# uw-x/AcousticSwarms-Speech

Hardware: AMD Instinct MI355X
Metric: TDoA candidates/sec (shift+normalise+spot forward+energies) (higher is better)
Workload: dtype f32 via f16x3 split-operand MFMA (fp32 accumulate); 1 GPU; configs[2] scene: 5-speaker reverberant mixture (image sources), 7 mics, T=48000 samples (BASELINE's '3 s @ 16 kHz' sample count; the reference pipeline and this scene generator run at 48 kHz, where it is a 1 s clip -- the reference-native 3 s is extras.T144000), fine-stage (Strict=1) candidate batch of one mixture, FULL spot net 47.27 M params, seeded random weights; internal_batch=256, parallelism=candidate-shard x1

## Files before the change

acousticswarms-speech_amd/csrc/asw_common.cpp:

```cpp
#include "asw_common.h"

#include <cmath>
#include <cstdlib>

namespace asw {
char* err_buf() {
  static thread_local char buf[512] = {0};
  return buf;
}
int set_error(int code, const char* fmt, ...) {
  va_list ap;
  va_start(ap, fmt);
  vsnprintf(err_buf(), 512, fmt, ap);
  va_end(ap);
  return code;
}
int SmemAttr::ensure(const void* kern, size_t want) {
  int dev = 0;
  ASW_HIP(hipGetDevice(&dev));
  if (dev < 0 || dev >= kMaxDev) return set_error(ASW_ERR_ARG, "device ordinal %d out of range", dev);
  if (bytes[dev] >= want) return ASW_OK;
  ASW_HIP(hipFuncSetAttribute(kern, hipFuncAttributeMaxDynamicSharedMemorySize, (int)want));
  bytes[dev] = want;
  return ASW_OK;
}
}

extern "C" const char* asw_last_error(void) { return asw::err_buf(); }
extern "C" int asw_abi_version(void) { return 3; }

extern "C" int asw_split_weights_f16(const float* w, size_t n, uint16_t* hi, uint16_t* lo, int32_t* w_shift) {
  ASW_CHECK_ARG(w && hi && lo && w_shift, "split_weights: null pointer");
  float mx = 0.f;
  for (size_t i = 0; i < n; ++i) { const float a = w[i] < 0 ? -w[i] : w[i]; if (a > mx || a != a) mx = a; }
  ASW_CHECK_ARG(mx == mx && mx < 3.0e38f, "split_weights: non-finite weight");
  int shift = 0;
  if (mx > 0.f) {
    int e;
    (void)frexpf(mx, &e);
    shift = 11 - e;
    if (shift > 24) shift = 24;
    if (shift < -24) shift = -24;
  }
  const float sc = ldexpf(1.0f, shift);
  for (size_t i = 0; i < n; ++i) {
    float c = w[i] * sc;
    if (c > 65504.f) c = 65504.f;
    if (c < -65504.f) c = -65504.f;
    const _Float16 h = (_Float16)c;
    const _Float16 l = (_Float16)(c - (float)h);
    memcpy(hi + i, &h, 2);
    memcpy(lo + i, &l, 2);
  }
  *w_shift = shift;
  return ASW_OK;
}

extern "C" int asw_pack_fragments_f16(const float* Wt, int N, int K, uint16_t* hi, uint16_t* lo, int32_t* w_shift) {
  ASW_CHECK_ARG(Wt && hi && lo && w_shift, "pack_fragments: null pointer");
  ASW_CHECK_ARG(N > 0 && K > 0 && N % 32 == 0 && K % 16 == 0, "pack_fragments: N %% 32, K %% 16 required (N=%d K=%d)", N, K);
  const size_t n = (size_t)N * K;
  uint16_t* th = new uint16_t[2 * n];
  uint16_t* tl = th + n;
  int rc = asw_split_weights_f16(Wt, n, th, tl, w_shift);
  if (rc == ASW_OK) {
    const int NT = N / 32;
    for (int ks = 0; ks < K / 16; ++ks)
      for (int nt = 0; nt < NT; ++nt)
        for (int l = 0; l < 64; ++l) {
          const size_t src = (size_t)(nt * 32 + (l & 31)) * K + ks * 16 + 8 * (l >> 5);
          const size_t dst = (((size_t)ks * NT + nt) * 64 + l) * 8;
          memcpy(hi + dst, th + src, 16);
          memcpy(lo + dst, tl + src, 16);
        }
  }
  delete[] th;
  return rc;
}

extern "C" int asw_up_feed_kperm(int k) { return (k & ~12) | ((k & 4) << 1) | ((k & 8) >> 1); }

extern "C" int asw_pack_up_feed_f16(const float* Wt, int N, int K, uint16_t* hi, uint16_t* lo, int32_t* w_shift) {
  ASW_CHECK_ARG(Wt && N > 0 && K > 0 && K % 16 == 0, "pack_up_feed: K %% 16 required (N=%d K=%d)", N, K);
  float* wp = new float[(size_t)N * K];
  for (int n = 0; n < N; ++n)
    for (int k = 0; k < K; ++k) wp[(size_t)n * K + k] = Wt[(size_t)n * K + (k & ~15) + asw_up_feed_kperm(k & 15)];
  const int rc = asw_pack_fragments_f16(wp, N, K, hi, lo, w_shift);
  delete[] wp;
  return rc;
}

namespace asw {
bool residue_feed_on() {
  static const bool off = getenv("ASW_NO_RESIDUE_FEED") != nullptr;
  return !off;
}
}

extern "C" int asw_residue_schedule(int taps, int stride, int dil, int pad, int Cin, int BK, int BM, int m0, int has_skip,
                                    asw_residue_stage* out, int cap, int* n_stages, int* max_shift) {
  ASW_CHECK_ARG(n_stages != nullptr && cap >= 0 && (out != nullptr || cap == 0), "residue_schedule: null pointer");
  ASW_CHECK_ARG(taps > 0 && stride > 0 && dil > 0 && Cin > 0 && BK > 0 && BM > 0, "residue_schedule: bad dims");
  *n_stages = 0;
  if (max_shift) *max_shift = 0;
  if (!asw::residue_feed_applies(taps, stride, dil, Cin, BK, has_skip != 0)) return ASW_OK;
  const asw::ResidueFeed rf{taps, stride, Cin / BK};
  ASW_CHECK_ARG(rf.ntaps(0) <= ASW_RESIDUE_MAX_TAPS, "residue_schedule: %d taps on one image, at most %d", rf.ntaps(0),
                ASW_RESIDUE_MAX_TAPS);
  *n_stages = rf.stages();
  if (max_shift) *max_shift = rf.shifts(0);
  for (int s = 0; s < rf.stages() && s < cap; ++s) {
    asw_residue_stage& d = out[s];
    memset(&d, 0, sizeof d);
    d.residue = s / rf.cpb;
    d.chunk = s - d.residue * rf.cpb;
    d.rows = BM + rf.shifts(d.residue);
    d.first_row = m0 * stride - pad + d.residue;
    d.ntaps = rf.ntaps(d.residue);
    for (int q = 0; q < d.ntaps; ++q) {
      d.tap[q] = rf.tap(d.residue, q);
      d.shift[q] = q;
      d.kstep[q] = rf.kstep(d.tap[q], d.chunk, BK / 16);
    }
  }
  return ASW_OK;
}

#include <map>
#include <mutex>
#include <vector>
namespace asw {
namespace {
struct Rec { std::string name; double work, bytes; hipEvent_t e0, e1; };
std::mutex g_mu;
bool g_on = false;
bool g_detail = false;
std::vector<Rec> g_recs;
std::vector<hipEvent_t> g_pool;
hipEvent_t take_event() {
  if (!g_pool.empty()) { hipEvent_t e = g_pool.back(); g_pool.pop_back(); return e; }
  hipEvent_t e = nullptr;
  (void)hipEventCreate(&e);
  return e;
}
}

std::string prof_name(const char* base, int bm, int bn, int bk, bool ln, bool stats) {
  char b[96];
  snprintf(b, sizeof b, "%s<%d,%d,%d,%s>", base, bm, bn, bk, ln ? "ln" : stats ? "stats" : "plain");
  return b;
}
bool prof_detail() { return g_detail; }
ProfScope::ProfScope(hipStream_t s, const std::string& name, double work, double bytes) : slot(-1), stream(s) {
  if (!g_on) return;
  std::lock_guard<std::mutex> lk(g_mu);
  Rec r{name, work, bytes, take_event(), take_event()};
  (void)hipEventRecord(r.e0, s);
  g_recs.push_back(r);
  slot = (int)g_recs.size() - 1;
}
ProfScope::~ProfScope() {
  if (slot < 0) return;
  std::lock_guard<std::mutex> lk(g_mu);
  if (slot < (int)g_recs.size()) (void)hipEventRecord(g_recs[slot].e1, stream);
}
}

extern "C" int asw_profile_enable(int on) {
  std::lock_guard<std::mutex> lk(asw::g_mu);
  for (auto& r : asw::g_recs) { asw::g_pool.push_back(r.e0); asw::g_pool.push_back(r.e1); }
  asw::g_recs.clear();
  asw::g_on = on != 0;
  asw::g_detail = on == 2;
  return ASW_OK;
}

extern "C" int asw_profile_report(char* buf, size_t cap) {
  if (!buf || cap < 64) return asw::set_error(ASW_ERR_ARG, "profile_report: buffer too small");
  std::lock_guard<std::mutex> lk(asw::g_mu);
  struct Agg { long n = 0; double ms = 0, work = 0, bytes = 0; };
  std::map<std::string, Agg> agg;
  for (auto& r : asw::g_recs) {
    if (hipEventSynchronize(r.e1) != hipSuccess) continue;
    float ms = 0.f;
    if (hipEventElapsedTime(&ms, r.e0, r.e1) != hipSuccess) continue;
    Agg& a = agg[r.name];
    a.n += 1; a.ms += ms; a.work += r.work; a.bytes += r.bytes;
  }
  size_t off = 0;
  off += snprintf(buf + off, cap - off, "{");
  bool first = true;
  for (auto& kv : agg) {
    if (off + 256 >= cap) break;
    off += snprintf(buf + off, cap - off, "%s\"%s\":{\"launches\":%ld,\"ms\":%.6f,\"work\":%.6e,\"bytes\":%.6e}", first ? "" : ",",
                    kv.first.c_str(), kv.second.n, kv.second.ms, kv.second.work, kv.second.bytes);
    first = false;
  }
  snprintf(buf + off, cap - off, "}");
  return ASW_OK;
}
```

acousticswarms-speech_amd/csrc/model_common.h:

```cpp
#pragma once
#include <cstdlib>
#include <iterator>
#include <map>
#include <memory>
#include <string>
#include <vector>

#include "asw_common.h"

namespace asw_model {

struct DevBuf {
  float* p = nullptr;
  size_t n = 0;
  DevBuf() = default;
  DevBuf(const DevBuf&) = delete;
  DevBuf& operator=(const DevBuf&) = delete;
  DevBuf(DevBuf&& o) noexcept : p(o.p), n(o.n) { o.p = nullptr; o.n = 0; }
  ~DevBuf() { if (p) (void)hipFree(p); }
  int upload(const std::vector<float>& h) {
    if (p) { (void)hipFree(p); p = nullptr; }
    n = h.size();
    if (hipMalloc(&p, n * sizeof(float)) != hipSuccess) return asw::set_error(ASW_ERR_NOMEM, "hipMalloc(%zu floats)", n);
    ASW_HIP(hipMemcpy(p, h.data(), n * sizeof(float), hipMemcpyHostToDevice));
// ... 86 lines not shown
inline int pack_res_layers(const std::map<std::string, std::vector<float>>& raw, const std::string& p, int ch, int K,
                           int n_layers, int dil_factor, std::vector<ResLayer>& out) {
  out.clear();
  out.resize(n_layers);
  int dil = 1;
  for (int j = 0; j < n_layers; ++j) {
    const std::string q = p + ".res.seq." + std::to_string(j);
    int rc;
    {
      const std::vector<float> packed = pack_conv(raw.at(q + ".conv.weight"), ch, ch, K, nullptr);
      if ((rc = out[j].wt.upload(packed))) return rc;
      if (ch % 32 == 0 && (ch * K) % 16 == 0 && (rc = out[j].wt.upload_frags(packed, ch, ch * K))) return rc;
    }
    if ((rc = out[j].bias.upload(raw.at(q + ".conv.bias")))) return rc;
    if ((rc = out[j].g.upload(raw.at(q + ".norm.weight")))) return rc;
    if ((rc = out[j].b.upload(raw.at(q + ".norm.bias")))) return rc;
    out[j].dil = dil;
    dil *= dil_factor;
  }
  return ASW_OK;
}

struct Arena {
  char* base;
  size_t off = 0, cap;
  bool dry;
  Arena(char* b, size_t c, bool d) : base(b), cap(c), dry(d) {}
  template <typename T>
  T* take(size_t n) {
    off = (off + 255) & ~(size_t)255;
    T* p = reinterpret_cast<T*>(base + off);
    off += n * sizeof(T);
    return p;
  }
};


struct GluSrc { const float* raw; const float* mr; const float* gamma; const float* beta; float* side_out = nullptr; };

inline bool glu_on_load_ok(const std::vector<ResLayer>& res, int prec, int ch) {
  static const int max_c = getenv("ASW_GLU_ON_LOAD_MAX_C") ? atoi(getenv("ASW_GLU_ON_LOAD_MAX_C")) : 512;
  return prec >= 1 && (ch == 64 || ch == 128 || ch == 256 || ch == 512) && ch <= max_c && !res.empty() &&
         res[0].dil == 1 && res[0].wt.fhi && res[0].wt.flo;
}

inline bool resstack_ok(const std::vector<ResLayer>& res, int prec, int ch, int K) {
  static const bool off = getenv("ASW_NO_RESSTACK") != nullptr;
  if (off || prec < 1 || ch != 64 || K % 2 == 0 || K < 3 || K > 15) return false;
  for (const ResLayer& r : res)
    if (!r.wt.fhi || !r.wt.flo) return false;
  return true;
}

inline size_t resstack_fuse_count(const std::vector<ResLayer>& res, size_t j, int K) {
  static const bool nofuse = getenv("ASW_RESSTACK_NOFUSE") != nullptr;
  size_t n = 1;
  int halo = 0;
  while (!nofuse && j + n < res.size() && n < 3) {
    const int pad = res[j + n].dil * (K - 1) / 2;
    if (halo + pad > 64) break;
    halo += pad;
    ++n;
  }
  return n;
}

struct SrcFeed { const void* hi; const void* lo; const WBuf* comp; const WBuf* pre; };

struct UpFeed { const WBuf* w; const float* bias; const float* skip; float* out; float* stats; int tiles; };

inline void resstack_last_launch(const std::vector<ResLayer>& res, int K, size_t& j0, size_t& n) {
  j0 = 0;
  n = resstack_fuse_count(res, 0, K);
  while (j0 + n < res.size()) { j0 += n; n = resstack_fuse_count(res, j0, K); }
}
inline int up_feed_tiles(const std::vector<ResLayer>& res, int K, int T, bool glu) {
  size_t j0, n;
  resstack_last_launch(res, K, j0, n);
  int32_t dil[3] = {1, 1, 1};
  for (size_t i = 0; i < n; ++i) dil[i] = res[j0 + i].dil;
  return asw_resstack_tiles(T, K, (int)n, dil, glu && j0 == 0);
}

inline int run_res(const std::vector<ResLayer>& res, int prec, int B, int T, int ch, int K, float* x, float* p, float* q,
            float** final_out, hipStream_t s, const GluSrc* glu = nullptr, const SrcFeed* feed = nullptr, UpFeed* up = nullptr) {
  const float* in = glu ? glu->raw : x;
  float* outb = p;
  if (feed && !(resstack_ok(res, prec, ch, K) && prec == 1 && resstack_fuse_count(res, 0, K) == 2))
    return asw::set_error(ASW_ERR_STATE, "run_res: the source-fed form needs the fused f16x3 pair");
  if (up && !(resstack_ok(res, prec, ch, K) && prec == 1))
    return asw::set_error(ASW_ERR_STATE, "run_res: UpFeed needs the f16x3 stack kernel");
  if (resstack_ok(res, prec, ch, K)) {
    size_t j = 0;
    while (j < res.size()) {
      const size_t n = resstack_fuse_count(res, j, K);
      asw_resstack_args a = {};
      a.x = ((glu || feed) && j == 0) ? nullptr : in;
      a.out = outb;
      a.B = B; a.T = T; a.C = ch; a.taps = K; a.n_layers = (int)n; a.precision = prec; a.ln_eps = 1e-5f;
      for (size_t i = 0; i < n; ++i) {
        const ResLayer& r = res[j + i];
        a.layer[i].Wf_hi = r.wt.fhi; a.layer[i].Wf_lo = r.wt.flo; a.layer[i].w_shift = r.wt.shift;
        a.layer[i].bias = r.bias.p; a.layer[i].ln_gamma = r.g.p; a.layer[i].ln_beta = r.b.p; a.layer[i].dil = r.dil;
      }
      if (glu && j == 0) {
        a.glu_raw = glu->raw; a.glu_mr = glu->mr; a.glu_gamma = glu->gamma; a.glu_beta = glu->beta; a.glu_out = glu->side_out;
      }
      if (feed && j == 0) {
        a.src_hi = feed->hi; a.src_lo = feed->lo;
        a.layer[0].Wf_hi = feed->comp->fhi; a.layer[0].Wf_lo = feed->comp->flo; a.layer[0].w_shift = feed->comp->shift;
        a.pre_hi = feed->pre->fhi; a.pre_lo = feed->pre->flo; a.pre_shift = feed->pre->shift;
      }
      if (up && j + n == res.size()) {
        a.out = nullptr;
        a.up_hi = up->w->fhi; a.up_lo = up->w->flo; a.up_shift = up->w->shift; a.up_bias = up->bias; a.up_skip = up->skip;
        a.up_out = up->out; a.up_stats = up->stats;
        up->tiles = up_feed_tiles(res, K, T, glu != nullptr);
        if (up->tiles < 0) return up->tiles;
        outb = nullptr;
      }
      int rc = asw_resstack64_f16x3(&a, s);
      if (rc) return rc;
      in = outb;
      outb = (outb == p) ? q : p;
      j += n;
    }
    *final_out = const_cast<float*>(in);
    return ASW_OK;
  }
  for (size_t j = 0; j < res.size(); ++j) {
    asw_convgemm_args a = {};
    a.A = in; res[j].wt.bind(a, prec); a.bias = res[j].bias.p; a.resid = in;
    if (glu && j == 0) {
      a.glu_raw = glu->raw; a.glu_mr = glu->mr; a.glu_gamma = glu->gamma; a.glu_beta = glu->beta; a.glu_out = glu->side_out;
    }
    a.ln_gamma = res[j].g.p; a.ln_beta = res[j].b.p; a.out = outb;
    a.B = B; a.M_out = T; a.N = ch; a.Cin = ch; a.taps = K; a.stride = 1; a.dil = res[j].dil;
    a.pad = (res[j].dil * (K - 1) + 1) / 2;
    a.a_row_stride = ch; a.a_batch_stride = (int64_t)T * ch; a.a_len = (int64_t)T * ch;
    a.relu = 1; a.ln_eps = 1e-5f;
    int rc = asw_convgemm_f32(&a, s);
    if (rc) return rc;
    in = outb;
    outb = (outb == p) ? q : p;
  }
  *final_out = const_cast<float*>(in);
  return ASW_OK;
}

inline int linear(const float* A, const WBuf& W, int prec, const float* bias, int rows, int N, int K, int relu, const float* resid,
           const float* g, const float* b, float* out, hipStream_t s) {
  asw_convgemm_args a = {};
  a.A = A; W.bind(a, prec); a.bias = bias; a.resid = resid; a.ln_gamma = g; a.ln_beta = b; a.out = out;
  a.B = 1; a.M_out = rows; a.N = N; a.Cin = K; a.taps = 1; a.stride = 1; a.dil = 1; a.pad = 0;
  a.a_row_stride = K; a.a_batch_stride = (int64_t)rows * K; a.a_len = (int64_t)rows * K;
  a.relu = relu; a.ln_eps = 1e-5f;
  if (g && N >= 1024 && N % 256 == 0 && N <= 2048) {
    a.resid = nullptr; a.ln_gamma = nullptr; a.ln_beta = nullptr;
    int rc = asw_convgemm_f32(&a, s);
    if (rc) return rc;
    return asw_add_layernorm(out, resid, g, b, rows, N, 1e-5f, out, s);
  }
  return asw_convgemm_f32(&a, s);
}

inline void pack_conv_transpose(const std::vector<float>& w, const std::vector<float>& b, int Cin, int N, int S,
                                const float* out_gate, std::vector<float>& wt, std::vector<float>& bb) {
  wt.assign((size_t)S * N * Cin, 0.f);
  bb.assign((size_t)S * N, 0.f);
  for (int r = 0; r < S; ++r)
    for (int n = 0; n < N; ++n) {
      bb[(size_t)r * N + n] = out_gate ? b[n] * out_gate[n] : b[n];
      for (int c = 0; c < Cin; ++c) {
        const float v = w[((size_t)c * N + n) * S + r];
        wt[((size_t)r * N + n) * Cin + c] = out_gate ? v * out_gate[n] : v;
      }
    }
}


#define UP(buf, vec) if ((rc = (buf).upload(vec))) return rc

struct TrunkCfg {
  int n_mics, kernel_size, depth, stride_list[8], channels, growth, encoder_channels, encoder_kernel_size,
      encoder_stride, residual_layers, residual_dilation_factor, ffw_dim;
  template <class Cfg>
  static TrunkCfg of(const Cfg& c) {
    TrunkCfg t = {c.n_mics, c.kernel_size, c.depth, {}, c.channels, c.growth, c.encoder_channels,
                  c.encoder_kernel_size, c.encoder_stride, c.residual_layers, c.residual_dilation_factor, c.ffw_dim};
    for (int i = 0; i < 8; ++i) t.stride_list[i] = c.stride_list[i];
    return t;
  }
};

inline int check_trunk_config(const TrunkCfg& c, const char* who, const char* odd) {
  ASW_CHECK_ARG(c.depth >= 1 && c.depth <= 8, "%s: depth %d", who, c.depth);
  ASW_CHECK_ARG(c.n_mics >= 1 && c.n_mics <= 32, "%s: n_mics %d", who, c.n_mics);
  ASW_CHECK_ARG(c.channels % 64 == 0, "%s: channels=%d must be a multiple of 64 for the MFMA tiles", who, c.channels);
  ASW_CHECK_ARG(c.growth >= 1 && c.residual_layers >= 1, "%s: bad config", who);
  ASW_CHECK_ARG(c.kernel_size % 2 == 1, "%s: %s", who, odd);
  ASW_CHECK_ARG(c.encoder_channels % 128 == 0, "%s: encoder_channels must be a multiple of 128", who);
  ASW_CHECK_ARG(c.encoder_stride % 4 == 0 && c.encoder_kernel_size / 2 == c.encoder_stride && c.encoder_kernel_size <= 64,
                "%s: encoder kernel/stride %d/%d unsupported (the reference's trim [9:-8] assumes 33/16)", who,
                c.encoder_kernel_size, c.encoder_stride);
  ASW_CHECK_ARG(c.ffw_dim % 128 == 0, "%s: ffw_dim must be a multiple of 128", who);
  return ASW_OK;
}

struct EncBlock { std::vector<ResLayer> res; DevBuf bias, gn_g, gn_b; };
struct DecBlock { std::vector<ResLayer> res; DevBuf gn_g, gn_b; };
struct GatedConvs { std::vector<WBuf> down_wt, up_wt, up_feed; std::vector<DevBuf> up_bias; };
struct Tap { const float* p; size_t numel; };
using ParamList = std::vector<std::pair<std::string, size_t>>;

struct TrunkPlan {
  int B, T, Tp, F, RL;
  std::vector<int> Tl;
  float *mean, *stdv, *refn;
  uint16_t *src_hi = nullptr, *src_lo = nullptr;
  std::vector<float*> X, Pb, Qb, raw_dn, raw_up, st_dn, st_up, mr_dn, mr_up;
  float *Y, *D, *ywave;
};

struct Trunk {
  TrunkCfg tc;
  std::map<std::string, std::vector<float>> raw;
  std::map<std::string, Tap> taps;
  bool finalized = false;
  int device = 0;
  int precision = 0;
  bool exact_raw = false;
  bool fuse_mask = true;
  bool want_src = false;
  bool src_stack = true;
  bool want_up = false;
  bool up_fusion = true;

  std::vector<int> enc_cin, enc_cout;
  std::vector<int> dec_cin, dec_cout, dec_stride;
  int stride_product = 1;

  DevBuf pre_w, pre_b;
  WBuf src_wt, src_pre;
  std::vector<EncBlock> enc;
  std::vector<DecBlock> dec;
  WBuf byp_wt, mask_wt, dec_wt;
  WBuf byp_wt48;
  DevBuf byp_b, mask_b;
  float out_bias = 0.f;
  int byp_k = 0;

  const std::vector<float>& P(const std::string& k) const { return raw.at(k); }

  enum class Src { Normed, Raw };
  int site(Src a) const { return !exact_raw ? precision : a == Src::Raw ? 0 : 3; }

  int init_shape(const TrunkCfg& c, const char* who) {
    tc = c;
    ASW_HIP(hipGetDevice(&device));
    int cin = c.channels, ch = c.channels;
    for (int i = 0; i < c.depth; ++i) {
      ASW_CHECK_ARG(c.stride_list[i] >= 1, "%s: stride", who);
      enc_cin.push_back(cin);
      enc_cout.push_back(ch);
      stride_product *= c.stride_list[i];
      cin = ch;
      ch *= c.growth;
    }
    dec_cin.assign(enc_cout.rbegin(), enc_cout.rend());
    dec_cout.assign(enc_cin.rbegin(), enc_cin.rend());
    dec_stride.assign(std::make_reverse_iterator(c.stride_list + c.depth), std::make_reverse_iterator(c.stride_list));
    return ASW_OK;
  }
  int check_level_widths(const char* who) const {
    for (int w : enc_cin) ASW_CHECK_ARG(w <= 512 && (w & (w - 1)) == 0, "%s: level width %d must be a power of two <= 512", who, w);
    return ASW_OK;
  }

  ParamList trunk_params() const {
    ParamList v;
    const size_t K = tc.kernel_size;
    v.push_back({"preproc.weight", (size_t)tc.channels * tc.n_mics});
    v.push_back({"preproc.bias", (size_t)tc.channels});
    auto res = [&](const std::string& p, size_t ch) {
      for (int j = 0; j < tc.residual_layers; ++j) {
        const std::string q = p + ".res.seq." + std::to_string(j);
        v.push_back({q + ".conv.weight", ch * ch * K});
        v.push_back({q + ".conv.bias", ch});
        v.push_back({q + ".norm.weight", ch});
        v.push_back({q + ".norm.bias", ch});
      }
    };
    for (int i = 0; i < tc.depth; ++i) {
      const std::string p = "encoder.module_list." + std::to_string(i);
      const size_t ci = enc_cin[i], co = enc_cout[i];
      res(p, ci);
      v.push_back({p + ".conv1.weight", 2 * co * ci * K});
      v.push_back({p + ".conv1.bias", 2 * co});
      v.push_back({p + ".norm1.weight", 2 * co});
      v.push_back({p + ".norm1.bias", 2 * co});
    }
    for (int i = 0; i < tc.depth; ++i) {
      const std::string p = "decoder.module_list." + std::to_string(i);
      const size_t ci = dec_cin[i], co = dec_cout[i], s = dec_stride[i];
      v.push_back({p + ".upsample.conv.weight", ci * 2 * co * s});
      v.push_back({p + ".upsample.conv.bias", 2 * co});
      v.push_back({p + ".norm1.weight", 2 * co});
      v.push_back({p + ".norm1.bias", 2 * co});
      res(p, co);
    }
    const size_t E = tc.encoder_channels, EK = tc.encoder_kernel_size;
    v.push_back({"reference_bypass.weight", E * EK});
    v.push_back({"reference_bypass.bias", E});
    v.push_back({"mask_encoder.weight", E * tc.channels * EK});
    v.push_back({"mask_encoder.bias", E});
    v.push_back({"output_decoder.weight", E * EK});
    v.push_back({"output_decoder.bias", 1});
    return v;
  }
// ... 97 lines not shown
    }
    return ASW_OK;
  }

  bool fused_mask_path() const {
    return fuse_mask && precision >= 1 && tc.encoder_channels % 256 == 0 && tc.channels % 32 == 0 &&
           tc.encoder_kernel_size <= 48 && tc.encoder_stride % 4 == 0 && byp_wt48.fhi && dec_wt.fhi && mask_wt.fhi;
  }
  bool src_path() const {
    return want_src && src_stack && precision == 1 && src_wt.fhi && src_pre.fhi && !enc.empty() &&
           resstack_ok(enc[0].res, precision, enc_cin[0], tc.kernel_size) &&
           resstack_fuse_count(enc[0].res, 0, tc.kernel_size) == 2;
  }
  bool up_feed_shape(int j) const {
    return j >= 1 && dec_cin[j] == 64 && dec_cout[j] == 64 && dec_stride[j] == 2 && dec_cout[j - 1] == 64;
  }
  bool up_path(const GatedConvs& g, int j) const {
    static const bool off = getenv("ASW_NO_UP_FUSION") != nullptr;
    return !off && want_up && up_fusion && precision == 1 && up_feed_shape(j) && g.up_feed[j].fhi &&
           resstack_ok(dec[j - 1].res, precision, 64, tc.kernel_size);
  }
  void layout_levels(int B, int T, Arena& a, TrunkPlan& pl) const {
    const int depth = tc.depth, EK = tc.encoder_kernel_size, ES = tc.encoder_stride;
    pl.B = B; pl.T = T;
    pl.Tp = ((T - 1) / stride_product + 1) * stride_product;
    pl.F = (pl.Tp + 2 * (EK / 2) - EK) / ES + 1;
    pl.RL = ((EK / 2 + pl.Tp + byp_k + 64) + 3) & ~3;
    pl.Tl.assign(depth + 1, pl.Tp);
    for (int i = 0; i < depth; ++i) pl.Tl[i + 1] = pl.Tl[i] / tc.stride_list[i];
    pl.mean = a.take<float>(B);
    pl.stdv = a.take<float>(B);
    pl.refn = a.take<float>((size_t)B * pl.RL);
    if (want_src) {
      pl.src_hi = a.take<uint16_t>((size_t)B * pl.Tp * 8);
      pl.src_lo = a.take<uint16_t>((size_t)B * pl.Tp * 8);
    }
    pl.X.resize(depth + 1); pl.Pb.resize(depth); pl.Qb.resize(depth);
    pl.raw_dn.resize(depth); pl.raw_up.resize(depth); pl.st_dn.resize(depth); pl.st_up.resize(depth);
    pl.mr_up.resize(depth); pl.mr_dn.resize(depth);
    for (int i = 0; i <= depth; ++i) {
      const int ch = i == 0 ? tc.channels : enc_cout[i - 1];
      pl.X[i] = a.take<float>((size_t)B * pl.Tl[i] * ch);
    }
    for (int i = 0; i < depth; ++i) {
      const size_t n = (size_t)B * pl.Tl[i] * enc_cin[i];
      pl.Pb[i] = a.take<float>(n);
      pl.Qb[i] = a.take<float>(n);
      pl.raw_dn[i] = a.take<float>((size_t)B * pl.Tl[i + 1] * 2 * enc_cout[i]);
      pl.st_dn[i] = a.take<float>((size_t)B * 4 * asw_convgemm_stats_tiles(pl.Tl[i + 1], 2 * enc_cout[i]));
      pl.mr_dn[i] = a.take<float>((size_t)B * 4);
    }
    for (int j = 0; j < depth; ++j) {
      const int lvl = depth - j;
      const int s = dec_stride[j], co2 = 2 * dec_cout[j];
      pl.raw_up[j] = a.take<float>((size_t)B * pl.Tl[lvl] * s * co2);
      int tiles = asw_convgemm_stats_tiles(pl.Tl[lvl], s * co2);
      if (want_up && up_feed_shape(j))
        for (int glu = 0; glu < 2; ++glu) {
          const int t = up_feed_tiles(dec[j - 1].res, tc.kernel_size, pl.Tl[lvl], glu != 0);
          tiles = t > tiles ? t : tiles;
        }
      pl.st_up[j] = a.take<float>((size_t)B * 4 * tiles);
      pl.mr_up[j] = a.take<float>((size_t)B * 4);
    }
  }
  void layout_mask(Arena& a, TrunkPlan& pl) const {
    const int E = tc.encoder_channels;
    const bool fused = fused_mask_path();
    pl.Y = fused ? nullptr : a.take<float>((size_t)pl.B * pl.F * E);
    pl.D = a.take<float>((size_t)(fused ? E / 256 : 1) * pl.B * pl.F * 64);
    pl.ywave = a.take<float>((size_t)pl.B * pl.T);
  }

  int encode(TrunkPlan& pl, const GatedConvs& g, hipStream_t s, bool src0 = false) {
    const int B = pl.B, K = tc.kernel_size;
    taps.clear();
    if (!src0) taps["preproc"] = {pl.X[0], (size_t)B * pl.Tl[0] * tc.channels};
    int rc;
    GluSrc src = {};
    const SrcFeed feed = {pl.src_hi, pl.src_lo, &src_wt, &src_pre};
    bool glu = false;
    for (int i = 0; i < tc.depth; ++i) {
      float* r = nullptr;
      if ((rc = run_res(enc[i].res, precision, B, pl.Tl[i], enc_cin[i], K, pl.X[i], pl.Pb[i], pl.Qb[i], &r, s,
                        glu ? &src : nullptr, (src0 && i == 0) ? &feed : nullptr)))
        return rc;
      asw_convgemm_args a = {};
      a.A = r; g.down_wt[i].bind(a, precision); a.bias = enc[i].bias.p; a.out = pl.raw_dn[i]; a.stats = pl.st_dn[i];
      a.B = B; a.M_out = pl.Tl[i + 1]; a.N = 2 * enc_cout[i]; a.Cin = enc_cin[i]; a.taps = K;
      a.stride = tc.stride_list[i]; a.dil = 1; a.pad = K / 2;
      a.a_row_stride = a.Cin; a.a_batch_stride = (int64_t)pl.Tl[i] * a.Cin; a.a_len = a.a_batch_stride;
      a.chan_mod = a.N;
      if ((rc = asw_convgemm_f32(&a, s))) return rc;
      glu = fuse_mask && i + 1 < tc.depth && glu_on_load_ok(enc[i + 1].res, precision, enc_cout[i]);
      const int tiles = asw_convgemm_stats_tiles(a.M_out, a.N);
      if (glu) {
        if ((rc = asw_gn_finalize(pl.st_dn[i], tiles, B, pl.Tl[i + 1], enc_cout[i], 1e-5f, pl.mr_dn[i], s))) return rc;
        src = {pl.raw_dn[i], pl.mr_dn[i], enc[i].gn_g.p, enc[i].gn_b.p, pl.X[i + 1]};
      } else if ((rc = asw_gn_glu(pl.raw_dn[i], pl.st_dn[i], tiles, enc[i].gn_g.p, enc[i].gn_b.p, B, pl.Tl[i + 1],
                                  enc_cout[i], 1e-5f, pl.X[i + 1], s))) {
        return rc;
      }
      taps["enc" + std::to_string(i)] = {pl.X[i + 1], (size_t)B * pl.Tl[i + 1] * enc_cout[i]};
    }
    return ASW_OK;
  }

  int decode(TrunkPlan& pl, const GatedConvs& g, const float*& x, hipStream_t s, bool up = false) {
    const int B = pl.B, K = tc.kernel_size;
    int rc;
    int fed_tiles = 0;
    for (int j = 0; j < tc.depth; ++j) {
      const int lvl = tc.depth - j, ci = dec_cin[j], co = dec_cout[j], st = dec_stride[j];
      int tiles = fed_tiles;
      if (!fed_tiles) {
        asw_convgemm_args a = {};
        a.A = x; a.A2 = pl.X[lvl]; g.up_wt[j].bind(a, precision); a.bias = g.up_bias[j].p; a.out = pl.raw_up[j];
        a.stats = pl.st_up[j];
        a.B = B; a.M_out = pl.Tl[lvl]; a.N = st * 2 * co; a.Cin = ci; a.taps = 1; a.stride = 1; a.dil = 1; a.pad = 0;
        a.a_row_stride = ci; a.a_batch_stride = (int64_t)pl.Tl[lvl] * ci; a.a_len = a.a_batch_stride;
        a.chan_mod = 2 * co;
        if ((rc = asw_convgemm_f32(&a, s))) return rc;
        tiles = asw_convgemm_stats_tiles(a.M_out, a.N);
      }
      const int To = pl.Tl[lvl] * st;
      float* gb = pl.Qb[lvl - 1];
      float* r = nullptr;
      const bool feed_next = up && j + 1 < tc.depth && up_path(g, j + 1);
      UpFeed uf = {};
      if (feed_next) uf = {&g.up_feed[j + 1], g.up_bias[j + 1].p, pl.X[lvl - 1], pl.raw_up[j + 1], pl.st_up[j + 1], 0};
      UpFeed* ufp = feed_next ? &uf : nullptr;
      if (fuse_mask && glu_on_load_ok(dec[j].res, precision, co)) {
        if ((rc = asw_gn_finalize(pl.st_up[j], tiles, B, To, co, 1e-5f, pl.mr_up[j], s))) return rc;
        const GluSrc src = {pl.raw_up[j], pl.mr_up[j], dec[j].gn_g.p, dec[j].gn_b.p, co > 64 ? gb : nullptr};
        if ((rc = run_res(dec[j].res, precision, B, To, co, K, gb, pl.Pb[lvl - 1], gb, &r, s, &src, nullptr, ufp))) return rc;
      } else {
        if ((rc = asw_gn_glu(pl.raw_up[j], pl.st_up[j], tiles, dec[j].gn_g.p, dec[j].gn_b.p, B, To, co, 1e-5f, gb, s)))
          return rc;
        if ((rc = run_res(dec[j].res, precision, B, To, co, K, gb, pl.Pb[lvl - 1], gb, &r, s, nullptr, nullptr, ufp))) return rc;
      }
      x = r;
      fed_tiles = feed_next ? uf.tiles : 0;
      if (!feed_next) taps["dec" + std::to_string(j)] = {x, (size_t)B * To * co};
    }
    return ASW_OK;
  }

  int mask_path(TrunkPlan& pl, const float* x, const float* mean, const float* stdv, float* out_wave, hipStream_t s) {
    const int B = pl.B, C = tc.channels, E = tc.encoder_channels, EK = tc.encoder_kernel_size, ES = tc.encoder_stride;
    int rc;
    asw_convgemm_args me = {};
    me.A = x; mask_wt.bind(me, site(Src::Normed)); me.bias = mask_b.p;
    me.B = B; me.M_out = pl.F; me.N = E; me.Cin = C; me.taps = EK; me.stride = ES; me.dil = 1; me.pad = EK / 2;
    me.a_row_stride = C; me.a_batch_stride = (int64_t)pl.Tp * C; me.a_len = me.a_batch_stride;
    if (fused_mask_path()) {
      asw_maskpath_args f = {};
      f.enc = me;
      f.ref = pl.refn; f.ref_batch_stride = pl.RL; f.ref_len = pl.RL; f.ref_hop = ES;
      f.byp_k = 48; f.byp_taps = EK; f.byp_shift = byp_wt48.shift; f.byp_hi = byp_wt48.fhi; f.byp_lo = byp_wt48.flo;
      f.byp_bias = byp_b.p;
      f.dec_hi = dec_wt.fhi; f.dec_lo = dec_wt.flo; f.dec_shift = dec_wt.shift; f.dec_taps = EK;
      f.taps = pl.D;
      f.enc.precision = precision;
      if ((rc = exact_raw ? asw_mask_path_f16x3_scaled(&f, s) : asw_mask_path_f16x3(&f, s))) return rc;
      return asw_overlap_add_parts(pl.D, E / 256, B, pl.F, 64, EK, EK / 2, pl.T, 9, 8, out_bias, mean, stdv, out_wave, s);
    }
    {
      asw_convgemm_args a = {};
      a.A = pl.refn; byp_wt.bind(a, site(Src::Normed)); a.bias = byp_b.p; a.out = pl.Y;
      a.B = B; a.M_out = pl.F; a.N = E; a.Cin = byp_k; a.taps = 1; a.stride = 1; a.dil = 1; a.pad = 0;
      a.a_row_stride = ES; a.a_batch_stride = pl.RL; a.a_len = pl.RL; a.relu = 1;
      if ((rc = asw_convgemm_f32(&a, s))) return rc;
    }
    me.mul = pl.Y; me.out = pl.Y; me.relu = 1;
    if ((rc = asw_convgemm_f32(&me, s))) return rc;
    taps["latent"] = {pl.Y, (size_t)B * pl.F * E};
    {
      asw_convgemm_args a = {};
      a.A = pl.Y; dec_wt.bind(a, site(Src::Raw)); a.out = pl.D;
      a.B = B; a.M_out = pl.F; a.N = 64; a.Cin = E; a.taps = 1; a.stride = 1; a.dil = 1; a.pad = 0;
      a.a_row_stride = E; a.a_batch_stride = (int64_t)pl.F * E; a.a_len = a.a_batch_stride;
      if ((rc = asw_convgemm_f32(&a, s))) return rc;
    }
    return asw_overlap_add_unnorm(pl.D, B, pl.F, 64, EK, EK / 2, pl.T, 9, 8, out_bias, mean, stdv, out_wave, s);
  }
};

struct PostNormLayer { WBuf w_in, w_out, w1, w2; DevBuf b_in, b_out, b1, b2, n1g, n1b, n2g, n2b; };
struct PostNormBufs { float *qkv, *ctx, *x1, *ff; };

template <class Attention>
int run_post_norm(const Trunk& m, const PostNormLayer& t, const PostNormBufs& b, const float* x, float* out, int rows, int d,
                  int ffw, Attention&& attention, hipStream_t s) {
  const int normed = m.site(Trunk::Src::Normed), rawp = m.site(Trunk::Src::Raw);
  int rc;
  if ((rc = linear(x, t.w_in, normed, t.b_in.p, rows, 3 * d, d, 0, nullptr, nullptr, nullptr, b.qkv, s))) return rc;
  if ((rc = attention(b.qkv, b.ctx))) return rc;
  if ((rc = linear(b.ctx, t.w_out, rawp, t.b_out.p, rows, d, d, 0, x, t.n1g.p, t.n1b.p, b.x1, s))) return rc;
  if ((rc = linear(b.x1, t.w1, normed, t.b1.p, rows, ffw, d, 1, nullptr, nullptr, nullptr, b.ff, s))) return rc;
  return linear(b.ff, t.w2, rawp, t.b2.p, rows, d, ffw, 0, b.x1, t.n2g.p, t.n2b.p, out, s);
}

inline int check_ready(const Trunk* m, const char* fin) {
  if (!m) return asw::set_error(ASW_ERR_ARG, "null model handle");
  if (!m->finalized) return asw::set_error(ASW_ERR_STATE, "%s() has not been called", fin);
  int dev = -1;
  ASW_HIP(hipGetDevice(&dev));
  if (dev != m->device)
    return asw::set_error(ASW_ERR_STATE, "model lives on HIP device %d but the current device is %d", m->device, dev);
  return ASW_OK;
}

inline int set_precision(Trunk* m, const char* who, int precision) {
  ASW_CHECK_ARG(m && (precision >= 0 && precision <= 3), "%s: 0 (f32), 1 (f16x3), 2 (single-pass f16) or 3 (f16x3_safe)", who);
  m->exact_raw = precision == 3;
  m->precision = m->exact_raw ? 1 : precision;
  return ASW_OK;
}

inline int set_param(Trunk* m, const char* who, const char* key, const float* host_data, size_t numel) {
  ASW_CHECK_ARG(m && key && host_data, "%s: null pointer", who);
  m->raw[key].assign(host_data, host_data + numel);
// ... 20 lines not shown
```

acousticswarms-speech_amd/csrc/resconv.hip:

```cpp
#include "gemm_epilogue.h"

namespace {
using namespace asw_mfma;

#ifdef ASW_PHASE_TIMING
__device__ unsigned long long g_phase_cycles[4] = {0, 0, 0, 0};
#endif

template <int BM, int PH, bool POLY>
struct ResRows {
  static constexpr int BMJ = BM / PH;
  int m0, jb, pb, dil, T;
  __device__ __forceinline__ int operator()(int trow) const {
    if (!POLY) { const int t = m0 + trow; return t < T ? t : -1; }
    const int ph = pb * PH + trow / BMJ;
    const int t = dil * (jb * BMJ + trow % BMJ) + ph;
    return (ph < dil && t < T) ? t : -1;
  }
};

template <int BM, int C, int WM, int WN, int PH, int QD = 4, bool POLY = (PH > 1), bool GLU = false, int NTERM = 3>
__global__ __launch_bounds__(64 * WM * WN)
__attribute__((amdgpu_waves_per_eu(C == 64 ? 4 : WM * WN == 8 ? 2 : (QD == 2 ? (C >= 512 || (C == 256 && BM == 128) ? 2 : 3) : (C == 64 && WM * WN == 4 ? 4 : 1)))))
void resconv16_kernel(const asw_convgemm_args p) {
  static_assert(QD == 2 || QD == 4, "B prefetch depth in k-steps");
  static_assert(!GLU || (PH == 1 && !POLY), "GroupNorm + GLU on load: contiguous tiles only");
  static_assert(WM * WN == 2 || WM * WN == 4 || WM * WN == 8, "2, 4 or 8 waves per workgroup");
  constexpr int NTHR = 64 * WM * WN;
  constexpr int TM = BM / WM / 32, TN = C / WN / 32;
  constexpr int NT = C / 32;
  constexpr int BMJ = BM / PH;
  constexpr int SU = (GLU && C > 64) ? 4 : 8;
  static_assert(BMJ % 32 == 0, "an MFMA row tile must stay inside one phase");

  extern __shared__ __align__(16) float smem[];
  char* img = reinterpret_cast<char*>(smem);

  const int tid = threadIdx.x, lane = tid & 63, wid = tid >> 6;
  const int wm = wid / WN, wn = wid % WN;
  const int b = blockIdx.z;
  const int taps = p.taps, dil = p.dil, pad = p.pad;
  const int T = p.M_out;
  const int n_pb = (dil + PH - 1) / PH;
  const int jb = !POLY ? 0 : blockIdx.x / n_pb, pb = !POLY ? 0 : blockIdx.x % n_pb;
  const int m0 = blockIdx.x * BM;
  const int RJ = BMJ + (!POLY ? (taps - 1) * dil : taps - 1);
  const int R = PH * RJ;
  const int tapstep = !POLY ? dil : 1;
  const __amdgpu_buffer_rsrc_t rX = GLU ? act_rsrc(p.glu_raw + (long)b * T * 2 * C, (long)T * 2 * C)
                                        : act_rsrc(p.A + (long)b * p.a_batch_stride, (long)T * C);
  const half8* __restrict__ Wh = reinterpret_cast<const half8*>(p.Wf_hi);
  const half8* __restrict__ Wl = reinterpret_cast<const half8*>(p.Wf_lo);

  floatx16 acc[TM][TN];
#pragma unroll
  for (int i = 0; i < TM; ++i)
#pragma unroll
    for (int j = 0; j < TN; ++j)
#pragma unroll
      for (int r = 0; r < 16; ++r) acc[i][j][r] = 0.f;

  const int sc4 = tid & 15;
  int a_base[TM];
#pragma unroll
  for (int i = 0; i < TM; ++i) {
    const int trow = wm * (BM / WM) + i * 32;
    a_base[i] = ((trow / BMJ) * RJ + trow % BMJ + (lane & 31)) * RS + (lane >> 5) * 16;
  }
  const int nt0 = wn * TN;

  GluCoef gc;
  if (GLU) gc.stats(p.glu_mr, b);
  ASW_PHASE_MARK(t_begin);
#ifdef ASW_PHASE_TIMING
  unsigned long long t_stage = 0, t_loop = 0;
#endif
#pragma unroll(C == 128 && (NTERM == 3 || GLU) ? 2 : 1)
  for (int cc = 0; cc < C / 64; ++cc) {
    ASW_PHASE_MARK(t_s0);
    if (GLU) gc.affine(p.glu_gamma, p.glu_beta, C, cc * 64 + sc4 * 4);
    __syncthreads();
    stage_image<NTHR, C, SU, GLU, NTERM, C == 64>(
        img, R, rX, cc * 64, gc,
        [&](int row) __attribute__((always_inline)) {
          int g;
          bool ok = row < R;
          if (!POLY) {
            g = m0 - pad + row;
          } else {
            const int ph = pb * PH + row / RJ;
            g = dil * (jb * BMJ + row % RJ - (taps - 1) / 2) + ph;
            ok = ok && ph < dil && (jb * BMJ + row % RJ - (taps - 1) / 2) >= 0;
          }
          return ImgSrc{g, ok && g >= 0 && g < T};
        },
        [&](int g, bool ok, const float4& o) __attribute__((always_inline)) {
          if (p.glu_out && ok && g >= m0 && g < m0 + BM)
            *reinterpret_cast<float4*>(p.glu_out + ((long)b * T + g) * C + cc * 64 + sc4 * 4) = o;
        });
    __syncthreads();
    auto bload = [&](int tap, int ks, half8 (&bh)[TN], half8 (&bl)[TN]) {
      const long kg = (long)tap * (C / 16) + cc * 4 + ks;
#pragma unroll
      for (int j = 0; j < TN; ++j) frag_load<NTERM>(Wh, Wl, kg * NT + nt0 + j, lane, bh[j], bl[j]);
    };
    auto aload = [&](int tap, int ks, half8 (&ah)[TM], half8 (&al)[TM]) {
#pragma unroll
      for (int i = 0; i < TM; ++i) {
        const char* q = img + a_base[i] + tap * tapstep * RS + ks * 32;
        ah[i] = *reinterpret_cast<const half8*>(q + IMG_HI);
        if (NTERM == 3) al[i] = *reinterpret_cast<const half8*>(q + IMG_LO);
      }
    };
    auto mma = [&](const half8 (&ah)[TM], const half8 (&al)[TM], const half8 (&bh)[TN], const half8 (&bl)[TN]) {
#pragma unroll
      for (int i = 0; i < TM; ++i)
#pragma unroll
        for (int j = 0; j < TN; ++j) mma3<NTERM>(acc[i][j], ah[i], al[i], bh[j], bl[j]);
    };
    constexpr bool ADB = C != 128;
    half8 qh[QD][TN], ql[QD][TN];
    half8 ah[ADB ? 2 : 1][TM], al[ADB ? 2 : 1][TM];
    ASW_PHASE_MARK(t_s1);
#pragma unroll
    for (int ks = 0; ks < QD; ++ks) bload(0, ks, qh[ks], ql[ks]);
    if (ADB) aload(0, 0, ah[0], al[0]);
    for (int tap = 0; tap < taps; ++tap) {
#pragma unroll
      for (int ks = 0; ks < 4; ++ks) {
        if (ADB) {
          const int nks = (ks + 1) & 3, ntp = tap + (ks == 3 ? 1 : 0);
          if (ntp < taps) aload(ntp, nks, ah[(ks + 1) & 1], al[(ks + 1) & 1]);
        } else {
          aload(tap, ks, ah[0], al[0]);
        }
        mma(ah[ADB ? (ks & 1) : 0], al[ADB ? (ks & 1) : 0], qh[ks % QD], ql[ks % QD]);
        const int nk = ks + QD, ntap = tap + nk / 4;
        if (ntap < taps) bload(ntap, nk % 4, qh[ks % QD], ql[ks % QD]);
      }
    }
#ifdef ASW_PHASE_TIMING
    {
      float sink = acc[0][0][0];
      asm volatile("" ::"v"(sink));
      const unsigned long long t_s2 = __builtin_readcyclecounter();
      t_stage += t_s1 - t_s0;
      t_loop += t_s2 - t_s1;
    }
#endif
  }
  ASW_PHASE_MARK(t_epi0);
  if constexpr (C == 64) {
    using G = EpiGeom<C, WM, WN>;
    float4 rpre[TM * G::NSTEP * G::VPL];
    const int sub = lane / G::LPR, lc = lane % G::LPR;
#pragma unroll
    for (int tm = 0; tm < TM; ++tm)
#pragma unroll
      for (int st = 0; st < G::NSTEP; ++st) {
        const int sr = (st * G::NW + wid) * G::RPI + sub;
        const int trow = (sr >> 5) * (BM / WM) + tm * 32 + (sr & 31);
        const int irow = POLY ? (trow / BMJ) * RJ + trow % BMJ + (taps - 1) / 2 : trow + pad;
#pragma unroll
        for (int q = 0; q < G::VPL; ++q) {
          const int col = (lc + q * G::LPR) * 4;
          const half4 hi = *reinterpret_cast<const half4*>(img + irow * RS + IMG_HI + col * 2);
          const half4 lo = *reinterpret_cast<const half4*>(img + irow * RS + IMG_LO + col * 2);
          rpre[(tm * G::NSTEP + st) * G::VPL + q] = make_float4((float)hi[0] + (float)lo[0], (float)hi[1] + (float)lo[1],
                                                                (float)hi[2] + (float)lo[2], (float)hi[3] + (float)lo[3]);
        }
      }
    epilogue<BM, C, WM, WN, true, false, true, false, ResRows<BM, PH, POLY>, true>(
        acc, p, smem, __builtin_ldexpf(1.0f, -p.w_shift), ResRows<BM, PH, POLY>{m0, jb, pb, dil, T}, blockIdx, gridDim.y, rpre);
  } else {
    epilogue<BM, C, WM, WN, true, false, true, false>(acc, p, smem, __builtin_ldexpf(1.0f, -p.w_shift),
                                                      ResRows<BM, PH, POLY>{m0, jb, pb, dil, T}, blockIdx, gridDim.y);
  }
#ifdef ASW_PHASE_TIMING
  {
    const unsigned long long t_end = __builtin_readcyclecounter();
    if (threadIdx.x == 0) {
      atomicAdd(&g_phase_cycles[0], t_stage);
      atomicAdd(&g_phase_cycles[1], t_loop);
      atomicAdd(&g_phase_cycles[2], t_end - t_epi0);
      atomicAdd(&g_phase_cycles[3], 1ull);
    }
    (void)t_begin;
  }
#endif
}

template <int BM, int C, int WM, int WN, int PH, int QD = 4, bool POLY = (PH > 1), bool GLU = false>
int launch_res(const asw_convgemm_args& a, hipStream_t s) {
  constexpr int BMJ = BM / PH;
  const int RJ = BMJ + (!POLY ? (a.taps - 1) * a.dil : a.taps - 1);
  const size_t img = (size_t)PH * RJ * RS;
  const size_t slab = (size_t)(WM * 32) * (C + 4) * sizeof(float);
  const size_t smem = img > slab ? img : slab;
  if (smem > 160 * 1024) return 1;
  const int gx = !POLY ? asw::cdiv(a.M_out, BM)
                       : asw::cdiv(asw::cdiv(a.M_out, a.dil), BMJ) * asw::cdiv(a.dil, PH);
  char nm[96];
  snprintf(nm, sizeof nm, "resconv16<%d,%d,%s%d%s%s>", BM, C, POLY ? "poly" : "ph", PH, QD == 2 ? ",q2" : "", GLU ? ",glu" : "");
  asw_convgemm_args k = a;
  if (GLU && C > 64) k.resid = a.glu_out;
  return asw::launch_pair<resconv16_kernel<BM, C, WM, WN, PH, QD, POLY, GLU, 1>, resconv16_kernel<BM, C, WM, WN, PH, QD, POLY, GLU, 3>>(
      a.precision, dim3(gx, 1, a.B), dim3(64 * WM * WN), smem, 160 * 1024, nm, asw::ShapeTag(a, 'd', a.dil).s,
      2.0 * a.B * (double)a.M_out * a.N * (double)a.taps * a.Cin, 0.0, s, k);
}

}

#ifdef ASW_PHASE_TIMING
extern "C" int asw_debug_phase_cycles(unsigned long long* out4, int reset) {
  ASW_HIP(hipMemcpyFromSymbol(out4, HIP_SYMBOL(g_phase_cycles), 4 * sizeof(unsigned long long)));
  if (reset) {
    const unsigned long long z[4] = {0, 0, 0, 0};
    ASW_HIP(hipMemcpyToSymbol(HIP_SYMBOL(g_phase_cycles), z, sizeof z));
  }
  return ASW_OK;
}
#endif

namespace asw {
int try_resconv(const asw_convgemm_args& a, hipStream_t s) {
  const bool shape = a.precision >= 1 && a.Wf_hi && a.Wf_lo && a.ln_gamma && a.stride == 1 && a.taps > 1 &&
                     a.taps % 2 == 1 && a.Cin == a.N && a.a_row_stride == a.Cin && a.resid == a.A && !a.A2 &&
                     !a.mul && !a.stats && a.pad * 2 == (a.taps - 1) * a.dil &&
                     a.a_len == (int64_t)a.M_out * a.Cin && a.a_batch_stride == a.a_len;
  if (!shape) return 1;
  if (a.glu_raw) {
    ASW_CHECK_ARG(a.dil == 1 && a.glu_mr && a.glu_gamma && a.glu_beta,
                  "convgemm: GroupNorm + GLU on load needs dilation 1 and the statistics / affine arrays");
    ASW_CHECK_ARG(a.N == 64 || a.glu_out, "convgemm: GroupNorm + GLU on load at %d channels takes the residual from glu_out", a.N);
  }
  const int rows_per_phase = a.M_out / a.dil;
  const bool poly = a.dil >= 16 && rows_per_phase >= 32;
  switch (a.N) {
    case 64:
      if (a.glu_raw) return launch_res<128, 64, 2, 2, 1, 4, false, true>(a, s);
      if (a.dil >= 7 && a.dil < 16 && rows_per_phase >= 96) return launch_res<128, 64, 2, 2, 1, 4, true>(a, s);
      if (!poly) return launch_res<128, 64, 2, 2, 1>(a, s);
      if (rows_per_phase >= 96) return launch_res<128, 64, 2, 2, 1, 4, true>(a, s);
      return rows_per_phase >= 48 ? launch_res<128, 64, 2, 2, 2>(a, s) : launch_res<128, 64, 2, 2, 4>(a, s);
    case 128:
      if (a.glu_raw) return launch_res<128, 128, 2, 2, 1, 2, false, true>(a, s);
      if (!poly) return launch_res<128, 128, 2, 2, 1, 2>(a, s);
      return rows_per_phase >= 48 ? launch_res<128, 128, 2, 2, 2, 2>(a, s) : launch_res<128, 128, 2, 2, 4, 2>(a, s);
    case 256: {
      if (a.glu_raw)
        return (long)asw::cdiv(a.M_out, 128) * a.B >= 512 ? launch_res<128, 256, 1, 4, 1, 2, false, true>(a, s)
                                                          : launch_res<64, 256, 1, 4, 1, 2, false, true>(a, s);
      if (!poly && (long)asw::cdiv(a.M_out, 128) * a.B >= 512) return launch_res<128, 256, 1, 4, 1, 2>(a, s);
      if (poly && rows_per_phase >= 48 && (long)asw::cdiv(a.M_out, 128) * a.B >= 512) return launch_res<128, 256, 1, 4, 2, 2>(a, s);
      return poly ? launch_res<64, 256, 1, 4, 2, 2>(a, s) : launch_res<64, 256, 1, 4, 1, 2>(a, s);
    }
    case 512:
      if (a.glu_raw) return launch_res<64, 512, 1, 4, 1, 2, false, true>(a, s);
      if (poly && a.M_out / a.dil >= 64) return launch_res<64, 512, 1, 4, 2>(a, s);
      return a.dil >= 16 ? launch_res<64, 512, 1, 4, 1>(a, s) : launch_res<64, 512, 1, 4, 1, 2>(a, s);
    default: return 1;
  }
}
}
```

acousticswarms-speech_amd/csrc/resstack.hip:

```cpp
#include <type_traits>

#include "asw_common.h"
#include "f16x3_tile.h"

namespace {
using namespace asw_mfma;

constexpr int C = 64;
constexpr int MAXL = 3;

struct LayerDev {
  const half8* Wh;
  const half8* Wl;
  const float* bias;
  const float* gamma;
  const float* beta;
  int dil, pad;
  int halo;
  int nfrag;
  float scale;
};

#ifdef ASW_PHASE_TIMING
__device__ unsigned long long g_rs_cycles[6] = {0, 0, 0, 0, 0, 0};
#define RS_MARK(var) const unsigned long long var = __builtin_readcyclecounter()
#else
#define RS_MARK(var)
#endif

struct KArgs {
  const float* x;
  float* out;
  const float* glu_raw;
  const float* glu_mr;
  const float* glu_gamma;
  const float* glu_beta;
  float* glu_out;
  const half8* src_h;
  const half8* src_l;
  const half8* Pre_h;
  const half8* Pre_l;
  float pre_up, pre_down;
  int B, T, taps, ntile, BM, img_rows;
  float eps;
  LayerDev L[MAXL];
};

constexpr int UPN = 256;
struct UpArgs {
  const half8* Wh;
  const half8* Wl;
  const float* bias;
  const float* skip;
  float* out;
  float* stats;
  float scale;
};
struct KArgsUp : KArgs { UpArgs u; };

__device__ __forceinline__ __amdgpu_buffer_rsrc_t src_rsrc(const half8* base, long rows) {
  return __builtin_amdgcn_make_buffer_rsrc(const_cast<half8*>(base), 0, (int)(rows * 16), 0x00020000);
}
__device__ __forceinline__ half8 src_load(__amdgpu_buffer_rsrc_t r, int row) {
  return __builtin_bit_cast(half8, __builtin_amdgcn_raw_buffer_load_b128(r, row >= 0 ? row * 16 : (int)0x80000000, 0, 0));
}

template <int NL, int NW, int TM, int PH, bool POLY, bool GLU, int NTERM, int QD, bool SRC = false, bool UP = false>
__global__ __launch_bounds__(64 * NW) __attribute__((amdgpu_waves_per_eu(TM >= 4 ? 1 : 2)))
void resstack64_kernel(const std::conditional_t<UP, KArgsUp, KArgs> p) {
  static_assert(!UP || (!SRC && NTERM == 3), "UpFeed: f16x3, never source-fed");
  static_assert(!POLY || NL == 1, "polyphase row sets: single layers only");
  static_assert(!SRC || (!POLY && !GLU && NTERM == 3), "source-fed layer 0: contiguous tiles, f16x3");
  static_assert(QD == 2 || QD == 4, "weight prefetch depth in k-steps");
  constexpr int NTHR = 64 * NW, SROWS = NTHR / 16;
  constexpr int R0 = 32 * NW * TM;
  constexpr int BMJ = R0 / PH;
  static_assert(BMJ % 32 == 0, "a row fragment must stay inside one phase");

  extern __shared__ __align__(16) char smem[];
  char* img = smem;
  float* tab = reinterpret_cast<float*>(smem + (size_t)p.img_rows * RS);

  const int tid = threadIdx.x, lane = tid & 63, wid = tid >> 6;
  int idx;
  if (!xcd_tile_run(p.B * p.ntile, idx)) return;
  const int b = idx / p.ntile, tile = idx - b * p.ntile;
  const int T = p.T, taps = p.taps;
  const int dil0 = p.L[0].dil, pad0 = p.L[0].pad;
  const int n_pb = POLY ? (dil0 + PH - 1) / PH : 1;
  const int jb = POLY ? tile / n_pb : 0, pb = POLY ? tile - jb * n_pb : 0;
  const int m0 = tile * p.BM;
  const int RJ = BMJ + taps - 1;
  const int R_img = POLY ? PH * RJ : R0 + 2 * pad0;

  RS_MARK(t_start);
  if constexpr (!SRC) {
    for (int i = tid; i < NL * 3 * 16; i += NTHR) {
      const int li = i / 48, w = (i - li * 48) / 16, c4 = i & 15;
      const float* src = w == 0 ? p.L[li].bias : w == 1 ? p.L[li].gamma : p.L[li].beta;
      reinterpret_cast<float4*>(tab)[i] = *reinterpret_cast<const float4*>(src + c4 * 4);
    }
  }
  if constexpr (!SRC) {
    const __amdgpu_buffer_rsrc_t rX = GLU ? act_rsrc(p.glu_raw + (long)b * T * 2 * C, (long)T * 2 * C)
                                          : act_rsrc(p.x + (long)b * T * C, (long)T * C);
    const int srow = tid >> 4, sc4 = tid & 15;
    GluCoef gc;
    if (GLU) {
      gc.stats(p.glu_mr, b);
      gc.affine(p.glu_gamma, p.glu_beta, C, sc4 * 4);
    }
    constexpr int SU = GLU ? 9 : 18;
    for (int r0 = 0; r0 < R_img; r0 += SROWS * SU) {
      float4 buf[SU];
      float4 gate[GLU ? SU : 1];
      bool okr[GLU ? SU : 1];
#pragma unroll
      for (int u = 0; u < SU; ++u) {
        const int row = r0 + u * SROWS + srow;
        int g;
        bool ok = row < R_img;
        if (!POLY) {
          g = m0 - p.L[0].halo - pad0 + row;
        } else {
          const int ph = pb * PH + row / RJ;
          const int jj = jb * BMJ + row % RJ - (taps - 1) / 2;
          g = dil0 * jj + ph;
          ok = ok && ph < dil0 && jj >= 0;
        }
        ok = ok && g >= 0 && g < T;
        if (GLU) {
          buf[u] = act_load4(rX, (long)g * 2 * C + sc4 * 4, ok);
          gate[u] = act_load4(rX, (long)g * 2 * C + C + sc4 * 4, ok);
          okr[u] = ok;
        } else {
          buf[u] = act_load4(rX, (long)g * C + sc4 * 4, ok);
        }
      }
      if (GLU) {
#pragma unroll
        for (int u = 0; u < SU; ++u) {
          const float4 o = gn_glu4(buf[u], gate[u], gc, okr[u]);
          buf[u] = o;
          if (p.glu_out && okr[u]) {
            const int g = m0 - p.L[0].halo - pad0 + r0 + u * SROWS + srow;
            if (g >= m0 && g < m0 + p.BM)
              *reinterpret_cast<float4*>(p.glu_out + ((long)b * T + g) * C + sc4 * 4) = o;
          }
        }
      }
#pragma unroll
      for (int u = 0; u < SU; ++u) {
        const int row = r0 + u * SROWS + srow;
        if (row < R_img) {
          half4 hi, lo;
          split4t<NTERM>(buf[u], hi, lo);
          *reinterpret_cast<half4*>(img + row * RS + IMG_HI + sc4 * 8) = hi;
          *reinterpret_cast<half4*>(img + row * RS + IMG_LO + sc4 * 8) = lo;
        }
      }
    }
  }
  if constexpr (!SRC) __syncthreads();
  RS_MARK(t_staged);
#ifdef ASW_PHASE_TIMING
  unsigned long long t_marks[2 * MAXL + 1];
  t_marks[0] = t_staged;
#endif

  const int h = lane >> 5;
  floatx16 acc[TM][2];
  auto layer = [&](auto lic) {
    constexpr int li = decltype(lic)::value;
    constexpr bool last = li == NL - 1;
    const LayerDev& Ld = p.L[li];
    const int tapstep = (POLY ? 1 : Ld.dil) * RS;
    const int nf = Ld.nfrag - wid * TM;
#pragma unroll
    for (int i = 0; i < TM; ++i)
#pragma unroll
      for (int cb = 0; cb < 2; ++cb)
#pragma unroll
        for (int r = 0; r < 16; ++r) acc[i][cb][r] = 0.f;
    auto img_row = [&](int trow) { return POLY ? (trow / BMJ) * RJ + trow % BMJ : trow; };
    auto run = [&](auto nfc) {
      constexpr int NF = decltype(nfc)::value;
      int xb[NF];
      floatx16 a[NF][2];
#pragma unroll
      for (int i = 0; i < NF; ++i) {
        xb[i] = (img_row((wid * TM + i) * 32) + (lane & 31)) * RS + h * 16;
        a[i][0] = acc[i][0];
        a[i][1] = acc[i][1];
      }
      kloop<NF, 2, QD, NTERM>(
          a, taps, [&](int tap, int i) __attribute__((always_inline)) { return img + xb[i] + tap * tapstep; }, Ld.Wh, Ld.Wl,
          [](int kg, int cb) __attribute__((always_inline)) { return (long)kg * 2 + cb; }, lane);
#pragma unroll
      for (int i = 0; i < NF; ++i) { acc[i][0] = a[i][0]; acc[i][1] = a[i][1]; }
    };
    if constexpr (SRC && li == 0) {
      const __amdgpu_buffer_rsrc_t rH = src_rsrc(p.src_h + (long)b * T, T), rL = src_rsrc(p.src_l + (long)b * T, T);
      const int g0 = m0 - Ld.halo - Ld.pad + wid * TM * 32 + (lane & 31);
      half8 xh[4][TM], xl[4][TM], rh[TM], rl[TM];
#pragma unroll
      for (int ks = 0; ks < 4; ++ks)
#pragma unroll
        for (int i = 0; i < TM; ++i) {
          xh[ks][i] = src_load(rH, g0 + i * 32 + 2 * ks + h);
          xl[ks][i] = src_load(rL, g0 + i * 32 + 2 * ks + h);
        }
#pragma unroll
      for (int i = 0; i < TM; ++i) {
        rh[i] = src_load(rH, g0 + i * 32 + Ld.pad);
        rl[i] = src_load(rL, g0 + i * 32 + Ld.pad);
      }
      half8 wh[2][2], wl[2][2];
      auto wload = [&](auto kgc, int slot) {
        constexpr int kg = decltype(kgc)::value;
#pragma unroll
        for (int cb = 0; cb < 2; ++cb) {
          if constexpr (kg < 4) frag_load<3>(Ld.Wh, Ld.Wl, (long)kg * 2 + cb, lane, wh[slot][cb], wl[slot][cb]);
          else frag_load<3>(p.Pre_h, p.Pre_l, (long)cb, lane, wh[slot][cb], wl[slot][cb]);
        }
      };
      wload(std::integral_constant<int, 0>{}, 0);
      wload(std::integral_constant<int, 1>{}, 1);
      for (int i = tid; i < NL * 3 * 16; i += NTHR) {
        const int lj = i / 48, w = (i - lj * 48) / 16, c4 = i & 15;
        const float* src = w == 0 ? p.L[lj].bias : w == 1 ? p.L[lj].gamma : p.L[lj].beta;
        reinterpret_cast<float4*>(tab)[i] = *reinterpret_cast<const float4*>(src + c4 * 4);
      }
      __syncthreads();
      auto kstep = [&](auto ksc) {
        constexpr int ks = decltype(ksc)::value;
#pragma unroll
        for (int i = 0; i < TM; ++i)
#pragma unroll
          for (int cb = 0; cb < 2; ++cb) mma3<3, true>(acc[i][cb], xh[ks][i], xl[ks][i], wh[ks & 1][cb], wl[ks & 1][cb]);
        if constexpr (ks + 2 <= 4) wload(std::integral_constant<int, ks + 2>{}, ks & 1);
        __builtin_amdgcn_sched_barrier(0);
      };
      kstep(std::integral_constant<int, 0>{});
      kstep(std::integral_constant<int, 1>{});
      kstep(std::integral_constant<int, 2>{});
      kstep(std::integral_constant<int, 3>{});
      const float* tb0 = tab;
#pragma unroll
      for (int i = 0; i < TM; ++i) {
#pragma unroll
        for (int cb = 0; cb < 2; ++cb)
#pragma unroll
          for (int q = 0; q < 4; ++q) {
            const float4 bi = *reinterpret_cast<const float4*>(tb0 + cb * 32 + q * 8 + h * 4);
            const float bv[4] = {bi.x, bi.y, bi.z, bi.w};
#pragma unroll
            for (int j = 0; j < 4; ++j)
              acc[i][cb][q * 4 + j] = fmaxf(acc[i][cb][q * 4 + j] * Ld.scale + bv[j], 0.f) * p.pre_up;
          }
#pragma unroll
        for (int cb = 0; cb < 2; ++cb) mma3<3, true>(acc[i][cb], rh[i], rl[i], wh[0][cb], wl[0][cb]);
      }
    } else {
    if (nf >= TM) run(std::integral_constant<int, TM>{});
    else if constexpr (TM > 1) {
      if (nf == 1) run(std::integral_constant<int, 1>{});
      if constexpr (TM > 2) {
        if (nf == 2) run(std::integral_constant<int, 2>{});
        if (nf == 3) run(std::integral_constant<int, 3>{});
      }
    }
    }
#ifdef ASW_PHASE_TIMING
    {
      float sink = acc[0][0][0];
      asm volatile("" ::"v"(sink));
      t_marks[2 * li + 1] = __builtin_readcyclecounter();
    }
#endif
    const float* tb = tab + li * 192;
    const int cpad = POLY ? (taps - 1) / 2 : Ld.pad;
#pragma unroll
    for (int i = 0; i < TM; ++i) {
      if (i < nf) {
        const int trow = (wid * TM + i) * 32 + (lane & 31);
        const char* rrow = img + (img_row(trow) + cpad) * RS;
        float s = 0.f;
#pragma unroll
        for (int cb = 0; cb < 2; ++cb)
#pragma unroll
          for (int q = 0; q < 4; ++q) {
            const int c0 = cb * 32 + q * 8 + h * 4;
            const float4 bi = *reinterpret_cast<const float4*>(tb + c0);
            const half4 rh = *reinterpret_cast<const half4*>(rrow + IMG_HI + c0 * 2);
            const half4 rl = *reinterpret_cast<const half4*>(rrow + IMG_LO + c0 * 2);
            const float bv[4] = {bi.x, bi.y, bi.z, bi.w};
#pragma unroll
            for (int j = 0; j < 4; ++j) {
              float v;
              if constexpr (SRC && li == 0) {
                v = acc[i][cb][q * 4 + j] * p.pre_down;
              } else {
                v = fmaxf(acc[i][cb][q * 4 + j] * Ld.scale + bv[j], 0.f);
                v += (float)rh[j] + (float)rl[j];
              }
              acc[i][cb][q * 4 + j] = v;
              s += v;
            }
          }
        s += __shfl_xor(s, 32, 64);
        const float mean = s * (1.0f / C);
        float d = 0.f;
#pragma unroll
        for (int cb = 0; cb < 2; ++cb)
#pragma unroll
          for (int r = 0; r < 16; ++r) { const float cx = acc[i][cb][r] - mean; d += cx * cx; }
        d += __shfl_xor(d, 32, 64);
        const float rstd = 1.0f / sqrtf(d * (1.0f / C) + p.eps);
#pragma unroll
        for (int cb = 0; cb < 2; ++cb)
#pragma unroll
          for (int q = 0; q < 4; ++q) {
            const int c0 = cb * 32 + q * 8 + h * 4;
            const float4 g4 = *reinterpret_cast<const float4*>(tb + 64 + c0);
            const float4 b4 = *reinterpret_cast<const float4*>(tb + 128 + c0);
            const float gv[4] = {g4.x, g4.y, g4.z, g4.w}, be[4] = {b4.x, b4.y, b4.z, b4.w};
#pragma unroll
            for (int j = 0; j < 4; ++j) acc[i][cb][q * 4 + j] = (acc[i][cb][q * 4 + j] - mean) * rstd * gv[j] + be[j];
          }
      }
    }
    if constexpr (!last) {
      if constexpr (!(SRC && li == 0)) __syncthreads();
#pragma unroll
      for (int i = 0; i < TM; ++i) {
        if (i < nf) {
          const int trow = (wid * TM + i) * 32 + (lane & 31);
          const int t = m0 - Ld.halo + trow;
          const bool inside = t >= 0 && t < T;
          char* wrow = img + trow * RS;
#pragma unroll
          for (int cb = 0; cb < 2; ++cb)
#pragma unroll
            for (int q = 0; q < 4; ++q) {
              const int c0 = cb * 32 + q * 8 + h * 4;
              float4 v = make_float4(acc[i][cb][q * 4 + 0], acc[i][cb][q * 4 + 1], acc[i][cb][q * 4 + 2], acc[i][cb][q * 4 + 3]);
              if (!inside) v = make_float4(0.f, 0.f, 0.f, 0.f);
              half4 hi, lo;
              split4t<NTERM>(v, hi, lo);
              *reinterpret_cast<half4*>(wrow + IMG_HI + c0 * 2) = hi;
              *reinterpret_cast<half4*>(wrow + IMG_LO + c0 * 2) = lo;
            }
        }
      }
      __syncthreads();
    } else if constexpr (UP) {
      const UpArgs& u = p.u;
      const __amdgpu_buffer_rsrc_t rS = act_rsrc(u.skip + (long)b * T * C, (long)T * C);
      const int tstep = POLY ? dil0 : 1;
      const int widu = __builtin_amdgcn_readfirstlane(wid);
      half8 xh[TM][4], xl[TM][4];
      int t0[TM], nv[TM];
#pragma unroll
      for (int i = 0; i < TM; ++i) {
        const int f0 = (widu * TM + i) * 32;
        int lim;
        if (!POLY) {
          t0[i] = m0 + f0;
          lim = min(p.BM, T - m0) - f0;
// ... 14 lines not shown
          for (int q = 0; q < 4; ++q) {
            const float4 s4 = sk[cb * 4 + q];
            const float4 v = make_float4(acc[i][cb][q * 4 + 0] + s4.x, acc[i][cb][q * 4 + 1] + s4.y,
                                         acc[i][cb][q * 4 + 2] + s4.z, acc[i][cb][q * 4 + 3] + s4.w);
            half4 hi, lo;
            split4t<NTERM>(v, hi, lo);
#pragma unroll
            for (int j = 0; j < 4; ++j) {
              xh[i][cb * 2 + (q >> 1)][(q & 1) * 4 + j] = hi[j];
              xl[i][cb * 2 + (q >> 1)][(q & 1) * 4 + j] = lo[j];
            }
          }
      }
      float st0 = 0.f, sq0 = 0.f, st1 = 0.f, sq1 = 0.f;
      __amdgpu_buffer_rsrc_t rO[TM];
#pragma unroll
      for (int i = 0; i < TM; ++i)
        rO[i] = __builtin_amdgcn_make_buffer_rsrc(u.out + ((long)b * T + t0[i]) * UPN, 0,
                                                  nv[i] > 0 ? ((nv[i] - 1) * tstep + 1) * UPN * 4 : 0, 0x00020000);
      const int voff = (4 * h * tstep * UPN + (lane & 31)) * 4;
      const int rstep = tstep * UPN * 4;
      half8 wh[2][2], wl[2][2];
      auto wload = [&](int ks, int nb2, int slot) __attribute__((always_inline)) {
#pragma unroll
        for (int e = 0; e < 2; ++e) frag_load<NTERM>(u.Wh, u.Wl, (long)ks * (UPN / 32) + nb2 * 2 + e, lane, wh[slot][e], wl[slot][e]);
      };
      wload(0, 0, 0);
#pragma unroll 1
      for (int nb2 = 0; nb2 < UPN / 64; ++nb2) {
        floatx16 y[TM][2];
#pragma unroll
        for (int i = 0; i < TM; ++i)
#pragma unroll
          for (int e = 0; e < 2; ++e)
#pragma unroll
            for (int r = 0; r < 16; ++r) y[i][e][r] = 0.f;
        const float bv[2] = {u.bias[nb2 * 64 + (lane & 31)], u.bias[nb2 * 64 + 32 + (lane & 31)]};
#pragma unroll
        for (int ks = 0; ks < 4; ++ks) {
          if (ks < 3) wload(ks + 1, nb2, (ks + 1) & 1);
          else wload(0, nb2 + 1 < UPN / 64 ? nb2 + 1 : nb2, 0);
#pragma unroll
          for (int i = 0; i < TM; ++i)
#pragma unroll
            for (int e = 0; e < 2; ++e) mma3<NTERM, false>(y[i][e], xh[i][ks], xl[i][ks], wh[ks & 1][e], wl[ks & 1][e]);
        }
        float s1 = 0.f, s2 = 0.f;
#pragma unroll
        for (int i = 0; i < TM; ++i) {
          const bool whole = nv[i] == 32;
#pragma unroll
          for (int e = 0; e < 2; ++e)
#pragma unroll
            for (int r = 0; r < 16; ++r) {
              const float v = y[i][e][r] * u.scale + bv[e];
              __builtin_amdgcn_raw_buffer_store_b32(__builtin_bit_cast(int, v), rO[i],
                                                    voff + ((r & 3) + 8 * (r >> 2)) * rstep + (nb2 * 64 + e * 32) * 4, 0, 0);
              const float m = (whole || acc_row(r, h) < nv[i]) ? v : 0.f;
              s1 += m;
              s2 += m * m;
            }
        }
        if (nb2 & 1) { st1 += s1; sq1 += s2; } else { st0 += s1; sq0 += s2; }
      }
      st0 = wave_sum(st0); sq0 = wave_sum(sq0); st1 = wave_sum(st1); sq1 = wave_sum(sq1);
      __syncthreads();
      float* red = reinterpret_cast<float*>(smem);
      if (lane == 0) { red[wid * 4 + 0] = st0; red[wid * 4 + 1] = sq0; red[wid * 4 + 2] = st1; red[wid * 4 + 3] = sq1; }
      __syncthreads();
      if (tid < 4) {
        float s = 0.f;
#pragma unroll
        for (int w = 0; w < NW; ++w) s += red[w * 4 + tid];
        u.stats[((long)b * p.ntile + tile) * 4 + tid] = s;
      }
    } else {
      float* __restrict__ ob = p.out + (long)b * T * C;
#pragma unroll
      for (int i = 0; i < TM; ++i) {
        if (i < nf) {
          const int trow = (wid * TM + i) * 32 + (lane & 31);
          int t;
          bool ok;
          if (!POLY) {
            t = m0 + trow;
            ok = trow < p.BM && t < T;
          } else {
            const int ph = pb * PH + trow / BMJ;
            t = dil0 * (jb * BMJ + trow % BMJ) + ph;
            ok = ph < dil0 && t < T;
          }
          if (ok) {
            float* orow = ob + (long)t * C;
#pragma unroll
            for (int cb = 0; cb < 2; ++cb)
#pragma unroll
              for (int q = 0; q < 4; ++q) {
                const int c0 = cb * 32 + q * 8 + h * 4;
                *reinterpret_cast<float4*>(orow + c0) =
                    make_float4(acc[i][cb][q * 4 + 0], acc[i][cb][q * 4 + 1], acc[i][cb][q * 4 + 2], acc[i][cb][q * 4 + 3]);
              }
          }
        }
      }
    }
  };
  layer(std::integral_constant<int, 0>{});
#ifdef ASW_PHASE_TIMING
  t_marks[2] = __builtin_readcyclecounter();
#endif
  if constexpr (NL > 1) layer(std::integral_constant<int, 1>{});
  if constexpr (NL > 2) layer(std::integral_constant<int, 2>{});
#ifdef ASW_PHASE_TIMING
  if (threadIdx.x == 0 && NL <= 2) {
    const unsigned long long t_end = __builtin_readcyclecounter();
    atomicAdd(&g_rs_cycles[0], t_staged - t_start);
    atomicAdd(&g_rs_cycles[1], t_marks[1] - t_marks[0]);
    if (NL == 1) {
      atomicAdd(&g_rs_cycles[4], t_end - t_marks[1]);
    } else {
      atomicAdd(&g_rs_cycles[2], t_marks[2] - t_marks[1]);
      atomicAdd(&g_rs_cycles[3], t_marks[3] - t_marks[2]);
      atomicAdd(&g_rs_cycles[4], t_end - t_marks[3]);
    }
    atomicAdd(&g_rs_cycles[5], 1ull);
  }
#endif
}

template <int NL, int NW, int TM, int PH, bool POLY, bool GLU, int QD, bool SRC = false>
int launch_stack(const KArgs& k, const UpArgs* up, int precision, size_t smem, double flops, const char* tag, hipStream_t s) {
  char nm[128], detail[48] = "";
  snprintf(nm, sizeof nm, "resstack64<%s,%dx%d%s%s%s%s>", tag, NW, TM, POLY ? (PH == 1 ? ",poly1" : PH == 2 ? ",poly2" : ",poly4") : "",
           GLU ? ",glu" : "", SRC ? ",src" : "", up ? ",up" : "");
  if (asw::prof_detail()) snprintf(detail, sizeof detail, "[B%d M%d d%d]", k.B, k.T, k.L[0].dil);
  if constexpr (!SRC) {
    if (up) {
      KArgsUp ku;
      static_cast<KArgs&>(ku) = k;
      ku.u = *up;
      return asw::launch_pair<resstack64_kernel<NL, NW, TM, PH, POLY, GLU, 3, QD, false, true>, resstack64_kernel<NL, NW, TM, PH, POLY, GLU, 3, QD, false, true>>(
          1, dim3(xcd_grid_run(k.B * k.ntile)), dim3(64 * NW), smem, 160 * 1024, nm, detail,
          flops + 2.0 * k.B * (double)k.T * C * UPN, (double)k.B * k.T * 4 * ((GLU ? 3 : 2) * C + UPN), s, ku);
    }
  }
  if constexpr (SRC) {
    return asw::launch_pair<resstack64_kernel<NL, NW, TM, PH, POLY, GLU, 3, QD, true>, resstack64_kernel<NL, NW, TM, PH, POLY, GLU, 3, QD, true>>(
        1, dim3(xcd_grid_run(k.B * k.ntile)), dim3(64 * NW), smem, 160 * 1024, nm, detail, flops,
        (double)k.B * k.T * (32 + C * 4), s, k);
  } else {
  return asw::launch_pair<resstack64_kernel<NL, NW, TM, PH, POLY, GLU, 1, QD>, resstack64_kernel<NL, NW, TM, PH, POLY, GLU, 3, QD>>(
      precision, dim3(xcd_grid_run(k.B * k.ntile)), dim3(64 * NW), smem, 160 * 1024, nm, detail, flops,
      (double)k.B * k.T * C * 4 * (GLU ? 3 : 2), s, k);
  }
}

struct TilePlan { bool poly; int PH, BM, ntile; };
TilePlan plan_tiles(int T, int n_layers, int dil0, int halo0, bool glu, int R0) {
  const int rpp = T / dil0;
  if (n_layers == 1 && dil0 >= 7 && rpp >= 48 && !glu) {
    const int PH = rpp >= R0 - 32 ? 1 : rpp >= R0 / 2 - 32 ? 2 : 4;
    return {true, PH, R0, asw::cdiv(asw::cdiv(T, dil0), R0 / PH) * asw::cdiv(dil0, PH)};
  }
  const int BM = R0 - 2 * halo0;
  return {false, 1, BM, BM > 0 ? asw::cdiv(T, BM) : 0};
}

template <int NW, int TM>
int dispatch(const asw_resstack_args& a, KArgs& k, const UpArgs* up, bool glu, double flops, hipStream_t s) {
  constexpr int R0 = 32 * NW * TM;
  const int dil0 = k.L[0].dil;
  const TilePlan tp = plan_tiles(a.T, a.n_layers, dil0, k.L[0].halo, glu, R0);
  k.BM = tp.BM;
  k.ntile = tp.ntile;
  if (tp.poly) {
    const int PH = tp.PH;
    const int BMJ = R0 / PH;
    k.L[0].nfrag = NW * TM;
    k.img_rows = PH * (BMJ + a.taps - 1);
    const size_t smem = (size_t)k.img_rows * RS + 3 * 64 * sizeof(float);
    switch (PH) {
      case 1: return launch_stack<1, NW, TM, 1, true, false, 4>(k, up, a.precision, smem, flops, "1", s);
      case 2: return launch_stack<1, NW, TM, 2, true, false, 4>(k, up, a.precision, smem, flops, "1", s);
      default: return launch_stack<1, NW, TM, 4, true, false, 4>(k, up, a.precision, smem, flops, "1", s);
    }
  }
  ASW_CHECK_ARG(k.BM >= R0 / 2, "resstack: the later layers' halo (%d rows per side) leaves %d of %d rows; fuse fewer layers",
                k.L[0].halo, k.BM, R0);
  int rows = 0;
  for (int i = 0; i < a.n_layers; ++i) {
    k.L[i].nfrag = asw::cdiv(k.BM + 2 * k.L[i].halo, 32);
    const int r = 32 * k.L[i].nfrag + 2 * k.L[i].pad;
    rows = r > rows ? r : rows;
  }
  k.img_rows = rows;
  const size_t smem = (size_t)rows * RS + (size_t)a.n_layers * 3 * 64 * sizeof(float);
  ASW_CHECK_ARG(smem <= 160 * 1024, "resstack: image of %d rows exceeds LDS (dilation %d x %d taps too wide for a contiguous tile)",
                rows, dil0, a.taps);
  if (k.src_h) {
    ASW_CHECK_ARG(k.L[0].nfrag == NW * TM, "resstack: source-fed layer 0 computes %d of %d fragments", k.L[0].nfrag, NW * TM);
    return launch_stack<2, NW, TM, 1, false, false, 4, true>(k, nullptr, a.precision, smem, flops, "2", s);
  }
  switch (a.n_layers) {
    case 1: return glu ? launch_stack<1, NW, TM, 1, false, true, 4>(k, up, a.precision, smem, flops, "1", s)
                       : launch_stack<1, NW, TM, 1, false, false, 4>(k, up, a.precision, smem, flops, "1", s);
    case 2: return glu ? launch_stack<2, NW, TM, 1, false, true, 4>(k, up, a.precision, smem, flops, "2", s)
                       : launch_stack<2, NW, TM, 1, false, false, 4>(k, up, a.precision, smem, flops, "2", s);
    default: return glu ? launch_stack<3, NW, TM, 1, false, true, 4>(k, up, a.precision, smem, flops, "3", s)
                        : launch_stack<3, NW, TM, 1, false, false, 4>(k, up, a.precision, smem, flops, "3", s);
  }
}

}

#ifdef ASW_PHASE_TIMING
extern "C" int asw_debug_resstack_cycles(unsigned long long* out6, int reset) {
  ASW_HIP(hipMemcpyFromSymbol(out6, HIP_SYMBOL(g_rs_cycles), 6 * sizeof(unsigned long long)));
  if (reset) {
    const unsigned long long z[6] = {0, 0, 0, 0, 0, 0};
    ASW_HIP(hipMemcpyToSymbol(HIP_SYMBOL(g_rs_cycles), z, sizeof z));
  }
  return ASW_OK;
}
#endif

extern "C" int asw_compose_source_weights(const float* wc, const float* wpre, const float* bpre, int M, int taps, float* comp,
                                          float* pre16) {
  ASW_CHECK_ARG(wc && wpre && bpre && comp && pre16, "compose_source_weights: null pointer");
  ASW_CHECK_ARG(M >= 1 && M <= 7 && taps >= 1 && taps <= 7, "compose_source_weights: M=%d taps=%d (at most 7 each)", M, taps);
  for (int i = 0; i < C * 16; ++i) pre16[i] = 0.f;
  for (int i = 0; i < C * 64; ++i) comp[i] = 0.f;
  for (int c = 0; c < C; ++c) {
    for (int m = 0; m < M; ++m) pre16[c * 16 + m] = wpre[c * M + m];
    pre16[c * 16 + 7] = bpre[c];
  }
  for (int n = 0; n < C; ++n)
    for (int k = 0; k < taps; ++k)
      for (int j = 0; j < 8; ++j) {
        double acc = 0.0;
        for (int c = 0; c < C; ++c) acc += (double)wc[((size_t)n * C + c) * taps + k] * (double)pre16[c * 16 + j];
        comp[n * 64 + k * 8 + j] = (float)acc;
      }
  return ASW_OK;
}

extern "C" int asw_resstack_tiles(int T, int taps, int n_layers, const int32_t* dil, int glu) {
  ASW_CHECK_ARG(T > 0 && taps >= 3 && taps % 2 == 1 && n_layers >= 1 && n_layers <= MAXL && dil, "resstack_tiles: bad argument");
  int halo0 = 0;
  for (int i = 1; i < n_layers; ++i) halo0 += dil[i] * (taps - 1) / 2;
  const TilePlan t = plan_tiles(T, n_layers, dil[0], halo0, glu != 0, 256);
  ASW_CHECK_ARG(t.BM >= 128, "resstack_tiles: the later layers' halo (%d rows per side) is too wide", halo0);
  return t.ntile;
}

// ... 48 lines not shown
```

acousticswarms-speech_amd/csrc/sep_model.hip:

```cpp
#include <cmath>
#include <map>
#include <memory>
#include <string>
#include <vector>

#include "model_common.h"

using namespace asw_model;

extern "C" int asw_joint_shift_stats_scratch_doubles(void);
namespace asw {
int inter_attention_launch(const char* who, const float* qkv, const int32_t* bounds, int G, int S_uniform, int L, int d,
                           int nhead, float* ctx, hipStream_t st);
}

namespace {

struct Ffn { DevBuf lng, lnb, b1, b2; WBuf w1, w2; };
struct ConfLayer {
  Ffn f1, f2;
  DevBuf n1g, n1b, n2g, n2b, fng, fnb;
  WBuf w_in, w_pos, w_out;
  DevBuf b_out, bu, bv;
  DevBuf cm_lng, cm_lnb, cm_pwb, dw_wT, dw_b, ac_lng, ac_lnb, ac_b;
// ... 157 lines not shown
  const int rows = pl.B * pl.L, d = pl.d, ffw = cfg.ffw_dim;
  const int prec = m->site(Trunk::Src::Normed), rawp = m->site(Trunk::Src::Raw);
  int rc;
  if ((rc = asw_add_layernorm2(x, nullptr, 0.f, c.f1.lng.p, c.f1.lnb.p, rows, d, 1e-5f, 0, nullptr, pl.h, s))) return rc;
  if ((rc = ffn_first(c.f1, prec, pl.h, rows, d, ffw, pl.f, s))) return rc;
  if ((rc = linear(pl.f, c.f1.w2, rawp, c.f1.b2.p, rows, d, ffw, 0, nullptr, nullptr, nullptr, pl.g, s))) return rc;
  if ((rc = asw_add_layernorm2(x, pl.g, 1.f, c.n1g.p, c.n1b.p, rows, d, 1e-5f, 0, pl.x1, pl.h, s))) return rc;
  if ((rc = linear(pl.h, c.w_in, prec, nullptr, rows, 3 * d, d, 0, nullptr, nullptr, nullptr, pl.qkv, s))) return rc;
  if ((rc = linear(m->pe.p, c.w_pos, prec, nullptr, 2 * pl.L - 1, d, d, 0, nullptr, nullptr, nullptr, pl.pos, s))) return rc;
  if ((rc = asw_relpos_attention(pl.qkv, pl.pos, c.bu.p, c.bv.p, pl.B, pl.L, d, cfg.num_head, 1.0f / sqrtf((float)d), pl.ctx, s)))
    return rc;
  if ((rc = linear(pl.ctx, c.w_out, rawp, c.b_out.p, rows, d, d, 0, nullptr, nullptr, nullptr, pl.g, s))) return rc;
  if ((rc = asw_add_layernorm2(pl.x1, pl.g, 1.f, c.cm_lng.p, c.cm_lnb.p, rows, d, 1e-5f, 0, pl.x2, pl.h, s))) return rc;
  if ((rc = linear(pl.h, c.cm_pw, prec, c.cm_pwb.p, rows, 2 * d, d, 0, nullptr, nullptr, nullptr, pl.raw2, s))) return rc;
  if ((rc = asw_glu_rows(pl.raw2, rows, d, pl.u, s))) return rc;
  if ((rc = asw_dwconv_ln_swish(pl.u, c.dw_wT.p, c.dw_b.p, c.ac_lng.p, c.ac_lnb.p, pl.B, pl.L, d, cfg.bottleneck_ksize, 1e-5f,
                                pl.v2, s)))
    return rc;
  if ((rc = linear(pl.v2, c.ac_w, prec, c.ac_b.p, rows, d, d, 0, nullptr, nullptr, nullptr, pl.g, s))) return rc;
  if ((rc = asw_add_layernorm2(pl.x2, pl.g, 1.f, c.f2.lng.p, c.f2.lnb.p, rows, d, 1e-5f, 0, pl.x3, pl.h, s))) return rc;
  if ((rc = ffn_first(c.f2, prec, pl.h, rows, d, ffw, pl.f, s))) return rc;
  if ((rc = linear(pl.f, c.f2.w2, rawp, c.f2.b2.p, rows, d, ffw, 0, pl.x3, c.n2g.p, c.n2b.p, pl.y, s))) return rc;
  return asw_add_layernorm2(pl.y, nullptr, 0.f, c.fng.p, c.fnb.p, rows, d, 1e-6f, 0, nullptr, out, s);
}

int run_inter(asw_sep* m, Plan& pl, PostNormLayer& t, const float* x, float* out, hipStream_t s) {
  auto attention = [&](const float* qkv, float* ctx) {
    return asw::inter_attention_launch("inter_attention", qkv, pl.bounds, pl.G, pl.S, pl.L, pl.d, m->cfg.num_head, ctx, s);
  };
  return run_post_norm(*m, t, {pl.qkv, pl.ctx, pl.x1, pl.f}, x, out, pl.B * pl.L, pl.d, m->cfg.ffw_dim, attention, s);
}

int run_network(asw_sep* m, Plan& pl, const float* mean, const float* stdv, float* out_wave, hipStream_t s) {
  const asw_sep_config& c = m->cfg;
  const int B = pl.B;
  int rc;
  if ((rc = m->encode(pl, m->convs, s))) return rc;
  if ((rc = ensure_pos_table(m, pl.L))) return rc;
  const float* x = pl.X[c.depth];
  for (int l = 0; l < c.bottleneck_layers; ++l) {
    if ((rc = run_conformer(m, pl, m->conf[l], x, pl.intra_out[l], s))) return rc;
    m->taps["intra" + std::to_string(l)] = {pl.intra_out[l], (size_t)B * pl.L * pl.d};
    if (pl.counts) {
      for (int n = 0; n < pl.G; ++n)
        if (pl.counts[n] < pl.S)
          ASW_HIP(hipMemsetAsync(pl.intra_out[l] + ((size_t)n * pl.S + pl.counts[n]) * pl.L * pl.d, 0,
                                 (size_t)(pl.S - pl.counts[n]) * pl.L * pl.d * sizeof(float), s));
    }
    if ((rc = run_inter(m, pl, m->inter[l], pl.intra_out[l], pl.inter_out[l], s))) return rc;
    m->taps["inter" + std::to_string(l)] = {pl.inter_out[l], (size_t)B * pl.L * pl.d};
    x = pl.inter_out[l];
  }
  m->taps["bottleneck"] = {x, (size_t)B * pl.L * pl.d};
  if ((rc = m->decode(pl, m->convs, x, s))) return rc;
  return m->mask_path(pl, x, mean, stdv, out_wave, s);
}

}

extern "C" int asw_sep_create(const asw_sep_config* cfg, asw_sep** out) {
  ASW_CHECK_ARG(cfg && out, "sep_create: null pointer");
  const asw_sep_config& c = *cfg;
  const TrunkCfg tc = TrunkCfg::of(c);
  int rc = check_trunk_config(tc, "sep_create", "kernel sizes must be odd");
  if (rc) return rc;
  ASW_CHECK_ARG(c.max_speakers >= 1 && c.max_speakers <= 64, "sep_create: max_speakers %d", c.max_speakers);
  ASW_CHECK_ARG(c.bottleneck_layers >= 0, "sep_create: bad config");
  ASW_CHECK_ARG(c.bottleneck_ksize % 2 == 1, "sep_create: kernel sizes must be odd");
  std::unique_ptr<asw_sep> m(new asw_sep());
  m->cfg = c;
  if ((rc = m->init_shape(tc, "sep_create"))) return rc;
  const int d = m->enc_cout.back();
  ASW_CHECK_ARG(d <= 1024 && (d & (d - 1)) == 0 && d >= 128, "sep_create: bottleneck width %d must be a power of two in 128..1024", d);
  const int hd = c.num_head > 0 && d % c.num_head == 0 ? d / c.num_head : 0;
  ASW_CHECK_ARG(hd == 16 || hd == 32 || hd == 64, "sep_create: head_dim %d unsupported (16, 32, 64)", hd);
  if ((rc = m->check_level_widths("sep_create"))) return rc;
  *out = m.release();
  return ASW_OK;
}

extern "C" void asw_sep_destroy(asw_sep* m) { delete m; }

extern "C" int asw_sep_set_precision(asw_sep* m, int precision) { return set_precision(m, "sep_set_precision", precision); }

extern "C" int asw_sep_set_param(asw_sep* m, const char* key, const float* host_data, size_t numel) {
  return set_param(m, "sep_set_param", key, host_data, numel);
}

extern "C" int asw_sep_finalize(asw_sep* m) {
  ASW_CHECK_ARG(m, "sep_finalize: null handle");
  const asw_sep_config& c = m->cfg;
  int rc = m->finalize_trunk("sep_finalize", expected_params(m));
  if (rc) return rc;
  if ((rc = m->pack_gated(m->convs, [](const std::string&) { return std::vector<float>(); }))) return rc;
  const int d = m->enc_cout.back(), H = c.num_head, hd = d / H, BK = c.bottleneck_ksize;
  m->inv_freq = m->P("bottleneck.pe_single.inv_freq");
  m->pe_L = 0;
  m->conf.clear(); m->conf.resize(c.bottleneck_layers);
  m->inter.clear(); m->inter.resize(c.bottleneck_layers);
  for (int l = 0; l < c.bottleneck_layers; ++l) {
    const std::string cl = "bottleneck.module_list." + std::to_string(l) + ".intra.layers.0";
    ConfLayer& q = m->conf[l];
    auto ffn = [&](Ffn& f, const std::string& p) -> int {
      UP(f.lng, m->P(p + ".0.weight")); UP(f.lnb, m->P(p + ".0.bias"));
      UP(f.w1, m->P(p + ".1.ffn.0.weight")); UP(f.b1, m->P(p + ".1.ffn.0.bias"));
      UP(f.w2, scaled(m->P(p + ".1.ffn.3.weight"), 0.5f)); UP(f.b2, scaled(m->P(p + ".1.ffn.3.bias"), 0.5f));
      return ASW_OK;
    };
    if ((rc = ffn(q.f1, cl + ".ffn_module1"))) return rc;
    if ((rc = ffn(q.f2, cl + ".ffn_module2"))) return rc;
    UP(q.n1g, m->P(cl + ".norm1.norm.weight")); UP(q.n1b, m->P(cl + ".norm1.norm.bias"));
    UP(q.n2g, m->P(cl + ".norm2.norm.weight")); UP(q.n2b, m->P(cl + ".norm2.norm.bias"));
    const std::string ce = "bottleneck.module_list." + std::to_string(l) + ".intra.norm.norm";
    UP(q.fng, m->P(ce + ".weight")); UP(q.fnb, m->P(ce + ".bias"));
    {
      const std::vector<float>& w = m->P(cl + ".mha_layer.in_proj_weight");
      std::vector<float> o(w.size());
      for (int h = 0; h < H; ++h)
        for (int part = 0; part < 3; ++part)
          for (int cc = 0; cc < hd; ++cc)
            memcpy(&o[((size_t)part * d + h * hd + cc) * d], &w[((size_t)h * 3 * hd + part * hd + cc) * d], sizeof(float) * d);
      UP(q.w_in, o);
    }
    UP(q.w_pos, m->P(cl + ".mha_layer.linear_pos.weight"));
    UP(q.w_out, m->P(cl + ".mha_layer.out_proj.weight")); UP(q.b_out, m->P(cl + ".mha_layer.out_proj.bias"));
    UP(q.bu, m->P(cl + ".mha_layer.pos_bias_u")); UP(q.bv, m->P(cl + ".mha_layer.pos_bias_v"));
    UP(q.cm_lng, m->P(cl + ".convolution_module.layer_norm.weight"));
    UP(q.cm_lnb, m->P(cl + ".convolution_module.layer_norm.bias"));
    UP(q.cm_pw, m->P(cl + ".convolution_module.bottleneck.0.weight"));
    UP(q.cm_pwb, m->P(cl + ".convolution_module.bottleneck.0.bias"));
    {
      const std::vector<float>& w = m->P(cl + ".convolution_module.conv.weight");
      std::vector<float> o((size_t)BK * d);
      for (int cc = 0; cc < d; ++cc)
        for (int k = 0; k < BK; ++k) o[(size_t)k * d + cc] = w[(size_t)cc * BK + k];
      UP(q.dw_wT, o);
    }
    UP(q.dw_b, m->P(cl + ".convolution_module.conv.bias"));
    UP(q.ac_lng, m->P(cl + ".convolution_module.after_conv.0.weight"));
    UP(q.ac_lnb, m->P(cl + ".convolution_module.after_conv.0.bias"));
    UP(q.ac_w, m->P(cl + ".convolution_module.after_conv.2.weight"));
    UP(q.ac_b, m->P(cl + ".convolution_module.after_conv.2.bias"));
    const std::string t = "bottleneck.module_list." + std::to_string(l) + ".inter.layers.0";
    PostNormLayer& il = m->inter[l];
    UP(il.w_in, m->P(t + ".self_attn.in_proj_weight")); UP(il.b_in, m->P(t + ".self_attn.in_proj_bias"));
    UP(il.w_out, m->P(t + ".self_attn.out_proj.weight")); UP(il.b_out, m->P(t + ".self_attn.out_proj.bias"));
    UP(il.w1, m->P(t + ".linear1.weight")); UP(il.b1, m->P(t + ".linear1.bias"));
    UP(il.w2, m->P(t + ".linear2.weight")); UP(il.b2, m->P(t + ".linear2.bias"));
    UP(il.n1g, m->P(t + ".norm1.weight")); UP(il.n1b, m->P(t + ".norm1.bias"));
    UP(il.n2g, m->P(t + ".norm2.weight")); UP(il.n2b, m->P(t + ".norm2.bias"));
  }
  m->finalized = true;
  return ASW_OK;
}

namespace {
int infer_groups(asw_sep* m, const float* mix, int M, int T, const int32_t* offsets, const std::vector<int32_t>& bounds,
                 const std::vector<int32_t>& item, float* out, hipStream_t s) {
  const int B = bounds.back(), G = (int)item.size();
  int rc;
  Plan pl;
  if ((rc = ensure_ws(m, B, T, pl, G))) return rc;
  const int C = m->cfg.channels, pad_l = m->cfg.encoder_kernel_size / 2;
  ASW_HIP(hipMemsetAsync(pl.refn, 0, (size_t)B * pl.RL * sizeof(float), s));
  if ((rc = asw_joint_shift_stats_groups(mix, M, T, offsets, bounds.data(), G, item.data(), pl.jscr, pl.mean, pl.stdv, s)))
    return rc;
// ... 111 lines not shown
```

acousticswarms-speech_amd/csrc/spot_model.hip:

```cpp
#include <map>
#include <memory>
#include <string>
#include <vector>

#include "model_common.h"

using namespace asw_model;

namespace {

struct GateSet : GatedConvs { uint64_t stamp = 0; };

}

struct asw_spot : Trunk {
  asw_spot_config cfg;
  int batch = 32;
  uint64_t clock = 0;
  std::vector<PostNormLayer> tf;
  std::map<std::pair<float, float>, std::unique_ptr<GateSet>> gates;

  char* ws[2] = {nullptr, nullptr};
  size_t ws_bytes[2] = {0, 0};
  int lanes = 1;
// ... 242 lines not shown
      Plan& p = pl[k % lanes];
      hipStream_t q = st[k % lanes];
      p.B = B;
      const int32_t* off = offsets + (size_t)i0 * (M - 1);
      const int32_t* mi = mix_index ? mix_index + i0 : nullptr;
      ASW_HIP(hipMemsetAsync(p.refn, 0, (size_t)B * p.RL * sizeof(float), q));
      int r;
      if ((r = asw_shift_stats_multi(mix, M, T, off, mi, B, circular, p.mean, p.stdv, q))) return r;
      if (src0) {
        if ((r = asw_shift_norm_src_multi(mix, M, T, p.Tp, off, mi, B, circular, p.mean, p.stdv, p.src_hi, p.src_lo,
                                          p.refn + pad_l, p.RL, q)))
          return r;
      } else if ((r = asw_shift_norm_preproc_multi(mix, M, T, p.Tp, off, mi, B, circular, p.mean, p.stdv, m->pre_w.p,
                                                   m->pre_b.p, C, p.X[0], p.refn + pad_l, p.RL, q))) {
        return r;
      }
      float* y = out_wave ? out_wave + (size_t)i0 * T : p.ywave;
      if ((r = run_network(m, p, gs, p.mean, p.stdv, y, q, src0, true))) return r;
      if (out_energy && (r = asw_energies(y, B, T, energy_window, nullptr, out_energy + (size_t)i0 * 2, q))) return r;
    }
    return ASW_OK;
  };
  rc = batches();
  if (lanes == 2) {
    if (hipEventRecord(m->ev_join, m->side) != hipSuccess || hipStreamWaitEvent(s, m->ev_join, 0) != hipSuccess) {
      (void)hipStreamSynchronize(m->side);
      if (!rc) rc = asw::set_error(ASW_ERR_HIP, "shift_and_sep: joining the side lane failed");
    }
  }
  return rc;
}

extern "C" int asw_spot_set_lanes(asw_spot* m, int lanes) {
  ASW_CHECK_ARG(m && (lanes == 1 || lanes == 2), "set_lanes: 1 or 2");
  m->lanes = lanes;
  return ASW_OK;
}

extern "C" int asw_spot_forward(asw_spot* m, const float* mix_norm, int B, int M, int t,
                                const float* window_embedding_host, float* out, void* stream) {
  int rc = check_ready(m, "asw_spot_finalize");
  if (rc) return rc;
  ASW_CHECK_ARG(B >= 0, "forward: B=%d", B);
  if (B == 0) return ASW_OK;
  ASW_CHECK_ARG(mix_norm && window_embedding_host && out, "forward: null pointer");
  ASW_CHECK_ARG(M == m->cfg.n_mics && t >= 1, "forward: bad shape");
  hipStream_t s = asw::as_stream(stream);
  GateSet* gs = nullptr;
  if ((rc = get_gates(m, window_embedding_host[0], window_embedding_host[1], &gs))) return rc;
  const int Bmax = B < m->batch ? B : m->batch;
  Plan pl;
  if ((rc = ensure_ws(m, Bmax, t, pl))) return rc;
  const int C = m->cfg.channels, pad_l = m->cfg.encoder_kernel_size / 2;
  for (int i0 = 0; i0 < B; i0 += Bmax) {
    const int b = B - i0 < Bmax ? B - i0 : Bmax;
    pl.B = b;
    ASW_HIP(hipMemsetAsync(pl.refn, 0, (size_t)b * pl.RL * sizeof(float), s));
    if ((rc = asw_pad_preproc(mix_norm + (size_t)i0 * M * t, b, M, t, pl.Tp, m->pre_w.p, m->pre_b.p, C, pl.X[0],
                              pl.refn + pad_l, pl.RL, s)))
      return rc;
    if ((rc = run_network(m, pl, gs, nullptr, nullptr, out + (size_t)i0 * t, s))) return rc;
  }
  return ASW_OK;
}

extern "C" int asw_spot_set_fused_mask(asw_spot* m, int on) {
  ASW_CHECK_ARG(m, "set_fused_mask: null model handle");
  m->fuse_mask = on != 0;
  return ASW_OK;
}

extern "C" int asw_spot_set_source_stack(asw_spot* m, int on) {
  ASW_CHECK_ARG(m, "set_source_stack: null model handle");
  m->src_stack = on != 0;
  return ASW_OK;
}

extern "C" int asw_spot_set_up_fusion(asw_spot* m, int on) {
  ASW_CHECK_ARG(m, "set_up_fusion: null model handle");
  m->up_fusion = on != 0;
  return ASW_OK;
}

extern "C" int asw_spot_get_tap(asw_spot* m, const char* name, float* dst, size_t capacity, size_t* numel,
                                void* stream) {
  return get_tap(m, "get_tap", name, dst, capacity, numel, stream);
}
```

acousticswarms-speech_amd/native.py:

```python
import ctypes
import glob
import os
import subprocess
import sys
from ctypes import (POINTER, Structure, c_char_p, c_double, c_float, c_int, c_int32, c_int64,
                    c_long, c_size_t, c_void_p)

_HERE = os.path.dirname(os.path.abspath(__file__))
LIB_PATH = os.environ.get("ASW_LIB_PATH") or os.path.join(_HERE, "libasw_hip.so")
CSRC = os.path.join(_HERE, "csrc")
SOURCES = ["asw_common.cpp", "convgemm.hip", "resconv.hip", "pipegemm.hip", "resstack.hip", "downconv.hip", "prep_kernels.hip",
           "misc_kernels.hip", "attention.hip", "srp_kernels.hip",
           "pruner_kernels.hip", "geometry_kernels.hip", "cluster_kernels.hip",
           "search_host.cpp", "sep_kernels.hip", "spot_model.hip", "sep_model.hip", "bss_kernels.hip", "eval_kernels.hip"]
EXTRA_FLAGS = {"geometry_kernels.hip": ["-ffp-contract=off"], "cluster_kernels.hip": ["-ffp-contract=off"],
               "eval_kernels.hip": ["-ffp-contract=off"]}
OPS_PATH = os.path.join(_HERE, "libasw_torch_ops.so")
OPS_SOURCE = "torch_ops.cpp"


def build(force: bool = False, verbose: bool = False) -> str:
    from concurrent.futures import ThreadPoolExecutor
    hdrs = glob.glob(os.path.join(CSRC, "*.h")) + [os.path.join(os.path.dirname(_HERE), "include", "asw_hip.h")]
    hdr_time = max(os.path.getmtime(h) for h in hdrs)
# ... 12 lines not shown

    def run(cmd):
        if verbose:
            print(" ".join(cmd), file=sys.stderr)
        subprocess.run(cmd, check=True)
    with ThreadPoolExecutor(max_workers=min(6, max(1, len(jobs)))) as ex:
        list(ex.map(run, jobs))
    run(["hipcc", "--offload-arch=gfx950", "-fPIC", "-shared", "-o", LIB_PATH] + objs)
    return LIB_PATH


def build_torch_ops(force: bool = False, verbose: bool = False) -> str:
    import torch
    src = os.path.join(CSRC, OPS_SOURCE)
    hdr = os.path.join(os.path.dirname(_HERE), "include", "asw_hip.h")
    if not force and os.path.exists(OPS_PATH) and os.path.getmtime(OPS_PATH) >= max(
            os.path.getmtime(src), os.path.getmtime(hdr), os.path.getmtime(LIB_PATH)):
        return OPS_PATH
    ti = os.path.dirname(torch.__file__)
    cmd = ["hipcc", "-O2", "-std=c++17", "-fPIC", "-shared", "-D__HIP_PLATFORM_AMD__=1", "-DUSE_ROCM=1",
           f"-D_GLIBCXX_USE_CXX11_ABI={int(torch._C._GLIBCXX_USE_CXX11_ABI)}", "-w",
           f"-I{ti}/include", f"-I{ti}/include/torch/csrc/api/include", "-I/opt/rocm/include", src, "-o", OPS_PATH,
           f"-L{_HERE}", "-lasw_hip", f"-L{ti}/lib", "-ltorch", "-ltorch_cpu", "-lc10", "-lc10_hip", "-ltorch_hip",
           "-Wl,-rpath,$ORIGIN", f"-Wl,-rpath,{ti}/lib"]
    if verbose:
        print(" ".join(cmd), file=sys.stderr)
    subprocess.run(cmd, check=True)
    return OPS_PATH


class SpotConfigC(Structure):
    _fields_ = [("n_mics", c_int32), ("kernel_size", c_int32), ("depth", c_int32),
                ("stride_list", c_int32 * 8), ("channels", c_int32), ("growth", c_int32),
                ("encoder_channels", c_int32), ("encoder_kernel_size", c_int32),
                ("encoder_stride", c_int32), ("residual_layers", c_int32),
                ("residual_dilation_factor", c_int32), ("num_head", c_int32), ("ffw_dim", c_int32),
                ("num_transformer_layers", c_int32)]

    @classmethod
    def from_config(cls, cfg):
        s = cls()
        s.n_mics, s.kernel_size, s.depth = cfg.n_mics, cfg.kernel_size, cfg.depth
        for i, v in enumerate(cfg.stride_list):
            s.stride_list[i] = v
        s.channels, s.growth = cfg.channels, int(cfg.growth)
        s.encoder_channels, s.encoder_kernel_size = cfg.encoder_channels, cfg.encoder_kernel_size
        s.encoder_stride, s.residual_layers = cfg.encoder_stride, cfg.residual_layers
        s.residual_dilation_factor, s.num_head = cfg.residual_dilation_factor, cfg.num_head
        s.ffw_dim, s.num_transformer_layers = cfg.ffw_dim, cfg.num_transformer_layers
        return s


class SepConfigC(Structure):
    _fields_ = [("n_mics", c_int32), ("max_speakers", c_int32), ("kernel_size", c_int32), ("depth", c_int32),
                ("stride_list", c_int32 * 8), ("channels", c_int32), ("growth", c_int32),
                ("encoder_channels", c_int32), ("encoder_kernel_size", c_int32), ("encoder_stride", c_int32),
                ("residual_layers", c_int32), ("residual_dilation_factor", c_int32), ("num_head", c_int32),
                ("ffw_dim", c_int32), ("bottleneck_layers", c_int32), ("bottleneck_ksize", c_int32)]

    @classmethod
    def from_config(cls, cfg):
        s = cls()
        s.n_mics, s.max_speakers, s.kernel_size, s.depth = cfg.n_mics, cfg.max_speakers, cfg.kernel_size, cfg.depth
        for i, v in enumerate(cfg.stride_list):
            s.stride_list[i] = v
        s.channels, s.growth = cfg.channels, int(cfg.growth)
        s.encoder_channels, s.encoder_kernel_size = cfg.encoder_channels, cfg.encoder_kernel_size
        s.encoder_stride, s.residual_layers = cfg.encoder_stride, cfg.residual_layers
        s.residual_dilation_factor, s.num_head = cfg.residual_dilation_factor, cfg.num_head
        s.ffw_dim, s.bottleneck_layers, s.bottleneck_ksize = cfg.ffw_dim, cfg.bottleneck_layers, cfg.bottleneck_ksize
        return s


class ConvGemmArgs(Structure):
    _fields_ = [("A", c_void_p), ("A2", c_void_p), ("Wt", c_void_p), ("bias", c_void_p),
                ("resid", c_void_p), ("mul", c_void_p), ("ln_gamma", c_void_p), ("ln_beta", c_void_p),
                ("out", c_void_p), ("stats", c_void_p),
                ("B", c_int32), ("M_out", c_int32), ("N", c_int32), ("Cin", c_int32), ("taps", c_int32),
                ("stride", c_int32), ("dil", c_int32), ("pad", c_int32), ("a_row_stride", c_int32),
                ("a_batch_stride", c_int64), ("a_len", c_int64), ("chan_mod", c_int32), ("relu", c_int32),
                ("ln_eps", c_float), ("precision", c_int32), ("w_shift", c_int32), ("Wt_hi", c_void_p),
                ("Wt_lo", c_void_p), ("Wf_hi", c_void_p), ("Wf_lo", c_void_p), ("stats_stride", c_int32),
                ("glu_raw", c_void_p), ("glu_mr", c_void_p), ("glu_gamma", c_void_p), ("glu_beta", c_void_p),
                ("glu_out", c_void_p)]


class MaskPathArgs(Structure):
    _fields_ = [("enc", ConvGemmArgs), ("ref", c_void_p), ("ref_batch_stride", c_int64), ("ref_len", c_int64),
                ("ref_hop", c_int32), ("byp_k", c_int32), ("byp_taps", c_int32), ("byp_shift", c_int32),
                ("byp_hi", c_void_p), ("byp_lo", c_void_p), ("byp_bias", c_void_p), ("dec_hi", c_void_p),
                ("dec_lo", c_void_p), ("dec_shift", c_int32), ("dec_taps", c_int32), ("taps", c_void_p)]


class ResLayerDesc(Structure):
    _fields_ = [("Wf_hi", c_void_p), ("Wf_lo", c_void_p), ("bias", c_void_p), ("ln_gamma", c_void_p),
                ("ln_beta", c_void_p), ("dil", c_int32), ("w_shift", c_int32)]


class ResStackArgs(Structure):
    _fields_ = [("x", c_void_p), ("out", c_void_p), ("B", c_int32), ("T", c_int32), ("C", c_int32), ("taps", c_int32),
                ("n_layers", c_int32), ("precision", c_int32), ("ln_eps", c_float), ("layer", ResLayerDesc * 3),
                ("glu_raw", c_void_p), ("glu_mr", c_void_p), ("glu_gamma", c_void_p), ("glu_beta", c_void_p),
                ("glu_out", c_void_p), ("src_hi", c_void_p), ("src_lo", c_void_p), ("pre_hi", c_void_p), ("pre_lo", c_void_p),
                ("pre_shift", c_int32), ("up_hi", c_void_p), ("up_lo", c_void_p), ("up_shift", c_int32), ("up_bias", c_void_p),
                ("up_skip", c_void_p), ("up_out", c_void_p), ("up_stats", c_void_p)]


RESIDUE_MAX_TAPS = 8


class ResidueStage(Structure):
    _fields_ = [("residue", c_int32), ("chunk", c_int32), ("rows", c_int32), ("first_row", c_int32), ("ntaps", c_int32),
                ("tap", c_int32 * RESIDUE_MAX_TAPS), ("shift", c_int32 * RESIDUE_MAX_TAPS),
                ("kstep", c_int32 * RESIDUE_MAX_TAPS)]


SIGNATURES = {
    "asw_last_error": (c_char_p, []),
    "asw_abi_version": (c_int, []),
    "asw_profile_enable": (c_int, [c_int]),
    "asw_profile_report": (c_int, [c_char_p, c_size_t]),
    "asw_spot_create": (c_int, [POINTER(SpotConfigC), POINTER(c_void_p)]),
    "asw_spot_destroy": (None, [c_void_p]),
    "asw_spot_set_param": (c_int, [c_void_p, c_char_p, c_void_p, c_size_t]),
    "asw_spot_finalize": (c_int, [c_void_p]),
    "asw_spot_set_batch": (c_int, [c_void_p, c_int]),
    "asw_spot_set_precision": (c_int, [c_void_p, c_int]),
    "asw_spot_set_lanes": (c_int, [c_void_p, c_int]),
    "asw_split_weights_f16": (c_int, [c_void_p, c_size_t, c_void_p, c_void_p, POINTER(c_int32)]),
    "asw_pack_fragments_f16": (c_int, [c_void_p, c_int, c_int, c_void_p, c_void_p, POINTER(c_int32)]),
    "asw_spot_shift_and_sep": (c_int, [c_void_p, c_void_p, c_int, c_int, c_void_p, c_int, c_int, c_int,
                                       c_void_p, c_void_p, c_int, c_void_p]),
    "asw_spot_shift_and_sep_multi": (c_int, [c_void_p, c_void_p, c_int, c_int, c_int, c_void_p, c_void_p, c_int, c_int, c_int,
                                             c_void_p, c_void_p, c_int, c_void_p]),
    "asw_spot_forward": (c_int, [c_void_p, c_void_p, c_int, c_int, c_int, POINTER(c_float), c_void_p, c_void_p]),
    "asw_spot_set_fused_mask": (c_int, [c_void_p, c_int]),
    "asw_spot_set_source_stack": (c_int, [c_void_p, c_int]),
    "asw_spot_set_up_fusion": (c_int, [c_void_p, c_int]),
    "asw_spot_get_tap": (c_int, [c_void_p, c_char_p, c_void_p, c_size_t, POINTER(c_size_t), c_void_p]),
    "asw_sep_create": (c_int, [POINTER(SepConfigC), POINTER(c_void_p)]),
    "asw_sep_destroy": (None, [c_void_p]),
    "asw_sep_set_param": (c_int, [c_void_p, c_char_p, c_void_p, c_size_t]),
    "asw_sep_finalize": (c_int, [c_void_p]),
    "asw_sep_set_precision": (c_int, [c_void_p, c_int]),
    "asw_sep_infer": (c_int, [c_void_p, c_void_p, c_int, c_int, c_void_p, c_int, c_void_p, c_void_p]),
    "asw_sep_infer_batch": (c_int, [c_void_p, c_void_p, c_int, c_int, c_int, c_void_p, c_void_p, c_void_p, c_void_p]),
    "asw_sep_forward": (c_int, [c_void_p, c_void_p, c_int, c_int, c_int, c_int, c_void_p, c_void_p]),
    "asw_sep_forward_counts": (c_int, [c_void_p, c_void_p, c_int, c_int, c_int, c_int, c_void_p, c_void_p, c_void_p]),
    "asw_sep_get_config": (c_int, [c_void_p, POINTER(SepConfigC)]),
    "asw_sep_get_tap": (c_int, [c_void_p, c_char_p, c_void_p, c_size_t, POINTER(c_size_t), c_void_p]),
    "asw_joint_shift_stats": (c_int, [c_void_p, c_int, c_int, c_void_p, c_int, c_void_p, c_void_p, c_void_p, c_void_p]),
    "asw_joint_shift_stats_scratch_doubles": (c_int, []),
    "asw_joint_shift_stats_groups": (c_int, [c_void_p, c_int, c_int, c_void_p, c_void_p, c_int, c_void_p, c_void_p, c_void_p,
                                             c_void_p, c_void_p]),
    "asw_add_layernorm2": (c_int, [c_void_p, c_void_p, c_float, c_void_p, c_void_p, c_int, c_int, c_float, c_int,
                                   c_void_p, c_void_p, c_void_p]),
    "asw_glu_rows": (c_int, [c_void_p, c_long, c_int, c_void_p, c_void_p]),
    "asw_dwconv_ln_swish": (c_int, [c_void_p, c_void_p, c_void_p, c_void_p, c_void_p, c_int, c_int, c_int, c_int,
                                    c_float, c_void_p, c_void_p]),
    "asw_relpos_attention": (c_int, [c_void_p, c_void_p, c_void_p, c_void_p, c_int, c_int, c_int, c_int, c_float,
                                     c_void_p, c_void_p]),
    "asw_inter_attention": (c_int, [c_void_p, c_int, c_int, c_int, c_int, c_int, c_void_p, c_void_p]),
    "asw_inter_attention_groups": (c_int, [c_void_p, c_void_p, c_int, c_int, c_int, c_int, c_void_p, c_void_p]),
    "asw_shift_stats": (c_int, [c_void_p, c_int, c_int, c_void_p, c_int, c_int, c_void_p, c_void_p, c_void_p]),
    "asw_shift_norm_preproc": (c_int, [c_void_p, c_int, c_int, c_int, c_void_p, c_int, c_int, c_void_p, c_void_p,
                                       c_void_p, c_void_p, c_int, c_void_p, c_void_p, c_long, c_void_p]),
    "asw_shift_stats_multi": (c_int, [c_void_p, c_int, c_int, c_void_p, c_void_p, c_int, c_int, c_void_p, c_void_p, c_void_p]),
    "asw_shift_norm_preproc_multi": (c_int, [c_void_p, c_int, c_int, c_int, c_void_p, c_void_p, c_int, c_int, c_void_p,
                                             c_void_p, c_void_p, c_void_p, c_int, c_void_p, c_void_p, c_long, c_void_p]),
    "asw_shift_norm_src_multi": (c_int, [c_void_p, c_int, c_int, c_int, c_void_p, c_void_p, c_int, c_int, c_void_p,
                                         c_void_p, c_void_p, c_void_p, c_void_p, c_long, c_void_p]),
    "asw_pad_preproc": (c_int, [c_void_p, c_int, c_int, c_int, c_int, c_void_p, c_void_p, c_int, c_void_p,
                                c_void_p, c_long, c_void_p]),
    "asw_convgemm_f32": (c_int, [POINTER(ConvGemmArgs), c_void_p]),
    "asw_mask_path_f16x3": (c_int, [POINTER(MaskPathArgs), c_void_p]),
    "asw_mask_path_f16x3_scaled": (c_int, [POINTER(MaskPathArgs), c_void_p]),
    "asw_resstack64_f16x3": (c_int, [POINTER(ResStackArgs), c_void_p]),
    "asw_resstack_tiles": (c_int, [c_int, c_int, c_int, POINTER(c_int32), c_int]),
    "asw_up_feed_kperm": (c_int, [c_int]),
    "asw_pack_up_feed_f16": (c_int, [c_void_p, c_int, c_int, c_void_p, c_void_p, POINTER(c_int32)]),
    "asw_compose_source_weights": (c_int, [c_void_p, c_void_p, c_void_p, c_int, c_int, c_void_p, c_void_p]),
    "asw_convgemm_stats_tiles": (c_int, [c_int, c_int]),
    "asw_f16x3_overflow_count": (c_int, [c_int, POINTER(c_int32)]),
    "asw_residue_schedule": (c_int, [c_int, c_int, c_int, c_int, c_int, c_int, c_int, c_int, c_int,
                                     POINTER(ResidueStage), c_int, POINTER(c_int), POINTER(c_int)]),
    "asw_gn_glu": (c_int, [c_void_p, c_void_p, c_int, c_void_p, c_void_p, c_int, c_int, c_int, c_float, c_void_p,
                           c_void_p]),
    "asw_gn_finalize": (c_int, [c_void_p, c_int, c_int, c_int, c_int, c_float, c_void_p, c_void_p]),
    "asw_attention": (c_int, [c_void_p, c_int, c_int, c_int, c_int, c_void_p, c_void_p]),
    "asw_attention_prec": (c_int, [c_void_p, c_int, c_int, c_int, c_int, c_int, c_void_p, c_void_p]),
    "asw_overlap_add_unnorm": (c_int, [c_void_p, c_int, c_int, c_int, c_int, c_int, c_int, c_int, c_int, c_float,
                                       c_void_p, c_void_p, c_void_p, c_void_p]),
    "asw_overlap_add_parts": (c_int, [c_void_p, c_int, c_int, c_int, c_int, c_int, c_int, c_int, c_int, c_int, c_float,
                                      c_void_p, c_void_p, c_void_p, c_void_p]),
    "asw_energies": (c_int, [c_void_p, c_int, c_int, c_int, c_void_p, c_void_p, c_void_p]),
    "asw_pair_sisdr": (c_int, [c_void_p, c_int, c_int, c_void_p, c_void_p]),
    "asw_center_rows": (c_int, [c_void_p, c_int, c_int, c_void_p]),
    "asw_segment_sisdr": (c_int, [c_void_p, c_int, c_int, c_void_p, c_void_p, c_int, c_void_p, c_void_p]),
    "asw_voiced_segments_workspace_bytes": (c_size_t, [c_int, c_int]),
    "asw_voiced_segments": (c_int, [c_void_p, c_int, c_int, c_double, c_double, c_void_p, c_int, c_void_p, c_void_p,
                                    c_void_p, c_size_t, c_void_p]),
    "asw_fine_clusters_workspace_bytes": (c_size_t, [c_void_p, c_int]),
    "asw_fine_clusters": (c_int, [c_void_p, c_int, c_int, c_void_p, c_int, c_void_p, c_void_p, c_void_p, c_double,
                                  c_double, c_void_p, c_size_t, c_void_p, c_void_p, c_void_p, c_void_p]),
    "asw_global_clusters_workspace_bytes": (c_size_t, [c_int]),
    "asw_global_clusters": (c_int, [c_void_p, c_void_p, c_void_p, c_void_p, c_int, c_int, c_double, c_double, c_double,
                                    c_double, c_double, c_void_p, c_size_t, c_void_p, c_void_p, c_void_p]),
    "asw_coarse_select_workspace_bytes": (c_size_t, [c_int, c_int]),
    "asw_coarse_select": (c_int, [c_void_p, c_void_p, c_void_p, c_int, c_double, c_int, c_double, c_int, c_void_p, c_size_t,
                                  c_void_p, c_void_p, c_void_p, c_void_p]),
    "asw_bss_eval_sdr_workspace_bytes": (c_size_t, [c_void_p, c_int, c_int, c_int, c_int]),
    "asw_bss_eval_sdr": (c_int, [c_void_p, c_void_p, c_void_p, c_int, c_int, c_int, c_int, c_void_p, c_void_p, c_void_p,
                                 c_size_t, c_void_p]),
    "asw_cross_sisdr_workspace_bytes": (c_size_t, [c_void_p, c_void_p, c_int, c_int]),
    "asw_cross_sisdr": (c_int, [c_void_p, c_void_p, c_void_p, c_void_p, c_int, c_int, c_void_p, c_void_p, c_void_p, c_size_t,
                                c_void_p]),
    "asw_add_layernorm": (c_int, [c_void_p, c_void_p, c_void_p, c_void_p, c_int, c_int, c_float, c_void_p, c_void_p]),
    "asw_search_area": (c_int, [c_void_p, c_int, c_void_p, c_int, c_void_p, c_void_p, c_void_p, c_double, c_double,
                                POINTER(c_int), POINTER(c_void_p), POINTER(c_void_p), POINTER(c_void_p),
                                POINTER(c_void_p)]),
    "asw_free": (None, [c_void_p]),
    "asw_cube_select": (c_int, [c_void_p, c_int, c_int, c_int, c_int, c_int, c_int, c_int, c_int, c_void_p, c_void_p,
                                c_void_p, c_int64, POINTER(c_int64)]),
    "asw_cube_select_planes": (c_int, [c_void_p, c_int, c_int, c_int, c_int, c_int, c_int, c_int, c_int, c_void_p, c_void_p,
                                c_void_p, c_int64, POINTER(c_int64)]),
    "asw_srp_frames": (c_int, [c_int, c_int, c_int]),
    "asw_srp_cross_spectra": (c_int, [c_void_p, c_int, c_int, c_int, c_int, c_int, c_int, c_int, c_int, c_int,
                                      c_float, c_void_p, c_void_p, c_void_p, c_int, c_void_p, c_void_p, c_void_p]),
    "asw_srp_map": (c_int, [c_void_p, c_int, c_int, c_int, c_void_p, c_int, c_int, c_void_p, c_void_p, c_void_p,
                            c_void_p, c_void_p, c_void_p]),
    "asw_pruner_covariance": (c_int, [c_void_p, c_int, c_int, c_int, c_int, c_int, c_int, c_int, c_int, c_int,
                                      c_void_p, c_void_p, c_void_p]),
    "asw_hermitian_eigh": (c_int, [c_void_p, c_int, c_int, c_void_p, c_void_p, c_void_p]),
    "asw_music_map": (c_int, [c_void_p, c_int, c_int, c_int, c_void_p, c_int, c_void_p, c_void_p, c_void_p, c_void_p,
                              c_void_p]),
    "asw_tops_map": (c_int, [c_void_p, c_void_p, c_int, c_int, c_int, c_int, c_void_p, c_int, c_double, c_void_p,
                             c_void_p, c_void_p, c_void_p]),
    "asw_geom_lookup_planes": (c_int, [c_void_p, c_int, c_void_p, c_int, c_void_p, c_int, c_void_p, c_int, c_double, c_double,
                                       c_void_p, c_void_p]),
    "asw_geom_voxel_map": (c_int, [c_void_p, c_int, c_void_p, c_int, c_void_p, c_int, c_void_p, c_int, c_void_p, c_void_p,
                                   c_double, c_double, c_double, c_void_p, c_void_p, c_void_p, c_void_p]),
    "asw_geom_label": (c_int, [c_void_p, c_void_p, c_int, c_int, c_int, c_int, c_void_p, c_void_p, c_void_p, POINTER(c_int),
                               c_void_p]),
    "asw_geom_workspace_bytes": (c_int64, [c_int]),
    "asw_geom_compact": (c_int, [c_void_p, c_void_p, c_void_p, c_int, c_void_p, c_int, c_void_p, c_int, c_void_p, c_int,
                                 c_void_p, c_double, c_void_p, c_int64, c_void_p, c_void_p, c_void_p, c_void_p, c_void_p,
                                 c_void_p, c_void_p, c_void_p, c_void_p, POINTER(c_int), c_void_p]),
    "asw_geom_lattice_workspace_bytes": (c_int64, [c_int, c_int]),
    "asw_geom_lattice": (c_int, [c_void_p, c_int, c_int, c_int, c_int, c_void_p, c_void_p, c_void_p, c_void_p, c_double,
                                 c_void_p, c_int64, c_void_p, c_void_p, c_void_p, c_void_p, POINTER(c_int), c_void_p]),
    "asw_lattice_nms_workspace_bytes": (c_int64, [c_int, c_int]),
    "asw_lattice_nms": (c_int, [c_void_p, c_int, c_int, c_void_p, c_int, c_void_p, c_int64, c_void_p, c_void_p, c_void_p]),
}

_lib = None


def lib():
    global _lib
    if _lib is None:
        if not os.path.exists(LIB_PATH):
            raise RuntimeError(
                f"{LIB_PATH} is missing: run `python -c 'import __graft_entry__ as g; g.build()'` "
                "(hipcc --offload-arch=gfx950).  There is no CPU fallback for the hot path.")
        import torch
        L = ctypes.CDLL(LIB_PATH)
        for name, (res, args) in SIGNATURES.items():
            fn = getattr(L, name)
            fn.restype = res
            fn.argtypes = args
        _lib = L
    return _lib


_ops = None


def torch_ops():
    global _ops
    if _ops is None:
        lib()
        if not os.path.exists(OPS_PATH):
            raise RuntimeError(f"{OPS_PATH} is missing: run `python -c 'import __graft_entry__ as g; g.build()'`.  "
                               "The hot path is exposed only through these custom ops; there is no fallback.")
        import torch
        torch.ops.load_library(OPS_PATH)
        _ops = torch.ops.asw
    return _ops


def residue_schedule(taps, stride, Cin, BK=32, BM=256, m0=0, dil=1, pad=0, has_skip=False):
    n, mx = c_int(), c_int()
    L = lib()
    check(L.asw_residue_schedule(taps, stride, dil, pad, Cin, BK, BM, m0, int(has_skip), None, 0, ctypes.byref(n),
                                 ctypes.byref(mx)))
    if n.value == 0:
        return None
    buf = (ResidueStage * n.value)()
    check(L.asw_residue_schedule(taps, stride, dil, pad, Cin, BK, BM, m0, int(has_skip), buf, n.value, ctypes.byref(n),
                                 ctypes.byref(mx)))
    stages = [{"residue": d.residue, "chunk": d.chunk, "rows": d.rows, "first_row": d.first_row,
               "taps": [(d.tap[q], d.shift[q], d.kstep[q]) for q in range(d.ntaps)]} for d in buf]
    return stages, mx.value


def check(status: int):
    if status != 0:
        msg = lib().asw_last_error()
        raise RuntimeError(f"libasw_hip: status {status}: {msg.decode() if msg else ''}")


def ptr(t):
    return None if t is None else c_void_p(t.data_ptr())


def current_stream():
    import torch
    return c_void_p(torch.cuda.current_stream().cuda_stream)


def to_device(a, device):
    import torch
    src = torch.from_numpy(a)
    host = torch.empty(src.shape, dtype=src.dtype, pin_memory=True)
    host.copy_(src)
    return host.to(device, non_blocking=True)


def to_host(t):
    import torch
    if not t.is_cuda:
        return t.numpy()
    host = torch.empty(t.shape, dtype=t.dtype, pin_memory=True)
    host.copy_(t)
    return host.numpy()


def read_back(*tensors):
    import torch
    if not tensors:
        return []
    flat = [t.contiguous().reshape(-1).view(torch.uint8) for t in tensors]
    back = torch.cat(flat).cpu()
    out, pos = [], 0
    for t, f in zip(tensors, flat):
        piece = back[pos:pos + f.numel()].clone()
        out.append(piece.view(t.dtype).reshape(t.shape).numpy())
        pos += f.numel()
    return out
```

acousticswarms-speech_amd/ops.py:

```python
from ctypes import byref

import torch

from .native import ConvGemmArgs, MaskPathArgs, ResStackArgs, check, current_stream, lib, ptr


def _f32(t):
    assert t.is_cuda and t.dtype == torch.float32 and t.is_contiguous(), "need contiguous float32 CUDA tensor"
    return t


def pack_conv_weight(w: torch.Tensor) -> torch.Tensor:
    N, Cin, K = w.shape
    return w.permute(0, 2, 1).reshape(N, K * Cin).contiguous()


def convgemm(A, Wt, M_out, N, Cin, taps=1, stride=1, dil=1, pad=0, bias=None, relu=False, resid=None, mul=None,
             ln=None, stats_chan_mod=0, A2=None, B=None, a_row_stride=None, a_batch_stride=None, a_len=None,
             out=None, ln_eps=1e-5, precision="f32", use_fragments=True, glu=None, glu_out=None):
    _f32(A); _f32(Wt)
    if B is None:
        B = A.shape[0]
    a_row_stride = Cin if a_row_stride is None else a_row_stride
    if a_batch_stride is None:
        a_batch_stride = A[0].numel()
    if a_len is None:
        a_len = a_batch_stride
    if out is None:
        out = torch.empty((B, M_out, N), dtype=torch.float32, device=A.device)
    stats = None
    if stats_chan_mod:
        tiles = lib().asw_convgemm_stats_tiles(M_out, N)
        stats = torch.zeros((B, tiles, 4), dtype=torch.float32, device=A.device)
    a = ConvGemmArgs()
    a.A, a.A2, a.Wt = A.data_ptr(), (A2.data_ptr() if A2 is not None else None), Wt.data_ptr()
    a.bias = bias.data_ptr() if bias is not None else None
    a.resid = resid.data_ptr() if resid is not None else None
    a.mul = mul.data_ptr() if mul is not None else None
    a.ln_gamma = ln[0].data_ptr() if ln is not None else None
    a.ln_beta = ln[1].data_ptr() if ln is not None else None
    a.out = out.data_ptr()
    a.stats = stats.data_ptr() if stats is not None else None
    a.B, a.M_out, a.N, a.Cin, a.taps, a.stride, a.dil, a.pad = B, M_out, N, Cin, taps, stride, dil, pad
    a.a_row_stride, a.a_batch_stride, a.a_len = a_row_stride, a_batch_stride, a_len
    a.chan_mod, a.relu, a.ln_eps = stats_chan_mod, int(relu), ln_eps
    if glu is not None:
        a.glu_raw, a.glu_mr, a.glu_gamma, a.glu_beta = (_f32(t).data_ptr() for t in glu)
        if glu_out is not None:
            a.glu_out = _f32(glu_out).data_ptr()
    keep = None
    if precision in ("f16x3", "f16"):
        hi, lo, shift = split_weights_f16(Wt)
        keep = (hi, lo)
        a.precision, a.w_shift, a.Wt_hi, a.Wt_lo = (1 if precision == "f16x3" else 2), shift, hi.data_ptr(), lo.data_ptr()
        if use_fragments and N % 32 == 0 and (taps * Cin) % 16 == 0:
            fh, fl, sh2 = pack_fragments_f16(Wt, N, taps * Cin)
            assert sh2 == shift
            keep = keep + (fh, fl)
            a.Wf_hi, a.Wf_lo = fh.data_ptr(), fl.data_ptr()
    check(lib().asw_convgemm_f32(byref(a), current_stream()))
    torch.cuda.current_stream().synchronize() if keep is not None else None
    return out, stats


def resstack(x, layers, taps=7, precision="f16x3", eps=1e-5, glu=None, out=None, glu_out=None):
    src = x if glu is None else glu[0]
    B, T = src.shape[0], src.shape[1]
    if out is None:
        out = torch.empty((B, T, 64), dtype=torch.float32, device=src.device)
    a = ResStackArgs()
    a.x = _f32(x).data_ptr() if x is not None else None
    a.out = out.data_ptr()
    a.B, a.T, a.C, a.taps, a.n_layers = B, T, 64, taps, len(layers)
    a.precision, a.ln_eps = (1 if precision == "f16x3" else 2), eps
    keep = []
    for i, (Wt, bias, gamma, beta, dil) in enumerate(layers):
        fh, fl, sh = pack_fragments_f16(_f32(Wt), 64, taps * 64)
        keep.append((fh, fl))
        d = a.layer[i]
        d.Wf_hi, d.Wf_lo, d.w_shift, d.dil = fh.data_ptr(), fl.data_ptr(), sh, dil
        d.bias, d.ln_gamma, d.ln_beta = _f32(bias).data_ptr(), _f32(gamma).data_ptr(), _f32(beta).data_ptr()
    if glu is not None:
        a.glu_raw, a.glu_mr, a.glu_gamma, a.glu_beta = (_f32(t).data_ptr() for t in glu)
        if glu_out is not None:
            a.glu_out = _f32(glu_out).data_ptr()
    check(lib().asw_resstack64_f16x3(byref(a), current_stream()))
    torch.cuda.current_stream().synchronize()
    return out


def resstack_up(x, layers, up_wt, up_bias, skip, taps=7, eps=1e-5, glu=None):
    import ctypes
    src = x if glu is None else glu[0]
    B, T = src.shape[0], src.shape[1]
    dev = src.device
    a = ResStackArgs()
    a.x = _f32(x).data_ptr() if x is not None else None
    a.B, a.T, a.C, a.taps, a.n_layers, a.precision, a.ln_eps = B, T, 64, taps, len(layers), 1, eps
    keep = []
    for i, (Wt, bias, gamma, beta, dil) in enumerate(layers):
        fh, fl, sh = pack_fragments_f16(_f32(Wt), 64, taps * 64)
        keep.append((fh, fl))
        d = a.layer[i]
        d.Wf_hi, d.Wf_lo, d.w_shift, d.dil = fh.data_ptr(), fl.data_ptr(), sh, dil
        d.bias, d.ln_gamma, d.ln_beta = _f32(bias).data_ptr(), _f32(gamma).data_ptr(), _f32(beta).data_ptr()
    if glu is not None:
        a.glu_raw, a.glu_mr, a.glu_gamma, a.glu_beta = (_f32(t).data_ptr() for t in glu)
    dils = (ctypes.c_int32 * 3)(*([l[4] for l in layers] + [1] * (3 - len(layers))))
    tiles = lib().asw_resstack_tiles(T, taps, len(layers), dils, int(glu is not None))
    check(min(tiles, 0))
    uh, ul, ush = pack_fragments_f16(up_wt, 256, 64, up_feed=True)
    raw = torch.full((B, T, 256), float("nan"), dtype=torch.float32, device=dev)
    stats = torch.full((B, tiles, 4), float("nan"), dtype=torch.float32, device=dev)
    a.up_hi, a.up_lo, a.up_shift = uh.data_ptr(), ul.data_ptr(), ush
    a.up_bias, a.up_skip, a.up_out, a.up_stats = _f32(up_bias).data_ptr(), _f32(skip).data_ptr(), raw.data_ptr(), stats.data_ptr()
    check(lib().asw_resstack64_f16x3(byref(a), current_stream()))
    torch.cuda.current_stream().synchronize()
    return raw, stats


def resstack_src(src_hi, src_lo, pre_w, pre_b, layers, taps=7, eps=1e-5, out=None):
    import ctypes
    import numpy as np
    B, T = src_hi.shape[0], src_hi.shape[1]
    dev = src_hi.device
    if out is None:
        out = torch.empty((B, T, 64), dtype=torch.float32, device=dev)
    M = pre_w.shape[1]
    wc = np.ascontiguousarray(layers[0][0].detach().cpu().numpy(), dtype=np.float32)
    wp = np.ascontiguousarray(pre_w.detach().cpu().numpy(), dtype=np.float32).reshape(64, M)
    bp = np.ascontiguousarray(pre_b.detach().cpu().numpy(), dtype=np.float32)
    comp, pre16 = np.empty((64, 64), dtype=np.float32), np.empty((64, 16), dtype=np.float32)
    check(lib().asw_compose_source_weights(ctypes.c_void_p(wc.ctypes.data), ctypes.c_void_p(wp.ctypes.data),
                                           ctypes.c_void_p(bp.ctypes.data), M, taps, ctypes.c_void_p(comp.ctypes.data),
                                           ctypes.c_void_p(pre16.ctypes.data)))
    a = ResStackArgs()
    a.out = out.data_ptr()
    a.B, a.T, a.C, a.taps, a.n_layers, a.precision, a.ln_eps = B, T, 64, taps, len(layers), 1, eps
    keep = []
    for i, (w, bias, gamma, beta, dil) in enumerate(layers):
        Wt = torch.from_numpy(comp).to(dev) if i == 0 else pack_conv_weight(w).to(dev)
        fh, fl, sh = pack_fragments_f16(Wt, 64, Wt.shape[1])
        keep.append((fh, fl))
        d = a.layer[i]
        d.Wf_hi, d.Wf_lo, d.w_shift, d.dil = fh.data_ptr(), fl.data_ptr(), sh, dil
        d.bias, d.ln_gamma, d.ln_beta = _f32(bias).data_ptr(), _f32(gamma).data_ptr(), _f32(beta).data_ptr()
    ph, pl, psh = pack_fragments_f16(torch.from_numpy(pre16).to(dev), 64, 16)
    a.src_hi, a.src_lo, a.pre_hi, a.pre_lo, a.pre_shift = src_hi.data_ptr(), src_lo.data_ptr(), ph.data_ptr(), pl.data_ptr(), psh
    check(lib().asw_resstack64_f16x3(byref(a), current_stream()))
    torch.cuda.current_stream().synchronize()
    return out


def pack_fragments_f16(Wt, N, K, up_feed=False):
    import ctypes
    import numpy as np
    w = np.ascontiguousarray(Wt.detach().cpu().numpy(), dtype=np.float32).reshape(N, K)
# ... 274 lines not shown
```

acousticswarms-speech_amd/spot.py:

```python
import numpy as np

from . import native
from .config import FULL, SpotConfig, spot_param_shapes
from .device_model import DeviceModel
from .scorer import DeviceScorer


def offsets_from_patches(patch_list, n_pairs: int = None) -> np.ndarray:
    if len(patch_list) == 0:
        return np.zeros((0, n_pairs or 0), dtype=np.int32)
    offs = np.stack([np.asarray(getattr(p, "sample_offset", p), dtype=np.float64) for p in patch_list])
    if n_pairs is not None and offs.shape[1] != n_pairs:
        raise RuntimeError(f"candidate has {offs.shape[1]} offsets, mixture has {n_pairs + 1} channels")
    return np.rint(offs.astype(np.float32)).astype(np.int32)


class SpotModel(DeviceModel, DeviceScorer):
    C_PREFIX, CONFIG_C, NAME, HOT_PATH = "spot", native.SpotConfigC, "SpotModel", "spot hot path"
    param_shapes = staticmethod(spot_param_shapes)

    def __init__(self, cfg: SpotConfig = FULL, state_dict=None, batch_size: int = 32, precision: str = "f32",
                 lanes: int = 1):
        DeviceModel.__init__(self, cfg, precision)
        self.batch_size = batch_size
# ... 64 lines not shown

    def shift_and_score(self, input_channels, patch_list, Strict: int = 0, window: int = 12000,
                        keep_waveforms: bool = True) -> np.ndarray:
        import torch
        self._need()
        mix = torch.as_tensor(input_channels)
        if len(patch_list) == 0:
            self.last_waveforms = None
            return np.empty((0, 2), dtype=np.float64)
        offs = offsets_from_patches(patch_list, mix.shape[0] - 1)
        mix_d = mix.to(self.device, dtype=torch.float32).contiguous()
        off_d = torch.from_numpy(offs).to(self.device)
        wave, en = self.shift_and_sep_device(mix_d, off_d, Strict, want_wave=keep_waveforms, want_energy=True,
                                             window=window)
        self.last_waveforms = wave
        return en.cpu().numpy()

    def shift_and_sep_resident(self, input_channels, patch_list, Strict: int = 0, window: int = 12000,
                               device_energies: bool = False):
        import torch
        self._need()
        mix = torch.as_tensor(input_channels)
        offs = offsets_from_patches(patch_list, mix.shape[0] - 1)
        mix_d = mix.to(self.device, dtype=torch.float32).contiguous()
        if device_energies:
            off_d = torch.from_numpy(offs).pin_memory().to(self.device, non_blocking=True)
        else:
            off_d = torch.from_numpy(offs).to(self.device)
        wave, en = self.shift_and_sep_device(mix_d, off_d, Strict, want_wave=True, want_energy=True, window=window)
        native.torch_ops().center_rows_(wave)
        return wave, (en if device_energies else en.cpu().numpy())

    def score_offsets(self, input_channels, offsets, Strict: int = 0, window: int = 12000):
        import torch
        self._need()
        mix = torch.as_tensor(input_channels)
        mix_d = mix.to(self.device, dtype=torch.float32).contiguous()
        if isinstance(offsets, torch.Tensor):
            off_d = offsets.to(self.device, dtype=torch.int32).contiguous()
        else:
            off_d = torch.from_numpy(np.ascontiguousarray(offsets, dtype=np.int32)).pin_memory().to(self.device, non_blocking=True)
        if off_d.dim() != 2 or off_d.shape[1] != mix_d.shape[0] - 1:
            raise RuntimeError(f"offsets of shape {tuple(off_d.shape)} do not fit a mixture of {mix_d.shape[0]} channels")
        if off_d.shape[0] == 0:
            return torch.empty((0, 2), dtype=torch.float64, device=self.device)
        _wave, en = self.shift_and_sep_device(mix_d, off_d, Strict, want_wave=False, want_energy=True, window=window)
        return en

    def forward(self, mix, window_embedding):
        import torch
        self._need()
        mix = torch.as_tensor(mix).to(self.device, dtype=torch.float32).contiguous()
        wemb = torch.as_tensor(window_embedding, dtype=torch.float32).cpu().numpy().reshape(mix.shape[0], 2)
        B, M, t = mix.shape
        out = torch.empty((B, 1, t), dtype=torch.float32, device=self.device)
        keys = {}
        for i, row in enumerate(map(tuple, wemb)):
            keys.setdefault(row, []).append(i)
        ops = native.torch_ops()
        for row, idx in keys.items():
            whole = len(idx) == B
            y = ops.spot_forward(self._h.value, mix if whole else mix[idx].contiguous(), float(row[0]), float(row[1]))
            if whole:
                return y.view(B, 1, t)
            out.view(B, t)[idx] = y
        return out

    __call__ = forward

    def set_fused_mask(self, on: bool = True):
        self._need()
        native.check(native.lib().asw_spot_set_fused_mask(self._h, int(bool(on))))
        return self

    def set_source_stack(self, on: bool = True):
        self._need()
        native.check(native.lib().asw_spot_set_source_stack(self._h, int(bool(on))))
        return self

    def set_up_fusion(self, on: bool = True):
        self._need()
        native.check(native.lib().asw_spot_set_up_fusion(self._h, int(bool(on))))
        return self
```

include/asw_hip.h:

```cpp
#ifndef ASW_HIP_H
#define ASW_HIP_H

#include <stddef.h>
#include <stdint.h>

#ifdef __cplusplus
extern "C" {
#endif

typedef enum asw_status {
  ASW_OK = 0,
  ASW_ERR_ARG = -1,
  ASW_ERR_HIP = -2,
  ASW_ERR_NOMEM = -3,
  ASW_ERR_STATE = -4
} asw_status;

const char* asw_last_error(void);
int asw_abi_version(void);

int asw_profile_enable(int on);
int asw_profile_report(char* buf, size_t cap);

typedef struct asw_spot_config {
  int32_t n_mics;
  int32_t kernel_size;
  int32_t depth;
  int32_t stride_list[8];
  int32_t channels;
  int32_t growth;
  int32_t encoder_channels;
  int32_t encoder_kernel_size;
  int32_t encoder_stride;
  int32_t residual_layers;
  int32_t residual_dilation_factor;
  int32_t num_head;
  int32_t ffw_dim;
  int32_t num_transformer_layers;
} asw_spot_config;

typedef struct asw_spot asw_spot;

int asw_spot_create(const asw_spot_config* cfg, asw_spot** out);
void asw_spot_destroy(asw_spot* m);

int asw_spot_set_param(asw_spot* m, const char* key, const float* host_data, size_t numel);
int asw_spot_finalize(asw_spot* m);

int asw_spot_set_batch(asw_spot* m, int batch);

int asw_spot_set_lanes(asw_spot* m, int lanes);

int asw_spot_set_precision(asw_spot* m, int precision);

int asw_spot_shift_and_sep(asw_spot* m, const float* mix, int M, int T,
                           const int32_t* offsets, int N, int strict, int circular,
                           float* out_wave, double* out_energy, int energy_window,
                           void* stream);

int asw_spot_shift_and_sep_multi(asw_spot* m, const float* mix, int K, int M, int T, const int32_t* offsets,
                                 const int32_t* mix_index, int N, int strict, int circular, float* out_wave,
                                 double* out_energy, int energy_window, void* stream);

int asw_spot_forward(asw_spot* m, const float* mix_norm, int B, int M, int t,
                     const float* window_embedding_host, float* out, void* stream);

int asw_spot_set_fused_mask(asw_spot* m, int on);

int asw_spot_set_source_stack(asw_spot* m, int on);

int asw_spot_set_up_fusion(asw_spot* m, int on);

int asw_spot_get_tap(asw_spot* m, const char* name, float* dst, size_t capacity, size_t* numel,
                     void* stream);

typedef struct asw_sep_config {
  int32_t n_mics;
  int32_t max_speakers;
  int32_t kernel_size;
  int32_t depth;
  int32_t stride_list[8];
  int32_t channels;
  int32_t growth;
  int32_t encoder_channels;
  int32_t encoder_kernel_size;
  int32_t encoder_stride;
  int32_t residual_layers;
  int32_t residual_dilation_factor;
  int32_t num_head;
  int32_t ffw_dim;
  int32_t bottleneck_layers;
  int32_t bottleneck_ksize;
} asw_sep_config;

typedef struct asw_sep asw_sep;

int asw_sep_create(const asw_sep_config* cfg, asw_sep** out);
void asw_sep_destroy(asw_sep* m);
int asw_sep_set_param(asw_sep* m, const char* key, const float* host_data, size_t numel);
int asw_sep_finalize(asw_sep* m);
int asw_sep_set_precision(asw_sep* m, int precision);

int asw_sep_infer(asw_sep* m, const float* mix, int M, int T, const int32_t* offsets, int S, float* out,
                  void* stream);

int asw_sep_infer_batch(asw_sep* m, const float* mix, int K, int M, int T, const int32_t* offsets,
                        const int32_t* counts, float* out, void* stream);

int asw_sep_forward(asw_sep* m, const float* mix_norm, int B, int S, int M, int t, float* out, void* stream);
int asw_sep_forward_counts(asw_sep* m, const float* mix_norm, int B, int S, int M, int t, const int32_t* counts,
                           float* out, void* stream);
int asw_sep_get_config(const asw_sep* m, asw_sep_config* out);

int asw_sep_get_tap(asw_sep* m, const char* name, float* dst, size_t capacity, size_t* numel, void* stream);

int asw_joint_shift_stats(const float* mix, int M, int T, const int32_t* offsets, int S, double* scratch,
                          float* mean, float* std, void* stream);
int asw_joint_shift_stats_scratch_doubles(void);
int asw_joint_shift_stats_groups(const float* mix, int M, int T, const int32_t* offsets, const int32_t* bounds, int G,
                                 const int32_t* item_of_group, double* scratch, float* mean, float* std, void* stream);

int asw_add_layernorm2(const float* x, const float* y, float alpha, const float* gamma, const float* beta,
                       int rows, int N, float eps, int act, float* sum_out, float* ln_out, void* stream);

int asw_glu_rows(const float* raw, long rows, int C, float* out, void* stream);

int asw_dwconv_ln_swish(const float* u, const float* wT, const float* bias, const float* gamma, const float* beta,
                        int BS, int L, int d, int K, float eps, float* out, void* stream);

int asw_relpos_attention(const float* qkv, const float* P, const float* bias_u, const float* bias_v, int BS, int L,
                         int d, int nhead, float scale, float* ctx, void* stream);

int asw_inter_attention(const float* qkv, int NB, int S, int L, int d, int nhead, float* ctx, void* stream);
int asw_inter_attention_groups(const float* qkv, const int32_t* bounds, int G, int L, int d, int nhead, float* ctx,
                               void* stream);


int asw_shift_stats(const float* mix, int M, int T, const int32_t* offsets, int N,
                    int circular, float* mean, float* std, void* stream);

int asw_shift_norm_preproc(const float* mix, int M, int T, int T_pad, const int32_t* offsets,
                           int N, int circular, const float* mean, const float* std,
                           const float* w, const float* b, int C, float* x0, float* refn,
                           long refn_stride, void* stream);

int asw_shift_stats_multi(const float* mix, int M, int T, const int32_t* offsets, const int32_t* mix_index, int N,
                          int circular, float* mean, float* std, void* stream);
int asw_shift_norm_preproc_multi(const float* mix, int M, int T, int T_pad, const int32_t* offsets,
                                 const int32_t* mix_index, int N, int circular, const float* mean, const float* std,
                                 const float* w, const float* b, int C, float* x0, float* refn, long refn_stride,
                                 void* stream);

int asw_shift_norm_src_multi(const float* mix, int M, int T, int T_pad, const int32_t* offsets,
                             const int32_t* mix_index, int N, int circular, const float* mean, const float* std,
                             void* src_hi, void* src_lo, float* refn, long refn_stride, void* stream);

int asw_pad_preproc(const float* x, int B, int M, int t, int T_pad, const float* w,
                    const float* b, int C, float* x0, float* refn, long refn_stride,
                    void* stream);

typedef struct asw_convgemm_args {
  const float* A;
  const float* A2;
  const float* Wt;
  const float* bias;
  const float* resid;
  const float* mul;
  const float* ln_gamma;
  const float* ln_beta;
  float* out;
  float* stats;
  int32_t B, M_out, N, Cin, taps, stride, dil, pad;
  int32_t a_row_stride;
  int64_t a_batch_stride;
  int64_t a_len;
  int32_t chan_mod;
  int32_t relu;
  float ln_eps;
  int32_t precision;
  int32_t w_shift;
  const void* Wt_hi;
  const void* Wt_lo;
  const void* Wf_hi;
  const void* Wf_lo;
  int32_t stats_stride;
  const float* glu_raw;
  const float* glu_mr;
  const float* glu_gamma;
  const float* glu_beta;
  float* glu_out;
} asw_convgemm_args;
int asw_pack_fragments_f16(const float* Wt, int N, int K, uint16_t* hi, uint16_t* lo, int32_t* w_shift);
int asw_convgemm_f32(const asw_convgemm_args* args, void* stream);
typedef struct asw_maskpath_args {
  asw_convgemm_args enc;
  const float* ref;
  int64_t ref_batch_stride;
  int64_t ref_len;
  int32_t ref_hop;
  int32_t byp_k;
  int32_t byp_taps;
  int32_t byp_shift;
  const void* byp_hi;
  const void* byp_lo;
  const float* byp_bias;
  const void* dec_hi;
  const void* dec_lo;
  int32_t dec_shift;
  int32_t dec_taps;
  float* taps;
} asw_maskpath_args;
int asw_mask_path_f16x3(const asw_maskpath_args* args, void* stream);
int asw_mask_path_f16x3_scaled(const asw_maskpath_args* args, void* stream);
typedef struct asw_reslayer_desc {
  const void* Wf_hi;
  const void* Wf_lo;
  const float* bias;
  const float* ln_gamma;
  const float* ln_beta;
  int32_t dil;
  int32_t w_shift;
} asw_reslayer_desc;
typedef struct asw_resstack_args {
  const float* x;
  float* out;
  int32_t B, T, C, taps, n_layers;
  int32_t precision;
  float ln_eps;
  asw_reslayer_desc layer[3];
  const float* glu_raw;
  const float* glu_mr;
  const float* glu_gamma;
  const float* glu_beta;
  float* glu_out;
  const void* src_hi;
  const void* src_lo;
  const void* pre_hi;
  const void* pre_lo;
  int32_t pre_shift;
  const void* up_hi;
  const void* up_lo;
  int32_t up_shift;
  const float* up_bias;
  const float* up_skip;
  float* up_out;
  float* up_stats;
} asw_resstack_args;
int asw_resstack64_f16x3(const asw_resstack_args* args, void* stream);
int asw_resstack_tiles(int T, int taps, int n_layers, const int32_t* dil, int glu);
int asw_up_feed_kperm(int k);
int asw_pack_up_feed_f16(const float* Wt, int N, int K, uint16_t* hi, uint16_t* lo, int32_t* w_shift);
int asw_compose_source_weights(const float* wc, const float* wpre, const float* bpre, int M, int taps, float* comp,
                               float* pre16);
int asw_split_weights_f16(const float* w, size_t n, uint16_t* hi, uint16_t* lo, int32_t* w_shift);
int asw_f16x3_overflow_count(int reset, uint32_t* count);
int asw_convgemm_stats_tiles(int M_out, int N);
#define ASW_RESIDUE_MAX_TAPS 8
#define ASW_RESIDUE_MAX_SHIFT 2
typedef struct asw_residue_stage {
  int32_t residue;
  int32_t chunk;
  int32_t rows;
  int32_t first_row;
  int32_t ntaps;
  int32_t tap[ASW_RESIDUE_MAX_TAPS];
  int32_t shift[ASW_RESIDUE_MAX_TAPS];
  int32_t kstep[ASW_RESIDUE_MAX_TAPS];
} asw_residue_stage;
int asw_residue_schedule(int taps, int stride, int dil, int pad, int Cin, int BK, int BM, int m0, int has_skip,
                         asw_residue_stage* out, int cap, int* n_stages, int* max_shift);

int asw_gn_glu(const float* raw, const float* stats, int n_partials, const float* gamma,
               const float* beta, int B, int T, int C, float eps, float* out, void* stream);
int asw_gn_finalize(const float* stats, int n_partials, int B, int T, int C, float eps, float* mr, void* stream);

int asw_attention(const float* qkv, int B, int L, int d, int nhead, float* ctx, void* stream);
int asw_attention_prec(const float* qkv, int B, int L, int d, int nhead, int precision, float* ctx, void* stream);

int asw_overlap_add_unnorm(const float* D, int B, int F, int ldd, int taps, int hop,
                           int t, int trim_left, int trim_right, float bias, const float* mean,
                           const float* std, float* out, void* stream);
int asw_overlap_add_parts(const float* D, int nparts, int B, int F, int ldd, int taps, int hop,
                          int t, int trim_left, int trim_right, float bias, const float* mean,
                          const float* std, float* out, void* stream);

int asw_energies(const float* y, int B, int T, int window, double* scratch, double* out,
                 void* stream);

int asw_add_layernorm(const float* x, const float* resid, const float* gamma, const float* beta,
                      int rows, int N, float eps, float* out, void* stream);

int asw_center_rows(float* y, int B, int T, void* stream);

int asw_pair_sisdr(const float* y, int n, int T, double* out, void* stream);

int asw_segment_sisdr(const float* y, int n, int T, const int32_t* segments, const int32_t* seg_count,
                      int kmax, double* out, void* stream);

size_t asw_voiced_segments_workspace_bytes(int n, int T);
int asw_voiced_segments(const float* y, int n, int T, double thr, double Q, int32_t* segments, int kcap,
                        int32_t* counts, double* ms, void* workspace, size_t workspace_bytes, void* stream);

size_t asw_fine_clusters_workspace_bytes(const int32_t* bounds_host, int G);
int asw_fine_clusters(const float* y, int N, int T, const int32_t* bounds_host, int G, const double* energies,
                      const double* gate, const double* group_gate, double min_trigger, double ratio, void* workspace,
                      size_t workspace_bytes, int32_t* order, int32_t* label, double* gram, void* stream);

size_t asw_global_clusters_workspace_bytes(int n);
int asw_global_clusters(const double* full, const double* seg, const int32_t* counts, const uint8_t* near, int n, int K,
                        double sim_db, double win_hi, double win_lo, double best_hi, double best_lo, void* workspace,
                        size_t workspace_bytes, int32_t* label, uint8_t* merge_or_null, void* stream);

size_t asw_coarse_select_workspace_bytes(int N, int cap);
int asw_coarse_select(const double* energies, const double* dis1, const int32_t* best_or_null, int N, double thr1,
                      int relative, double rel, int cap, void* workspace, size_t workspace_bytes, int32_t* kept,
                      int32_t* counts, double* thr, void* stream);

size_t asw_bss_eval_sdr_workspace_bytes(const int32_t* counts_host, int K, int R, int T, int flen);
int asw_bss_eval_sdr(const float* ref, const float* est, const int32_t* counts_host, int K, int R, int T, int flen,
                     double* sdr, int32_t* status, void* workspace, size_t workspace_bytes, void* stream);

size_t asw_cross_sisdr_workspace_bytes(const int32_t* est_counts_host, const int32_t* ref_counts_host, int K, int T);
int asw_cross_sisdr(const float* est, const float* ref, const int32_t* est_counts_host, const int32_t* ref_counts_host,
                    int K, int T, double* out, int32_t* status, void* workspace, size_t workspace_bytes, void* stream);

int asw_search_area(const double* points, int n_pts, const double* mic, int M, double* offset,
                    double* width, const double* ub, double sound_speed, double fs, int* n_children,
                    double** child_offset, double** child_width, int** child_count, int** child_index);
void asw_free(void* p);

int asw_cube_select(const double* offsets, int ny, int nx, int nz, int P, int y0, int y1, int x0, int x1,
                    const double* lo, const double* hi, int32_t* out_idx, int64_t cap, int64_t* count);
int asw_cube_select_planes(const double* planes, int ny, int nx, int nz, int P, int y0, int y1, int x0, int x1,
                    const double* lo, const double* hi, int32_t* out_idx, int64_t cap, int64_t* count);

int asw_srp_frames(int window, int nfft, int hop);
int asw_srp_cross_spectra(const float* mix, int M, int T, int window, int step, int n_windows,
                          int nfft, int hop, int nbins, int nb_pad, float tol,
                          const float* twiddle, const int32_t* pair_i, const int32_t* pair_j,
                          int P, float* xf_scratch, float* cc, void* stream);
int asw_srp_map(const float* cc, int n_windows, int nbins, int P, const double* tau, int G, int M,
                const double* omega, const int32_t* pair_i, const int32_t* pair_j,
                float* part_scratch, float* out, void* stream);

int asw_pruner_covariance(const float* mix, int M, int T, int window, int step, int n_windows,
                          int nfft, int hop, int bin0, int nbins, double* cov, double* magsum,
                          void* stream);
int asw_hermitian_eigh(const double* a, int n, int M, double* evals, double* evecs, void* stream);
int asw_music_map(const double* evecs, int n_windows, int nbins, int M, const double* tau, int G,
                  const double* omega, double* p_scratch, double* max_scratch, float* out,
                  void* stream);
int asw_tops_map(const double* evecs, const double* magsum, int n_windows, int nbins, int bin0,
                 int M, const double* delta, int G, double coef, double* q_scratch,
                 int32_t* max_bin, float* out, void* stream);
// ... 29 lines not shown
```

Baseline: 2471 candidates/s.

## Tile dilated residual convs over phase-major runs instead of per-phase blocks

Adds a 'run' form of the polyphase dilated residual conv kernel. Rows are ordered phase-major and tiled contiguously, so one tile can span several phase segments. Each segment gets its own halo in LDS, and a per-tile row table drives the epilogue scatter. This is meant to remove the padding waste of per-phase tiling when rows per phase are few or not a multiple of the block, and so cut wasted MFMA work and tile count. In exchange it adds per-row index arithmetic (float-reciprocal division), extra LDS for halos and the row table, and a new dispatch heuristic keyed on N and rows per phase.

New measurement: 2485 candidates/s (median of 6 runs). About the same (+0.6%).

```diff
diff --git a/acousticswarms-speech_amd/csrc/asw_common.cpp b/acousticswarms-speech_amd/csrc/asw_common.cpp
--- a/acousticswarms-speech_amd/csrc/asw_common.cpp
+++ b/acousticswarms-speech_amd/csrc/asw_common.cpp
@@ -1,4 +1,5 @@
 #include "asw_common.h"
+#include "poly_runs.h"
 
 #include <cmath>
 #include <cstdlib>
@@ -126,6 +127,50 @@
   return ASW_OK;
 }
 
+namespace asw {
+bool poly_runs_on() {
+  static const bool off = getenv("ASW_POLY_PER_PHASE") != nullptr;
+  return !off;
+}
+}
+
+extern "C" int asw_poly_run_schedule(int T, int dil, int taps, int BM, int tile, asw_poly_segment* out, int cap, int* n_segs,
+                                     int* img_rows, int* n_tiles, int* max_segs, int* lds_rows) {
+  ASW_CHECK_ARG(cap >= 0 && (out != nullptr || cap == 0), "poly_run_schedule: null pointer");
+  ASW_CHECK_ARG(asw::poly_runs_ok(T, dil, taps) && BM >= 2, "poly_run_schedule: bad dims (T=%d dil=%d taps=%d BM=%d)", T, dil, taps, BM);
+  const int nt = asw::cdiv(T, BM);
+  ASW_CHECK_ARG(tile >= 0 && tile < nt, "poly_run_schedule: tile %d of %d", tile, nt);
+  const asw::PolyRuns m = asw::PolyRuns::make(T, dil, 0);
+  const asw::PolyTile t(m, taps, BM, tile);
+  int n = 0, prev_ph = -1;
+  for (int i = 0; i < t.rows; ++i) {
+    int g;
+    const int ir = asw::poly_tile_row(m, t, taps, i, g);
+    const int ph = g % dil;
+    if (ph != prev_ph) {
+      if (n < cap) out[n] = asw_poly_segment{ph, g / dil, 0, i, ir};
+      ++n;
+      prev_ph = ph;
+    }
+    if (n <= cap) ++out[n - 1].rows;
+  }
+  if (n_segs) *n_segs = n;
+  if (img_rows) *img_rows = t.img_rows;
+  if (n_tiles) *n_tiles = nt;
+  if (max_segs) *max_segs = asw::poly_run_nseg(T, dil, BM);
+  if (lds_rows) *lds_rows = asw::poly_run_image_rows(T, dil, taps, BM);
+  return ASW_OK;
+}
+
+extern "C" int asw_poly_run_image_row(int T, int dil, int taps, int BM, int tile, int img_row, int* seq_row) {
+  ASW_CHECK_ARG(seq_row != nullptr, "poly_run_image_row: null pointer");
+  ASW_CHECK_ARG(asw::poly_runs_ok(T, dil, taps) && BM >= 2 && tile >= 0 && tile < asw::cdiv(T, BM) && img_row >= 0,
+                "poly_run_image_row: bad dims (T=%d dil=%d taps=%d BM=%d tile=%d)", T, dil, taps, BM, tile);
+  const asw::PolyRuns m = asw::PolyRuns::make(T, dil, 0), x = asw::PolyRuns::make(T, dil, taps - 1);
+  *seq_row = asw::poly_image_src(m, x, asw::PolyTile(m, taps, BM, tile), taps, img_row);
+  return ASW_OK;
+}
+
 #include <map>
 #include <mutex>
 #include <vector>
diff --git a/acousticswarms-speech_amd/csrc/model_common.h b/acousticswarms-speech_amd/csrc/model_common.h
--- a/acousticswarms-speech_amd/csrc/model_common.h
+++ b/acousticswarms-speech_amd/csrc/model_common.h
@@ -192,7 +192,7 @@
   return asw_resstack_tiles(T, K, (int)n, dil, glu && j0 == 0);
 }
 
-inline int run_res(const std::vector<ResLayer>& res, int prec, int B, int T, int ch, int K, float* x, float* p, float* q,
+inline int run_res(const std::vector<ResLayer>& res, int prec, int poly_runs, int B, int T, int ch, int K, float* x, float* p, float* q,
             float** final_out, hipStream_t s, const GluSrc* glu = nullptr, const SrcFeed* feed = nullptr, UpFeed* up = nullptr) {
   const float* in = glu ? glu->raw : x;
   float* outb = p;
@@ -229,6 +229,7 @@
         if (up->tiles < 0) return up->tiles;
         outb = nullptr;
       }
+      a.poly_runs = poly_runs;
       int rc = asw_resstack64_f16x3(&a, s);
       if (rc) return rc;
       in = outb;
@@ -249,6 +250,7 @@
     a.pad = (res[j].dil * (K - 1) + 1) / 2;
     a.a_row_stride = ch; a.a_batch_stride = (int64_t)T * ch; a.a_len = (int64_t)T * ch;
     a.relu = 1; a.ln_eps = 1e-5f;
+    a.poly_runs = poly_runs;
     int rc = asw_convgemm_f32(&a, s);
     if (rc) return rc;
     in = outb;
@@ -345,6 +347,7 @@
   bool src_stack = true;
   bool want_up = false;
   bool up_fusion = true;
+  int poly_runs = 1;
 
   std::vector<int> enc_cin, enc_cout;
   std::vector<int> dec_cin, dec_cout, dec_stride;
@@ -608,7 +611,7 @@
     bool glu = false;
     for (int i = 0; i < tc.depth; ++i) {
       float* r = nullptr;
-      if ((rc = run_res(enc[i].res, precision, B, pl.Tl[i], enc_cin[i], K, pl.X[i], pl.Pb[i], pl.Qb[i], &r, s,
+      if ((rc = run_res(enc[i].res, precision, poly_runs, B, pl.Tl[i], enc_cin[i], K, pl.X[i], pl.Pb[i], pl.Qb[i], &r, s,
                         glu ? &src : nullptr, (src0 && i == 0) ? &feed : nullptr)))
         return rc;
       asw_convgemm_args a = {};
@@ -659,11 +662,11 @@
       if (fuse_mask && glu_on_load_ok(dec[j].res, precision, co)) {
         if ((rc = asw_gn_finalize(pl.st_up[j], tiles, B, To, co, 1e-5f, pl.mr_up[j], s))) return rc;
         const GluSrc src = {pl.raw_up[j], pl.mr_up[j], dec[j].gn_g.p, dec[j].gn_b.p, co > 64 ? gb : nullptr};
-        if ((rc = run_res(dec[j].res, precision, B, To, co, K, gb, pl.Pb[lvl - 1], gb, &r, s, &src, nullptr, ufp))) return rc;
+        if ((rc = run_res(dec[j].res, precision, poly_runs, B, To, co, K, gb, pl.Pb[lvl - 1], gb, &r, s, &src, nullptr, ufp))) return rc;
       } else {
         if ((rc = asw_gn_glu(pl.raw_up[j], pl.st_up[j], tiles, dec[j].gn_g.p, dec[j].gn_b.p, B, To, co, 1e-5f, gb, s)))
           return rc;
-        if ((rc = run_res(dec[j].res, precision, B, To, co, K, gb, pl.Pb[lvl - 1], gb, &r, s, nullptr, nullptr, ufp))) return rc;
+        if ((rc = run_res(dec[j].res, precision, poly_runs, B, To, co, K, gb, pl.Pb[lvl - 1], gb, &r, s, nullptr, nullptr, ufp))) return rc;
       }
       x = r;
       fed_tiles = feed_next ? uf.tiles : 0;
diff --git a/acousticswarms-speech_amd/csrc/poly_runs.h b/acousticswarms-speech_amd/csrc/poly_runs.h
--- /dev/null
+++ b/acousticswarms-speech_amd/csrc/poly_runs.h
@@ -0,0 +1,79 @@
+#pragma once
+#include "asw_common.h"
+
+namespace asw {
+
+struct PolyRuns {
+  int d, q, r, nb, total;
+  float inv_long, inv_short;
+
+  static inline PolyRuns make(int T, int d, int extra) {
+    PolyRuns m;
+    m.d = d; m.q = T / d + extra; m.r = T % d;
+    m.nb = m.r * (m.q + 1); m.total = m.q * d + m.r;
+    m.inv_long = 1.0f / (float)(m.q + 1);
+    m.inv_short = m.q > 0 ? 1.0f / (float)m.q : 0.f;
+    return m;
+  }
+  ASW_HOST_DEVICE int len(int ph) const { return ph < r ? q + 1 : q; }
+  ASW_HOST_DEVICE int start(int ph) const { return ph * q + (ph < r ? ph : r); }
+  ASW_HOST_DEVICE static int div(int m, int L, float inv) {
+    int k = (int)((float)m * inv);
+    if (k * L > m) --k;
+    else if ((k + 1) * L <= m) ++k;
+    return k;
+  }
+  ASW_HOST_DEVICE void row(int n, int& ph, int& j) const {
+    if (n < nb) {
+      ph = div(n, q + 1, inv_long);
+      j = n - ph * (q + 1);
+    } else {
+      const int m = n - nb, k = div(m, q, inv_short);
+      ph = r + k;
+      j = m - k * q;
+    }
+  }
+  ASW_HOST_DEVICE int phase(int n) const { int ph, j; row(n, ph, j); return ph; }
+};
+
+bool poly_runs_on();
+inline bool poly_runs_ok(int T, int d, int taps) {
+  return T > 0 && d > 0 && taps > 0 && taps % 2 == 1 && (long)T + (long)d * (taps - 1) < (1L << 22);
+}
+inline int poly_run_nseg(int T, int d, int BM) {
+  const int q = T / d;
+  const int nonempty = q > 0 ? d : T, by_len = (BM - 2) / (q > 0 ? q : 1) + 2;
+  return nonempty < by_len ? nonempty : by_len;
+}
+inline int poly_run_image_rows(int T, int d, int taps, int BM) { return BM + poly_run_nseg(T, d, BM) * (taps - 1); }
+
+struct PolyTile {
+  int n0, ph0, e0, rows, nseg, img_rows;
+  PolyTile() = default;
+  ASW_HOST_DEVICE PolyTile(const PolyRuns& m, int taps, int BM, int tile) {
+    n0 = tile * BM;
+    rows = m.total - n0 < BM ? m.total - n0 : BM;
+    ph0 = m.phase(n0);
+    e0 = n0 + ph0 * (taps - 1);
+    nseg = m.phase(n0 + rows - 1) - ph0 + 1;
+    img_rows = BM + nseg * (taps - 1);
+  }
+};
+
+ASW_HOST_DEVICE inline int poly_image_src(const PolyRuns& m, const PolyRuns& x, const PolyTile& t, int taps, int i) {
+  const int e = t.e0 + i;
+  if (i >= t.img_rows || e >= x.total) return -1;
+  int ph, jx;
+  x.row(e, ph, jx);
+  const int j = jx - (taps - 1) / 2;
+  return (j >= 0 && j < m.len(ph)) ? ph + m.d * j : -1;
+}
+ASW_HOST_DEVICE inline int poly_tile_row(const PolyRuns& m, const PolyTile& t, int taps, int i, int& seq_row) {
+  const int n = t.n0 + i;
+  int ph, j;
+  m.row(n < m.total ? n : m.total - 1, ph, j);
+  seq_row = n < m.total ? ph + m.d * j : -1;
+  return i + (ph - t.ph0) * (taps - 1);
+}
+
+}
diff --git a/acousticswarms-speech_amd/csrc/resconv.hip b/acousticswarms-speech_amd/csrc/resconv.hip
--- a/acousticswarms-speech_amd/csrc/resconv.hip
+++ b/acousticswarms-speech_amd/csrc/resconv.hip
@@ -1,4 +1,5 @@
 #include "gemm_epilogue.h"
+#include "poly_runs.h"
 
 namespace {
 using namespace asw_mfma;
@@ -7,6 +8,11 @@
 __device__ unsigned long long g_phase_cycles[4] = {0, 0, 0, 0};
 #endif
 
+struct ResRunArgs : asw_convgemm_args { asw::PolyRuns rows, ext; int row_tab; };
+struct ResRowsRun {
+  const int* tab;
+  __device__ __forceinline__ int operator()(int trow) const { return tab[trow]; }
+};
 template <int BM, int PH, bool POLY>
 struct ResRows {
   static constexpr int BMJ = BM / PH;
@@ -19,11 +25,12 @@
   }
 };
 
-template <int BM, int C, int WM, int WN, int PH, int QD = 4, bool POLY = (PH > 1), bool GLU = false, int NTERM = 3>
+template <int BM, int C, int WM, int WN, int PH, int QD = 4, bool POLY = (PH > 1), bool GLU = false, int NTERM = 3, bool RUN = false>
 __global__ __launch_bounds__(64 * WM * WN)
 __attribute__((amdgpu_waves_per_eu(C == 64 ? 4 : WM * WN == 8 ? 2 : (QD == 2 ? (C >= 512 || (C == 256 && BM == 128) ? 2 : 3) : (C == 64 && WM * WN == 4 ? 4 : 1)))))
-void resconv16_kernel(const asw_convgemm_args p) {
+void resconv16_kernel(const std::conditional_t<RUN, ResRunArgs, asw_convgemm_args> p) {
   static_assert(QD == 2 || QD == 4, "B prefetch depth in k-steps");
+  static_assert(!RUN || (POLY && PH == 1 && !GLU), "run form: one phase-major run per tile");
   static_assert(!GLU || (PH == 1 && !POLY), "GroupNorm + GLU on load: contiguous tiles only");
   static_assert(WM * WN == 2 || WM * WN == 4 || WM * WN == 8, "2, 4 or 8 waves per workgroup");
   constexpr int NTHR = 64 * WM * WN;
@@ -45,7 +52,19 @@
   const int jb = !POLY ? 0 : blockIdx.x / n_pb, pb = !POLY ? 0 : blockIdx.x % n_pb;
   const int m0 = blockIdx.x * BM;
   const int RJ = BMJ + (!POLY ? (taps - 1) * dil : taps - 1);
-  const int R = PH * RJ;
+  asw::PolyTile pt;
+  if constexpr (RUN) {
+    const asw::PolyTile v(p.rows, taps, BM, blockIdx.x);
+    pt.n0 = __builtin_amdgcn_readfirstlane(v.n0); pt.ph0 = __builtin_amdgcn_readfirstlane(v.ph0);
+    pt.e0 = __builtin_amdgcn_readfirstlane(v.e0); pt.rows = __builtin_amdgcn_readfirstlane(v.rows);
+    pt.nseg = __builtin_amdgcn_readfirstlane(v.nseg); pt.img_rows = __builtin_amdgcn_readfirstlane(v.img_rows);
+  }
+  const int R = RUN ? pt.img_rows : PH * RJ;
+  int* row_tab = nullptr;
+  if constexpr (RUN) {
+    row_tab = reinterpret_cast<int*>(img + p.row_tab);
+    for (int i = tid; i < BM; i += NTHR) asw::poly_tile_row(p.rows, pt, taps, i, row_tab[i]);
+  }
   const int tapstep = !POLY ? dil : 1;
   const __amdgpu_buffer_rsrc_t rX = GLU ? act_rsrc(p.glu_raw + (long)b * T * 2 * C, (long)T * 2 * C)
                                         : act_rsrc(p.A + (long)b * p.a_batch_stride, (long)T * C);
@@ -66,6 +85,10 @@
   for (int i = 0; i < TM; ++i) {
     const int trow = wm * (BM / WM) + i * 32;
     a_base[i] = ((trow / BMJ) * RJ + trow % BMJ + (lane & 31)) * RS + (lane >> 5) * 16;
+    if constexpr (RUN) {
+      int g;
+      a_base[i] = asw::poly_tile_row(p.rows, pt, taps, trow + (lane & 31), g) * RS + (lane >> 5) * 16;
+    }
   }
   const int nt0 = wn * TN;
 
@@ -80,11 +103,17 @@
     ASW_PHASE_MARK(t_s0);
     if (GLU) gc.affine(p.glu_gamma, p.glu_beta, C, cc * 64 + sc4 * 4);
     __syncthreads();
+    int per_slice = 0;
+    if constexpr (RUN) asm volatile("" : "+s"(per_slice));
     stage_image<NTHR, C, SU, GLU, NTERM, C == 64>(
         img, R, rX, cc * 64, gc,
         [&](int row) __attribute__((always_inline)) {
           int g;
           bool ok = row < R;
+          if constexpr (RUN) {
+            g = asw::poly_image_src(p.rows, p.ext, pt, taps, row + per_slice);
+            return ImgSrc{g, g >= 0};
+          }
           if (!POLY) {
             g = m0 - pad + row;
           } else {
@@ -160,7 +189,11 @@
       for (int st = 0; st < G::NSTEP; ++st) {
         const int sr = (st * G::NW + wid) * G::RPI + sub;
         const int trow = (sr >> 5) * (BM / WM) + tm * 32 + (sr & 31);
-        const int irow = POLY ? (trow / BMJ) * RJ + trow % BMJ + (taps - 1) / 2 : trow + pad;
+        int irow = POLY ? (trow / BMJ) * RJ + trow % BMJ + (taps - 1) / 2 : trow + pad;
+        if constexpr (RUN) {
+          int g;
+          irow = asw::poly_tile_row(p.rows, pt, taps, trow, g) + (taps - 1) / 2;
+        }
 #pragma unroll
         for (int q = 0; q < G::VPL; ++q) {
           const int col = (lc + q * G::LPR) * 4;
@@ -170,8 +203,15 @@
                                                                 (float)hi[2] + (float)lo[2], (float)hi[3] + (float)lo[3]);
         }
       }
+    if constexpr (RUN)
+      epilogue<BM, C, WM, WN, true, false, true, false, ResRowsRun, true>(
+          acc, p, smem, __builtin_ldexpf(1.0f, -p.w_shift), ResRowsRun{row_tab}, blockIdx, gridDim.y, rpre);
+    else
     epilogue<BM, C, WM, WN, true, false, true, false, ResRows<BM, PH, POLY>, true>(
         acc, p, smem, __builtin_ldexpf(1.0f, -p.w_shift), ResRows<BM, PH, POLY>{m0, jb, pb, dil, T}, blockIdx, gridDim.y, rpre);
+  } else if constexpr (RUN) {
+    epilogue<BM, C, WM, WN, true, false, true, false>(acc, p, smem, __builtin_ldexpf(1.0f, -p.w_shift),
+                                                      ResRowsRun{row_tab}, blockIdx, gridDim.y);
   } else {
     epilogue<BM, C, WM, WN, true, false, true, false>(acc, p, smem, __builtin_ldexpf(1.0f, -p.w_shift),
                                                       ResRows<BM, PH, POLY>{m0, jb, pb, dil, T}, blockIdx, gridDim.y);
@@ -190,21 +230,30 @@
 #endif
 }
 
-template <int BM, int C, int WM, int WN, int PH, int QD = 4, bool POLY = (PH > 1), bool GLU = false>
+template <int BM, int C, int WM, int WN, int PH, int QD = 4, bool POLY = (PH > 1), bool GLU = false, bool RUN = false>
 int launch_res(const asw_convgemm_args& a, hipStream_t s) {
   constexpr int BMJ = BM / PH;
   const int RJ = BMJ + (!POLY ? (a.taps - 1) * a.dil : a.taps - 1);
-  const size_t img = (size_t)PH * RJ * RS;
+  const size_t img = (size_t)(RUN ? asw::poly_run_image_rows(a.M_out, a.dil, a.taps, BM) : PH * RJ) * RS;
   const size_t slab = (size_t)(WM * 32) * (C + 4) * sizeof(float);
-  const size_t smem = img > slab ? img : slab;
+  const size_t tiles = ((img > slab ? img : slab) + 15) / 16 * 16;
+  const size_t smem = tiles + (RUN ? BM * sizeof(int) : 0);
   if (smem > 160 * 1024) return 1;
-  const int gx = !POLY ? asw::cdiv(a.M_out, BM)
-                       : asw::cdiv(asw::cdiv(a.M_out, a.dil), BMJ) * asw::cdiv(a.dil, PH);
-  char nm[96];
-  snprintf(nm, sizeof nm, "resconv16<%d,%d,%s%d%s%s>", BM, C, POLY ? "poly" : "ph", PH, QD == 2 ? ",q2" : "", GLU ? ",glu" : "");
-  asw_convgemm_args k = a;
+  const int gx = !POLY || RUN ? asw::cdiv(a.M_out, BM)
+                              : asw::cdiv(asw::cdiv(a.M_out, a.dil), BMJ) * asw::cdiv(a.dil, PH);
+  char nm[96], rows[16];
+  if (RUN) snprintf(rows, sizeof rows, "run");
+  else snprintf(rows, sizeof rows, "%s%d", POLY ? "poly" : "ph", PH);
+  snprintf(nm, sizeof nm, "resconv16<%d,%d,%s%s%s>", BM, C, rows, QD == 2 ? ",q2" : "", GLU ? ",glu" : "");
+  std::conditional_t<RUN, ResRunArgs, asw_convgemm_args> k;
+  static_cast<asw_convgemm_args&>(k) = a;
+  if constexpr (RUN) {
+    k.rows = asw::PolyRuns::make(a.M_out, a.dil, 0);
+    k.ext = asw::PolyRuns::make(a.M_out, a.dil, a.taps - 1);
+    k.row_tab = (int)tiles;
+  }
   if (GLU && C > 64) k.resid = a.glu_out;
-  return asw::launch_pair<resconv16_kernel<BM, C, WM, WN, PH, QD, POLY, GLU, 1>, resconv16_kernel<BM, C, WM, WN, PH, QD, POLY, GLU, 3>>(
+  return asw::launch_pair<resconv16_kernel<BM, C, WM, WN, PH, QD, POLY, GLU, 1, RUN>, resconv16_kernel<BM, C, WM, WN, PH, QD, POLY, GLU, 3, RUN>>(
       a.precision, dim3(gx, 1, a.B), dim3(64 * WM * WN), smem, 160 * 1024, nm, asw::ShapeTag(a, 'd', a.dil).s,
       2.0 * a.B * (double)a.M_out * a.N * (double)a.taps * a.Cin, 0.0, s, k);
 }
@@ -236,6 +285,21 @@
   }
   const int rows_per_phase = a.M_out / a.dil;
   const bool poly = a.dil >= 16 && rows_per_phase >= 32;
+  const bool big = (long)asw::cdiv(a.M_out, 128) * a.B >= 512;
+  const int runs = poly_runs_on() && a.dil >= 16 && poly_runs_ok(a.M_out, a.dil, a.taps) ? a.poly_runs : 0;
+  if (runs >= 2 || (runs == 1 && ((a.N == 512 && rows_per_phase < 64) || (a.N == 256 && big && rows_per_phase >= 48)))) {
+    int rc = 1;
+    switch (a.N) {
+      case 64: rc = launch_res<128, 64, 2, 2, 1, 4, true, false, true>(a, s); break;
+      case 128: rc = launch_res<128, 128, 2, 2, 1, 2, true, false, true>(a, s); break;
+      case 256:
+        rc = big ? launch_res<128, 256, 1, 4, 1, 2, true, false, true>(a, s) : launch_res<64, 256, 1, 4, 1, 2, true, false, true>(a, s);
+        break;
+      case 512: rc = launch_res<64, 512, 1, 4, 1, 2, true, false, true>(a, s); break;
+      default: break;
+    }
+    if (rc != 1) return rc;
+  }
   switch (a.N) {
     case 64:
       if (a.glu_raw) return launch_res<128, 64, 2, 2, 1, 4, false, true>(a, s);
diff --git a/acousticswarms-speech_amd/csrc/resstack.hip b/acousticswarms-speech_amd/csrc/resstack.hip
--- a/acousticswarms-speech_amd/csrc/resstack.hip
+++ b/acousticswarms-speech_amd/csrc/resstack.hip
@@ -2,6 +2,7 @@
 
 #include "asw_common.h"
 #include "f16x3_tile.h"
+#include "poly_runs.h"
 
 namespace {
 using namespace asw_mfma;
@@ -57,6 +58,7 @@
   float scale;
 };
 struct KArgsUp : KArgs { UpArgs u; };
+struct KArgsRun : KArgs { asw::PolyRuns rows, ext; };
 
 __device__ __forceinline__ __amdgpu_buffer_rsrc_t src_rsrc(const half8* base, long rows) {
   return __builtin_amdgcn_make_buffer_rsrc(const_cast<half8*>(base), 0, (int)(rows * 16), 0x00020000);
@@ -65,9 +67,10 @@
   return __builtin_bit_cast(half8, __builtin_amdgcn_raw_buffer_load_b128(r, row >= 0 ? row * 16 : (int)0x80000000, 0, 0));
 }
 
-template <int NL, int NW, int TM, int PH, bool POLY, bool GLU, int NTERM, int QD, bool SRC = false, bool UP = false>
+template <int NL, int NW, int TM, int PH, bool POLY, bool GLU, int NTERM, int QD, bool SRC = false, bool UP = false, bool RUN = false>
 __global__ __launch_bounds__(64 * NW) __attribute__((amdgpu_waves_per_eu(TM >= 4 ? 1 : 2)))
-void resstack64_kernel(const std::conditional_t<UP, KArgsUp, KArgs> p) {
+void resstack64_kernel(const std::conditional_t<UP, KArgsUp, std::conditional_t<RUN, KArgsRun, KArgs>> p) {
+  static_assert(!RUN || (POLY && PH == 1 && !GLU && !SRC && !UP), "run form: one phase-major run per tile, plain single layers");
   static_assert(!UP || (!SRC && NTERM == 3), "UpFeed: f16x3, never source-fed");
   static_assert(!POLY || NL == 1, "polyphase row sets: single layers only");
   static_assert(!SRC || (!POLY && !GLU && NTERM == 3), "source-fed layer 0: contiguous tiles, f16x3");
@@ -91,7 +94,18 @@
   const int jb = POLY ? tile / n_pb : 0, pb = POLY ? tile - jb * n_pb : 0;
   const int m0 = tile * p.BM;
   const int RJ = BMJ + taps - 1;
-  const int R_img = POLY ? PH * RJ : R0 + 2 * pad0;
+  asw::PolyTile pt;
+  if constexpr (RUN) {
+    const asw::PolyTile v(p.rows, taps, R0, tile);
+    pt.n0 = __builtin_amdgcn_readfirstlane(v.n0); pt.ph0 = __builtin_amdgcn_readfirstlane(v.ph0);
+    pt.e0 = __builtin_amdgcn_readfirstlane(v.e0); pt.rows = __builtin_amdgcn_readfirstlane(v.rows);
+    pt.nseg = __builtin_amdgcn_readfirstlane(v.nseg); pt.img_rows = __builtin_amdgcn_readfirstlane(v.img_rows);
+  }
+  auto run_row = [&](int trow, int& t) __attribute__((always_inline)) {
+    if constexpr (RUN) return asw::poly_tile_row(p.rows, pt, taps, trow, t);
+    else { t = -1; return 0; }
+  };
+  const int R_img = RUN ? pt.img_rows : POLY ? PH * RJ : R0 + 2 * pad0;
 
   RS_MARK(t_start);
   if constexpr (!SRC) {
@@ -120,7 +134,9 @@
         const int row = r0 + u * SROWS + srow;
         int g;
         bool ok = row < R_img;
-        if (!POLY) {
+        if constexpr (RUN) {
+          g = asw::poly_image_src(p.rows, p.ext, pt, taps, row);
+        } else if (!POLY) {
           g = m0 - p.L[0].halo - pad0 + row;
         } else {
           const int ph = pb * PH + row / RJ;
@@ -190,6 +206,10 @@
 #pragma unroll
       for (int i = 0; i < NF; ++i) {
         xb[i] = (img_row((wid * TM + i) * 32) + (lane & 31)) * RS + h * 16;
+        if constexpr (RUN) {
+          int t;
+          xb[i] = run_row((wid * TM + i) * 32 + (lane & 31), t) * RS + h * 16;
+        }
         a[i][0] = acc[i][0];
         a[i][1] = acc[i][1];
       }
@@ -284,7 +304,8 @@
     for (int i = 0; i < TM; ++i) {
       if (i < nf) {
         const int trow = (wid * TM + i) * 32 + (lane & 31);
-        const char* rrow = img + (img_row(trow) + cpad) * RS;
+        int trun;
+        const char* rrow = img + ((RUN ? run_row(trow, trun) : img_row(trow)) + cpad) * RS;
         float s = 0.f;
 #pragma unroll
         for (int cb = 0; cb < 2; ++cb)
@@ -465,7 +486,10 @@
           const int trow = (wid * TM + i) * 32 + (lane & 31);
           int t;
           bool ok;
-          if (!POLY) {
+          if constexpr (RUN) {
+            run_row(trow, t);
+            ok = t >= 0;
+          } else if (!POLY) {
             t = m0 + trow;
             ok = trow < p.BM && t < T;
           } else {
@@ -511,12 +535,23 @@
 #endif
 }
 
-template <int NL, int NW, int TM, int PH, bool POLY, bool GLU, int QD, bool SRC = false>
+template <int NL, int NW, int TM, int PH, bool POLY, bool GLU, int QD, bool SRC = false, bool RUN = false>
 int launch_stack(const KArgs& k, const UpArgs* up, int precision, size_t smem, double flops, const char* tag, hipStream_t s) {
   char nm[128], detail[48] = "";
-  snprintf(nm, sizeof nm, "resstack64<%s,%dx%d%s%s%s%s>", tag, NW, TM, POLY ? (PH == 1 ? ",poly1" : PH == 2 ? ",poly2" : ",poly4") : "",
+  snprintf(nm, sizeof nm, "resstack64<%s,%dx%d%s%s%s%s>", tag, NW, TM,
+           RUN ? ",run" : POLY ? (PH == 1 ? ",poly1" : PH == 2 ? ",poly2" : ",poly4") : "",
            GLU ? ",glu" : "", SRC ? ",src" : "", up ? ",up" : "");
   if (asw::prof_detail()) snprintf(detail, sizeof detail, "[B%d M%d d%d]", k.B, k.T, k.L[0].dil);
+  if constexpr (RUN) {
+    KArgsRun kr;
+    static_cast<KArgs&>(kr) = k;
+    kr.rows = asw::PolyRuns::make(k.T, k.L[0].dil, 0);
+    kr.ext = asw::PolyRuns::make(k.T, k.L[0].dil, k.taps - 1);
+    return asw::launch_pair<resstack64_kernel<NL, NW, TM, PH, POLY, GLU, 1, QD, false, false, true>,
+                            resstack64_kernel<NL, NW, TM, PH, POLY, GLU, 3, QD, false, false, true>>(
+        precision, dim3(xcd_grid_run(k.B * k.ntile)), dim3(64 * NW), smem, 160 * 1024, nm, detail, flops,
+        (double)k.B * k.T * C * 4 * 2, s, kr);
+  } else {
   if constexpr (!SRC) {
     if (up) {
       KArgsUp ku;
@@ -536,6 +571,7 @@
       precision, dim3(xcd_grid_run(k.B * k.ntile)), dim3(64 * NW), smem, 160 * 1024, nm, detail, flops,
       (double)k.B * k.T * C * 4 * (GLU ? 3 : 2), s, k);
   }
+  }
 }
 
 struct TilePlan { bool poly; int PH, BM, ntile; };
@@ -553,6 +589,17 @@
 int dispatch(const asw_resstack_args& a, KArgs& k, const UpArgs* up, bool glu, double flops, hipStream_t s) {
   constexpr int R0 = 32 * NW * TM;
   const int dil0 = k.L[0].dil;
+  if (a.poly_runs >= 2 && asw::poly_runs_on() && a.n_layers == 1 && dil0 >= 16 && !glu && !up && asw::poly_runs_ok(a.T, dil0, a.taps)) {
+    const int rows = asw::poly_run_image_rows(a.T, dil0, a.taps, R0);
+    const size_t smem = (size_t)rows * RS + 3 * 64 * sizeof(float);
+    if (smem <= 160 * 1024) {
+      k.BM = R0;
+      k.ntile = asw::cdiv(a.T, R0);
+      k.L[0].nfrag = NW * TM;
+      k.img_rows = rows;
+      return launch_stack<1, NW, TM, 1, true, false, 4, false, true>(k, nullptr, a.precision, smem, flops, "1", s);
+    }
+  }
   const TilePlan tp = plan_tiles(a.T, a.n_layers, dil0, k.L[0].halo, glu, R0);
   k.BM = tp.BM;
   k.ntile = tp.ntile;
diff --git a/acousticswarms-speech_amd/csrc/sep_model.hip b/acousticswarms-speech_amd/csrc/sep_model.hip
--- a/acousticswarms-speech_amd/csrc/sep_model.hip
+++ b/acousticswarms-speech_amd/csrc/sep_model.hip
@@ -263,6 +263,12 @@
 extern "C" void asw_sep_destroy(asw_sep* m) { delete m; }
 
 extern "C" int asw_sep_set_precision(asw_sep* m, int precision) { return set_precision(m, "sep_set_precision", precision); }
+extern "C" int asw_sep_set_poly_runs(asw_sep* m, int on) {
+  ASW_CHECK_ARG(m, "sep_set_poly_runs: null model handle");
+  ASW_CHECK_ARG(on >= 0 && on <= 2, "sep_set_poly_runs: 0 (per-phase tiles), 1 (runs where measured faster) or 2 (runs wherever they apply)");
+  m->poly_runs = on;
+  return ASW_OK;
+}
 
 extern "C" int asw_sep_set_param(asw_sep* m, const char* key, const float* host_data, size_t numel) {
   return set_param(m, "sep_set_param", key, host_data, numel);
diff --git a/acousticswarms-speech_amd/csrc/spot_model.hip b/acousticswarms-speech_amd/csrc/spot_model.hip
--- a/acousticswarms-speech_amd/csrc/spot_model.hip
+++ b/acousticswarms-speech_amd/csrc/spot_model.hip
@@ -348,6 +348,13 @@
   return ASW_OK;
 }
 
+extern "C" int asw_spot_set_poly_runs(asw_spot* m, int on) {
+  ASW_CHECK_ARG(m, "set_poly_runs: null model handle");
+  ASW_CHECK_ARG(on >= 0 && on <= 2, "set_poly_runs: 0 (per-phase tiles), 1 (runs where measured faster) or 2 (runs wherever they apply)");
+  m->poly_runs = on;
+  return ASW_OK;
+}
+
 extern "C" int asw_spot_get_tap(asw_spot* m, const char* name, float* dst, size_t capacity, size_t* numel,
                                 void* stream) {
   return get_tap(m, "get_tap", name, dst, capacity, numel, stream);
diff --git a/acousticswarms-speech_amd/native.py b/acousticswarms-speech_amd/native.py
--- a/acousticswarms-speech_amd/native.py
+++ b/acousticswarms-speech_amd/native.py
@@ -118,7 +118,7 @@
                 ("ln_eps", c_float), ("precision", c_int32), ("w_shift", c_int32), ("Wt_hi", c_void_p),
                 ("Wt_lo", c_void_p), ("Wf_hi", c_void_p), ("Wf_lo", c_void_p), ("stats_stride", c_int32),
                 ("glu_raw", c_void_p), ("glu_mr", c_void_p), ("glu_gamma", c_void_p), ("glu_beta", c_void_p),
-                ("glu_out", c_void_p)]
+                ("glu_out", c_void_p), ("poly_runs", c_int32)]
 
 
 class MaskPathArgs(Structure):
@@ -139,10 +139,14 @@
                 ("glu_raw", c_void_p), ("glu_mr", c_void_p), ("glu_gamma", c_void_p), ("glu_beta", c_void_p),
                 ("glu_out", c_void_p), ("src_hi", c_void_p), ("src_lo", c_void_p), ("pre_hi", c_void_p), ("pre_lo", c_void_p),
                 ("pre_shift", c_int32), ("up_hi", c_void_p), ("up_lo", c_void_p), ("up_shift", c_int32), ("up_bias", c_void_p),
-                ("up_skip", c_void_p), ("up_out", c_void_p), ("up_stats", c_void_p)]
+                ("up_skip", c_void_p), ("up_out", c_void_p), ("up_stats", c_void_p), ("poly_runs", c_int32)]
 
 
 RESIDUE_MAX_TAPS = 8
+
+
+class PolySegment(Structure):
+    _fields_ = [("phase", c_int32), ("j_first", c_int32), ("rows", c_int32), ("tile_row", c_int32), ("img_row", c_int32)]
 
 
 class ResidueStage(Structure):
@@ -173,12 +177,14 @@
     "asw_spot_set_fused_mask": (c_int, [c_void_p, c_int]),
     "asw_spot_set_source_stack": (c_int, [c_void_p, c_int]),
     "asw_spot_set_up_fusion": (c_int, [c_void_p, c_int]),
+    "asw_spot_set_poly_runs": (c_int, [c_void_p, c_int]),
     "asw_spot_get_tap": (c_int, [c_void_p, c_char_p, c_void_p, c_size_t, POINTER(c_size_t), c_void_p]),
     "asw_sep_create": (c_int, [POINTER(SepConfigC), POINTER(c_void_p)]),
     "asw_sep_destroy": (None, [c_void_p]),
     "asw_sep_set_param": (c_int, [c_void_p, c_char_p, c_void_p, c_size_t]),
     "asw_sep_finalize": (c_int, [c_void_p]),
     "asw_sep_set_precision": (c_int, [c_void_p, c_int]),
+    "asw_sep_set_poly_runs": (c_int, [c_void_p, c_int]),
     "asw_sep_infer": (c_int, [c_void_p, c_void_p, c_int, c_int, c_void_p, c_int, c_void_p, c_void_p]),
     "asw_sep_infer_batch": (c_int, [c_void_p, c_void_p, c_int, c_int, c_int, c_void_p, c_void_p, c_void_p, c_void_p]),
     "asw_sep_forward": (c_int, [c_void_p, c_void_p, c_int, c_int, c_int, c_int, c_void_p, c_void_p]),
@@ -220,6 +226,9 @@
     "asw_f16x3_overflow_count": (c_int, [c_int, POINTER(c_int32)]),
     "asw_residue_schedule": (c_int, [c_int, c_int, c_int, c_int, c_int, c_int, c_int, c_int, c_int,
                                      POINTER(ResidueStage), c_int, POINTER(c_int), POINTER(c_int)]),
+    "asw_poly_run_schedule": (c_int, [c_int, c_int, c_int, c_int, c_int, POINTER(PolySegment), c_int, POINTER(c_int),
+                                      POINTER(c_int), POINTER(c_int), POINTER(c_int), POINTER(c_int)]),
+    "asw_poly_run_image_row": (c_int, [c_int, c_int, c_int, c_int, c_int, c_int, POINTER(c_int)]),
     "asw_gn_glu": (c_int, [c_void_p, c_void_p, c_int, c_void_p, c_void_p, c_int, c_int, c_int, c_float, c_void_p,
                            c_void_p]),
     "asw_gn_finalize": (c_int, [c_void_p, c_int, c_int, c_int, c_int, c_float, c_void_p, c_void_p]),
@@ -340,6 +349,21 @@
     return stages, mx.value
 
 
+def poly_run_schedule(T, dil, BM, tile, taps=7):
+    n, ir, nt, ms, lr, g = c_int(), c_int(), c_int(), c_int(), c_int(), c_int()
+    L = lib()
+    check(L.asw_poly_run_schedule(T, dil, taps, BM, tile, None, 0, ctypes.byref(n), ctypes.byref(ir), ctypes.byref(nt),
+                                  ctypes.byref(ms), ctypes.byref(lr)))
+    buf = (PolySegment * n.value)()
+    check(L.asw_poly_run_schedule(T, dil, taps, BM, tile, buf, n.value, ctypes.byref(n), None, None, None, None))
+    image = []
+    for i in range(ir.value):
+        check(L.asw_poly_run_image_row(T, dil, taps, BM, tile, i, ctypes.byref(g)))
+        image.append(g.value)
+    return {"segments": [{k: getattr(d, k) for k, _ in PolySegment._fields_} for d in buf], "img_rows": ir.value,
+            "n_tiles": nt.value, "max_segs": ms.value, "lds_rows": lr.value, "image": image}
+
+
 def check(status: int):
     if status != 0:
         msg = lib().asw_last_error()
diff --git a/acousticswarms-speech_amd/ops.py b/acousticswarms-speech_amd/ops.py
--- a/acousticswarms-speech_amd/ops.py
+++ b/acousticswarms-speech_amd/ops.py
@@ -17,7 +17,7 @@
 
 def convgemm(A, Wt, M_out, N, Cin, taps=1, stride=1, dil=1, pad=0, bias=None, relu=False, resid=None, mul=None,
              ln=None, stats_chan_mod=0, A2=None, B=None, a_row_stride=None, a_batch_stride=None, a_len=None,
-             out=None, ln_eps=1e-5, precision="f32", use_fragments=True, glu=None, glu_out=None):
+             out=None, ln_eps=1e-5, precision="f32", use_fragments=True, glu=None, glu_out=None, poly_runs=0):
     _f32(A); _f32(Wt)
     if B is None:
         B = A.shape[0]
@@ -44,6 +44,7 @@
     a.B, a.M_out, a.N, a.Cin, a.taps, a.stride, a.dil, a.pad = B, M_out, N, Cin, taps, stride, dil, pad
     a.a_row_stride, a.a_batch_stride, a.a_len = a_row_stride, a_batch_stride, a_len
     a.chan_mod, a.relu, a.ln_eps = stats_chan_mod, int(relu), ln_eps
+    a.poly_runs = int(poly_runs)
     if glu is not None:
         a.glu_raw, a.glu_mr, a.glu_gamma, a.glu_beta = (_f32(t).data_ptr() for t in glu)
         if glu_out is not None:
@@ -63,7 +64,7 @@
     return out, stats
 
 
-def resstack(x, layers, taps=7, precision="f16x3", eps=1e-5, glu=None, out=None, glu_out=None):
+def resstack(x, layers, taps=7, precision="f16x3", eps=1e-5, glu=None, out=None, glu_out=None, poly_runs=0):
     src = x if glu is None else glu[0]
     B, T = src.shape[0], src.shape[1]
     if out is None:
@@ -73,6 +74,7 @@
     a.out = out.data_ptr()
     a.B, a.T, a.C, a.taps, a.n_layers = B, T, 64, taps, len(layers)
     a.precision, a.ln_eps = (1 if precision == "f16x3" else 2), eps
+    a.poly_runs = int(poly_runs)
     keep = []
     for i, (Wt, bias, gamma, beta, dil) in enumerate(layers):
         fh, fl, sh = pack_fragments_f16(_f32(Wt), 64, taps * 64)
diff --git a/acousticswarms-speech_amd/spot.py b/acousticswarms-speech_amd/spot.py
--- a/acousticswarms-speech_amd/spot.py
+++ b/acousticswarms-speech_amd/spot.py
@@ -170,3 +170,8 @@
         self._need()
         native.check(native.lib().asw_spot_set_up_fusion(self._h, int(bool(on))))
         return self
+
+    def set_poly_runs(self, on: int = 1):
+        self._need()
+        native.check(native.lib().asw_spot_set_poly_runs(self._h, int(on)))
+        return self
diff --git a/include/asw_hip.h b/include/asw_hip.h
--- a/include/asw_hip.h
+++ b/include/asw_hip.h
@@ -70,6 +70,8 @@
 int asw_spot_set_source_stack(asw_spot* m, int on);
 
 int asw_spot_set_up_fusion(asw_spot* m, int on);
+
+int asw_spot_set_poly_runs(asw_spot* m, int on);
 
 int asw_spot_get_tap(asw_spot* m, const char* name, float* dst, size_t capacity, size_t* numel,
                      void* stream);
@@ -100,6 +102,7 @@
 int asw_sep_set_param(asw_sep* m, const char* key, const float* host_data, size_t numel);
 int asw_sep_finalize(asw_sep* m);
 int asw_sep_set_precision(asw_sep* m, int precision);
+int asw_sep_set_poly_runs(asw_sep* m, int on);
 
 int asw_sep_infer(asw_sep* m, const float* mix, int M, int T, const int32_t* offsets, int S, float* out,
                   void* stream);
@@ -189,6 +192,7 @@
   const float* glu_gamma;
   const float* glu_beta;
   float* glu_out;
+  int32_t poly_runs;
 } asw_convgemm_args;
 int asw_pack_fragments_f16(const float* Wt, int N, int K, uint16_t* hi, uint16_t* lo, int32_t* w_shift);
 int asw_convgemm_f32(const asw_convgemm_args* args, void* stream);
@@ -245,6 +249,7 @@
   const float* up_skip;
   float* up_out;
   float* up_stats;
+  int32_t poly_runs;
 } asw_resstack_args;
 int asw_resstack64_f16x3(const asw_resstack_args* args, void* stream);
 int asw_resstack_tiles(int T, int taps, int n_layers, const int32_t* dil, int glu);
@@ -270,6 +275,17 @@
 int asw_residue_schedule(int taps, int stride, int dil, int pad, int Cin, int BK, int BM, int m0, int has_skip,
                          asw_residue_stage* out, int cap, int* n_stages, int* max_shift);
 
+typedef struct asw_poly_segment {
+  int32_t phase;
+  int32_t j_first;
+  int32_t rows;
+  int32_t tile_row;
+  int32_t img_row;
+} asw_poly_segment;
+int asw_poly_run_schedule(int T, int dil, int taps, int BM, int tile, asw_poly_segment* out, int cap, int* n_segs,
+                          int* img_rows, int* n_tiles, int* max_segs, int* lds_rows);
+int asw_poly_run_image_row(int T, int dil, int taps, int BM, int tile, int img_row, int* seq_row);
+
 int asw_gn_glu(const float* raw, const float* stats, int n_partials, const float* gamma,
                const float* beta, int B, int T, int C, float eps, float* out, void* stream);
 int asw_gn_finalize(const float* stats, int n_partials, int B, int T, int C, float eps, float* mr, void* stream);
```
